# a-ludi/dentist

Measured on AMD Instinct MI355X. Metric: gap-bases closed/sec, higher is better.
Workload: dtype u8

## Files before the change

dentist_amd/_lib.py:

```python
import ctypes
import os
import weakref

import numpy as np

_HERE = os.path.dirname(os.path.abspath(__file__))


def lib_path():
    return os.environ.get("DH_DEV_LIB") or os.path.join(_HERE, "libdentist_hip.so")


class DhError(RuntimeError):
    def __init__(self, code, msg):
        super().__init__(f"libdentist_hip error {code}: {msg}")
        self.code = code


class AlignOpts(ctypes.Structure):
    _fields_ = [(n, ctypes.c_int32) for n in (
        "k", "hmin", "band_shift", "tspace", "min_len", "pen", "xdrop", "max_err_ppm", "max_cand",
        "max_la", "tcap", "strands", "skip_self", "dmax", "width", "kmer_mod", "algo")]


class AlignStats(ctypes.Structure):
    _fields_ = [("hits", ctypes.c_int64), ("cands", ctypes.c_int64), ("alignments", ctypes.c_int64),
                ("wave_cells", ctypes.c_int64), ("las", ctypes.c_int64), ("b_bases", ctypes.c_int64),
                ("ms_index", ctypes.c_float), ("ms_seed", ctypes.c_float), ("ms_wave", ctypes.c_float),
                ("ms_gather", ctypes.c_float), ("ms_total", ctypes.c_float),
                ("wave_launches", ctypes.c_int32), ("overflow_items", ctypes.c_int32), ("big_items", ctypes.c_int64)]

    def as_dict(self):
        return {n: getattr(self, n) for n, _ in self._fields_}


class CumStats(ctypes.Structure):
    _fields_ = [("ms_index", ctypes.c_double), ("ms_seed", ctypes.c_double), ("ms_wave", ctypes.c_double),
                ("ms_gather", ctypes.c_double)] + [(n, ctypes.c_int64) for n in (
                    "wave_launches", "wave_cells", "alignments", "las", "aligned_bp", "trace_values", "hits",
                    "b_bases")]

    def as_dict(self):
        return {n: getattr(self, n) for n, _ in self._fields_}


class ProcessOpts(ctypes.Structure):
    _fields_ = [(n, ctypes.c_int32) for n in (
        "tspace_map", "allowance", "min_anchor", "min_reads", "max_reads", "tspace_pile", "rounds",
        "flank_window", "max_align_err_ppm", "max_ins_err_ppm", "bad_fraction_ppm", "width", "dust", "algo",
        "max_partners", "min_relative_score_ppm")]


INSERTION_DTYPE = np.dtype([(n, "<i4") for n in (
    "contig_left", "status", "nreads", "ref_read", "ref_read_id", "crop_left", "crop_right", "left_aepos",
    "right_abpos", "ins_begin", "ins_end", "comp", "cons_len", "left_diffs", "right_diffs", "join")]
    + [("cons_off", "<i8"), ("contig_right", "<i4"), ("pad", "<i4")])

LA_DTYPE = np.dtype([("tlen", "<i4"), ("diffs", "<i4"), ("abpos", "<i4"), ("bbpos", "<i4"),
                     ("aepos", "<i4"), ("bepos", "<i4"), ("flags", "<u4"), ("aread", "<i4"),
                     ("bread", "<i4"), ("pad", "<i4"), ("toff", "<i8")])

SYMBOLS = [
    "dh_last_error", "dh_abi_version", "dh_ctx_create", "dh_ctx_destroy", "dh_ctx_sync",
    "dh_default_align_opts", "dh_db_create", "dh_db_destroy", "dh_db_drop_cache", "dh_db_nreads",
    "dh_db_total_bases", "dh_la_set_destroy", "dh_la_set_count", "dh_la_set_trace_len",
    "dh_la_set_records", "dh_la_set_trace", "dh_la_set_tspace", "dh_get_align_stats", "dh_get_cum_stats", "dh_get_mjoin_counts", "dh_ctx_release_scratch",
    "dh_align_db",
    "dh_las_write", "dh_las_read", "dh_default_process_opts", "dh_collect_spanning", "dh_pileups_destroy",
    "dh_pileups_count", "dh_pileups_get", "dh_process_pileups", "dh_insertions_destroy",
    "dh_insertions_count", "dh_insertions_records", "dh_insertions_bases", "dh_insertions_bases_len",
    "dh_get_process_stats", "dh_dazz_create_dam", "dh_dazz_create_db", "dh_dazz_split", "dh_dazz_open",
    "dh_dazz_close", "dh_dazz_nreads", "dh_dazz_first_id", "dh_dazz_bases", "dh_dazz_offsets",
    "dh_dazz_origin", "dh_dazz_fpulse", "dh_dazz_header", "dh_dazz_read_mask", "dh_dazz_write_mask",
    "dh_db_set_mask", "dh_output_fasta", "dh_tile_qv", "dh_consensus", "dh_las_merge",
    "dh_collect_candidates", "dh_pileups_create", "dh_pileups_select", "dh_align_db_block", "dh_la_set_merge",
    "dh_crop_pileups", "dh_cropped_create", "dh_cropped_destroy", "dh_cropped_npiles", "dh_cropped_records",
    "dh_cropped_nreads", "dh_cropped_pile", "dh_cropped_entry", "dh_cropped_read_id", "dh_cropped_offsets",
    "dh_cropped_bases", "dh_process_cropped", "dh_translate_trace_point", "dh_db_dust", "dh_db_get_mask",
    "dh_dazz_write_track", "dh_dazz_read_track", "dh_dazz_remove", "dh_dazz_flags",
    "dh_pileupdb_write", "dh_pileupdb_read", "dh_insertiondb_write", "dh_insertiondb_read", "dh_insertiondb_merge", "dh_chaindb_destroy",
    "dh_chaindb_npiles", "dh_chaindb_pile_counts", "dh_chaindb_nread_alignments", "dh_chaindb_read_alignment_counts",
    "dh_chaindb_nseeded", "dh_chaindb_seeded", "dh_chaindb_nlas", "dh_chaindb_las", "dh_chaindb_ntrace",
    "dh_chaindb_trace", "dh_chaindb_ninsertions", "dh_chaindb_insertions", "dh_chaindb_bases", "dh_chaindb_read_ids",
    "dh_insertions_write_db", "dh_pileups_write_db", "dh_pileups_flat", "dh_collect_filter",
    "dh_map_reads", "dh_validate_regions", "dh_propagate_mask", "dh_db_mask_coverage", "dh_max_coverage_reads", "dh_max_improper_coverage_reads",
    "dh_default_scaffold_opts", "dh_scaffold_pileups", "dh_scaffold_npiles", "dh_scaffold_nentries", "dh_scaffold_joins",
    "dh_scaffold_entries", "dh_scaffold_destroy", "dh_scaffold_spanning", "dh_scaffold_gap_pileups", "dh_cropped_create2",
    "dh_cropped_kind", "dh_get_process_work", "dh_scaffold_pileups_cb", "dh_scaffold_pileups_resolved", "dh_comm_unique_id", "dh_comm_create", "dh_comm_create_local", "dh_comm_destroy",
    "dh_comm_rank", "dh_comm_world", "dh_comm_all_gather", "dh_comm_all_to_all", "dh_shard_run", "dh_set_near_best", "dh_ctx_set_near_best", "dh_shard_free", "dh_shard_pack_candidates", "dh_shard_plan_create", "dh_shard_read_joins", "dh_align_db_transposed", "dh_remap_skipping_reads", "dh_shard_graph_plan_create", "dh_shard_plan_destroy",
    "dh_shard_plan_las", "dh_shard_plan_nlas", "dh_shard_plan_pileups", "dh_shard_plan_owner", "dh_shard_pack_cropped",
    "dh_shard_unpack_cropped", "dh_insertions_read_ids", "dh_insertions_read_ids_off", "dh_output_assembly", "dh_default_output_opts",
    "dh_common_trace_point", "dh_pileups_create_joins", "dh_pileups_get_join", "dh_scaffold_all_pileups",
    "dh_crop_pileups_masked", "dh_process_pileups_masked", "dh_process_pileups_set", "dh_la_set_trace_on_device", "dh_scaffold_graph_probe",
    "dh_la_edit_paths", "dh_la_set_edit_paths", "dh_edit_paths_destroy", "dh_edit_paths_count", "dh_edit_paths_op_off",
    "dh_edit_paths_ops", "dh_edit_paths_score", "dh_edit_paths_tile_off", "dh_edit_paths_tile_score",
    "dh_edit_paths_general_tiles", "dh_format_cigar", "dh_format_alignment", "dh_la_transpose", "dh_la_set_transpose",
]

_LIB = None


def lib():
    global _LIB
    if _LIB is not None:
        return _LIB
    path = lib_path()
    if not os.path.exists(path):
        raise RuntimeError(f"{path} is missing: build it with `make` or __graft_entry__.build(); "
                           "dentist_amd has no CPU fallback")
    L = ctypes.CDLL(path)
    vp, i32, i64 = ctypes.c_void_p, ctypes.c_int32, ctypes.c_int64
    L.dh_last_error.restype = ctypes.c_char_p
    L.dh_abi_version.restype = i32
    L.dh_ctx_create.argtypes = [i32, vp, ctypes.POINTER(vp)]
    L.dh_ctx_destroy.argtypes = [vp]
    L.dh_ctx_sync.argtypes = [vp]
    L.dh_default_align_opts.argtypes = [ctypes.POINTER(AlignOpts)]
    L.dh_db_create.argtypes = [vp, vp, vp, i32, vp, ctypes.POINTER(vp)]
    L.dh_db_destroy.argtypes = [vp]
    L.dh_db_drop_cache.argtypes = [vp]
    L.dh_db_nreads.argtypes = [vp]
    L.dh_db_nreads.restype = i32
    L.dh_db_total_bases.argtypes = [vp]
    L.dh_db_total_bases.restype = i64
    L.dh_la_set_destroy.argtypes = [vp]
    L.dh_la_set_count.argtypes = [vp]
    L.dh_la_set_count.restype = i64
    L.dh_la_set_trace_len.argtypes = [vp]
    L.dh_la_set_trace_len.restype = i64
    L.dh_la_set_records.argtypes = [vp]
    L.dh_la_set_records.restype = vp
    L.dh_la_set_trace.argtypes = [vp]
    L.dh_la_set_trace.restype = vp
    L.dh_la_set_tspace.argtypes = [vp]
    L.dh_la_set_tspace.restype = i32
    L.dh_get_align_stats.argtypes = [vp, ctypes.POINTER(AlignStats)]
    L.dh_get_cum_stats.argtypes = [vp, ctypes.POINTER(CumStats), i32]
    L.dh_align_db.argtypes = [vp, vp, vp, ctypes.POINTER(AlignOpts), i32, ctypes.POINTER(vp)]
    L.dh_align_db_block.argtypes = [vp, vp, vp, i32, i32, ctypes.POINTER(AlignOpts), i32, ctypes.POINTER(vp)]
    L.dh_la_set_merge.argtypes = [ctypes.POINTER(vp), i32, ctypes.POINTER(vp)]
    L.dh_las_write.argtypes = [ctypes.c_char_p, vp, i64, vp, i32]
    L.dh_las_read.argtypes = [ctypes.c_char_p, ctypes.POINTER(vp)]
    L.dh_default_process_opts.argtypes = [ctypes.POINTER(ProcessOpts)]
    L.dh_collect_spanning.argtypes = [vp, i64, vp, i32, ctypes.POINTER(ProcessOpts), ctypes.POINTER(vp)]
    L.dh_collect_candidates.argtypes = L.dh_collect_spanning.argtypes
    L.dh_pileups_create.argtypes = [vp, vp, i32, vp, ctypes.POINTER(vp)]
    L.dh_pileups_select.argtypes = [vp, vp, i64, ctypes.POINTER(ProcessOpts), ctypes.POINTER(vp)]
    L.dh_pileups_destroy.argtypes = [vp]
    L.dh_pileups_count.argtypes = [vp]
    L.dh_pileups_count.restype = i32
    L.dh_pileups_get.argtypes = [vp, i32, ctypes.POINTER(i32), ctypes.POINTER(vp)]
    L.dh_pileups_get.restype = i32
    L.dh_process_pileups.argtypes = [vp, vp, vp, vp, i64, vp, vp, ctypes.POINTER(ProcessOpts), ctypes.POINTER(vp)]
    L.dh_crop_pileups.argtypes = [vp, vp, vp, i32, vp, i64, vp, vp, ctypes.POINTER(ProcessOpts), ctypes.POINTER(vp)]
    L.dh_cropped_create.argtypes = [vp, i32, i32, vp, vp, vp, vp, vp, ctypes.POINTER(vp)]
    L.dh_cropped_create2.argtypes = [vp, i32, i32, vp, vp, vp, vp, vp, vp, ctypes.POINTER(vp)]
    L.dh_cropped_kind.argtypes = [vp]
    L.dh_cropped_kind.restype = vp
    L.dh_cropped_destroy.argtypes = [vp]
    for fn in (L.dh_cropped_npiles, L.dh_cropped_nreads):
        fn.argtypes = [vp]
        fn.restype = i32
    for fn in (L.dh_cropped_records, L.dh_cropped_pile, L.dh_cropped_entry, L.dh_cropped_read_id,
               L.dh_cropped_offsets, L.dh_cropped_bases):
        fn.argtypes = [vp]
        fn.restype = vp
    L.dh_process_cropped.argtypes = [vp, vp, vp, ctypes.POINTER(ProcessOpts), ctypes.POINTER(vp)]
    L.dh_translate_trace_point.argtypes = [vp, vp, i32, i32, i32, ctypes.POINTER(i32), ctypes.POINTER(i32)]
    L.dh_insertions_destroy.argtypes = [vp]
    L.dh_insertions_count.argtypes = [vp]
    L.dh_insertions_count.restype = i32
    L.dh_insertions_records.argtypes = [vp]
    L.dh_insertions_records.restype = vp
    L.dh_insertions_bases.argtypes = [vp]
    L.dh_insertions_bases.restype = vp
    L.dh_insertions_bases_len.argtypes = [vp]
    L.dh_insertions_bases_len.restype = i64
    L.dh_get_process_stats.argtypes = [vp, vp, vp]
    L.dh_dazz_create_dam.argtypes = [ctypes.c_char_p, ctypes.c_char_p, i64]
    L.dh_dazz_create_db.argtypes = [ctypes.c_char_p, ctypes.c_char_p, i64]
    L.dh_dazz_split.argtypes = [ctypes.c_char_p, i32, i32, i64]
    L.dh_dazz_open.argtypes = [ctypes.c_char_p, ctypes.POINTER(vp)]
    L.dh_dazz_close.argtypes = [vp]
    L.dh_dazz_nreads.argtypes = [vp]
    L.dh_dazz_nreads.restype = i32
    L.dh_dazz_first_id.argtypes = [vp]
    L.dh_dazz_first_id.restype = i32
    for fn in (L.dh_dazz_bases, L.dh_dazz_offsets, L.dh_dazz_origin, L.dh_dazz_fpulse):
        fn.argtypes = [vp]
        fn.restype = vp
    L.dh_dazz_header.argtypes = [vp, i32]
    L.dh_dazz_read_mask.argtypes = [vp, ctypes.c_char_p, ctypes.c_char_p, vp, vp, i64]
    L.dh_dazz_read_mask.restype = i64
    L.dh_dazz_write_mask.argtypes = [ctypes.c_char_p, ctypes.c_char_p, i32, vp, vp]
    L.dh_db_set_mask.argtypes = [vp, vp, vp]
    L.dh_db_dust.argtypes = [vp]
    L.dh_db_get_mask.argtypes = [vp, vp, vp, i64]
    L.dh_db_get_mask.restype = i64
    L.dh_las_merge.argtypes = [ctypes.POINTER(ctypes.c_char_p), i32, ctypes.c_char_p]
    L.dh_tile_qv.argtypes = [vp, vp, vp, i64, vp, i32, i32, vp, i32]
    L.dh_consensus.argtypes = [vp, vp, vp, i64, vp, i32, i32, i32, vp, i64, ctypes.POINTER(i64)]
    L.dh_output_fasta.argtypes = [ctypes.c_char_p, ctypes.c_char_p, vp, vp, i32, vp, ctypes.POINTER(ctypes.c_char_p),
                                  vp, vp, i32, vp, i32, i32]
    L.dh_dazz_header.restype = ctypes.c_char_p
    L.dh_la_edit_paths.argtypes = [vp, vp, vp, vp, i64, vp, i32, i64, i64, ctypes.POINTER(vp)]
    L.dh_la_set_edit_paths.argtypes = [vp, vp, vp, vp, i64, i64, ctypes.POINTER(vp)]
    L.dh_la_transpose.argtypes = [vp, vp, vp, vp, i64, vp, i32, i32, ctypes.POINTER(vp), vp]
    L.dh_la_set_transpose.argtypes = [vp, vp, vp, vp, i32, ctypes.POINTER(vp), vp]
    L.dh_edit_paths_destroy.argtypes = [vp]
    L.dh_edit_paths_destroy.restype = None
    for fn in (L.dh_edit_paths_count, L.dh_edit_paths_general_tiles):
        fn.argtypes = [vp]
        fn.restype = i64
    for fn in (L.dh_edit_paths_op_off, L.dh_edit_paths_ops, L.dh_edit_paths_score, L.dh_edit_paths_tile_off,
               L.dh_edit_paths_tile_score):
        fn.argtypes = [vp]
        fn.restype = vp
    L.dh_format_cigar.argtypes = [vp, i64, i32, vp, i64]
    L.dh_format_cigar.restype = i64
    L.dh_format_alignment.argtypes = [vp, vp, vp, i64, i32, vp, i64]
    L.dh_format_alignment.restype = i64
    _LIB = L
    return L


def _check(rc):
    if rc != 0:
        raise DhError(rc, lib().dh_last_error().decode(errors="replace"))


def default_align_opts(**kw):
    o = AlignOpts()
    lib().dh_default_align_opts(ctypes.byref(o))
    for k, v in kw.items():
        if not hasattr(o, k):
            raise AttributeError(k)
        setattr(o, k, v)
    return o


class _LaSetOwner:

    def __init__(self, h):
        self._h = h

    def __del__(self):
        try:
            if self._h:
                lib().dh_la_set_destroy(self._h)
                self._h = None
        except Exception:
            pass


def _take_la_set(h):
    L = lib()
    n, tn = L.dh_la_set_count(h), L.dh_la_set_trace_len(h)
    ts = L.dh_la_set_tspace(h)
    owner = _LaSetOwner(h)
    if n:
        buf = (ctypes.c_uint8 * (n * LA_DTYPE.itemsize)).from_address(L.dh_la_set_records(h))
        buf._owner = owner
        las = np.frombuffer(buf, dtype=LA_DTYPE)
    else:
        las = np.zeros(0, dtype=LA_DTYPE)
    if tn:
        buf = (ctypes.c_uint16 * tn).from_address(L.dh_la_set_trace(h))
        buf._owner = owner
        trace = np.frombuffer(buf, dtype=np.uint16)
    else:
        trace = np.zeros(0, dtype=np.uint16)
    return las, trace, ts


class Context:

    def __init__(self, device=0, stream=None):
        h = ctypes.c_void_p()
        _check(lib().dh_ctx_create(device, ctypes.c_void_p(stream) if stream else None, ctypes.byref(h)))
        self._h = h
        self._dbs = []

    def close(self):
        if self._h:
            for ref in self._dbs:
                d = ref()
                if d is not None:
                    d.close()
            self._dbs = []
            lib().dh_ctx_destroy(self._h)
            self._h = None

    def __del__(self):
        try:
            self.close()
        except Exception:
            pass

    def sync(self):
        _check(lib().dh_ctx_sync(self._h))

    def db(self, seqdb):
        return Db(self, seqdb)

    def align_stats(self):
        st = AlignStats()
        _check(lib().dh_get_align_stats(self._h, ctypes.byref(st)))
        return st

    def release_scratch(self):
        lib().dh_ctx_release_scratch.argtypes = [ctypes.c_void_p]
        _check(lib().dh_ctx_release_scratch(self._h))

    def mjoin_counts(self, reset=False):
        out = (ctypes.c_int64 * 2)()
        lib().dh_get_mjoin_counts.argtypes = [ctypes.c_void_p, ctypes.c_void_p, ctypes.c_int32]
        _check(lib().dh_get_mjoin_counts(self._h, out, int(reset)))
        return int(out[0]), int(out[1])

    def cum_stats(self, reset=False):
        st = CumStats()
        _check(lib().dh_get_cum_stats(self._h, ctypes.byref(st), int(reset)))
        return st

    def remap_skipping_reads(self, contigs, reads, contig_ids, read_ids, opts, allowance):
        ci = np.ascontiguousarray(contig_ids, dtype=np.int32)
        ri = np.ascontiguousarray(read_ids, dtype=np.int32)
        h = ctypes.c_void_p()
        L = lib()
        L.dh_remap_skipping_reads.argtypes = [ctypes.c_void_p, ctypes.c_void_p, ctypes.c_void_p, ctypes.c_void_p, ctypes.c_int32,
                                              ctypes.c_void_p, ctypes.c_int32, ctypes.c_void_p, ctypes.c_int32,
# ... 997 lines not shown
    nb = L.dh_insertions_bases_len(h)
    rec = (np.frombuffer(ctypes.string_at(L.dh_insertions_records(h), n * INSERTION_DTYPE.itemsize),
                         dtype=INSERTION_DTYPE).copy() if n else np.zeros(0, dtype=INSERTION_DTYPE))
    bases = (np.frombuffer(ctypes.string_at(L.dh_insertions_bases(h), nb), dtype=np.uint8).copy()
             if nb else np.zeros(0, dtype=np.uint8))
    ids = None
    if read_ids:
        L.dh_insertions_read_ids.restype = ctypes.c_void_p
        L.dh_insertions_read_ids_off.restype = ctypes.c_void_p
        L.dh_insertions_read_ids.argtypes = L.dh_insertions_read_ids_off.argtypes = [ctypes.c_void_p]
        po = L.dh_insertions_read_ids_off(h)
        if po and n:
            off = np.frombuffer(ctypes.string_at(po, 4 * (n + 1)), dtype=np.int32).astype(np.int64)
            tot = int(off[-1])
            idv = (np.frombuffer(ctypes.string_at(L.dh_insertions_read_ids(h), 4 * tot), dtype=np.int32).copy()
                   if tot else np.zeros(0, np.int32))
            ids = (idv, off)
        else:
            ids = (np.zeros(0, np.int32), np.zeros(n + 1, np.int64))
    L.dh_insertions_destroy(h)
    return (rec, bases, ids) if read_ids else (rec, bases)


def _mask_args(repeat_mask):
    if repeat_mask is None:
        return None, None, None
    rp = np.ascontiguousarray(repeat_mask[0], dtype=np.int64)
    ri = np.ascontiguousarray(np.concatenate([np.asarray(repeat_mask[1]).reshape(-1), [0, 0]]), dtype=np.int32)
    return (rp, ri), rp.ctypes.data, ri.ctypes.data


def process_pileups(ctx, contigs, reads, las, trace, piles, opts, insertions_db=None, read_ids=False, repeat_mask=None):
    L = lib()
    h = ctypes.c_void_p()
    keep, rp, ri = _mask_args(repeat_mask)
    if isinstance(trace, DeviceTrace):
        L.dh_process_pileups_set.argtypes = [ctypes.c_void_p] * 9
        _check(L.dh_process_pileups_set(ctx._h, contigs._h, reads._h, trace._h, piles._h, rp, ri, ctypes.byref(opts), ctypes.byref(h)))
        return _take_insertions(h, insertions_db, read_ids)
    arr = np.ascontiguousarray(las, dtype=LA_DTYPE)
    tr = np.ascontiguousarray(trace, dtype=np.uint16)
    L.dh_process_pileups_masked.argtypes = [ctypes.c_void_p] * 4 + [ctypes.c_int64] + [ctypes.c_void_p] * 6
    _check(L.dh_process_pileups_masked(ctx._h, contigs._h, reads._h, arr.ctypes.data, len(arr), tr.ctypes.data,
                                       piles._h, rp, ri, ctypes.byref(opts), ctypes.byref(h)))
    return _take_insertions(h, insertions_db, read_ids)


class OutputOpts(ctypes.Structure):
    _fields_ = [("line_width", ctypes.c_int32), ("highlight", ctypes.c_int32), ("join_policy", ctypes.c_int32),
                ("agp_dazzler", ctypes.c_int32), ("agp_skip_read_ids", ctypes.c_int32), ("only", ctypes.c_int32),
                ("agp_version", ctypes.c_char_p), ("tool", ctypes.c_char_p), ("input_assembly", ctypes.c_char_p),
                ("min_extension_length", ctypes.c_int32), ("pad", ctypes.c_int32)]


JOIN_POLICIES = {"scaffoldGaps": 0, "scaffolds": 1, "contigs": 2}


def output_assembly(fasta_path, contigs, scaffold_of, headers, gap_len, rec, bases, read_ids=None, bed_path=None,
                    agp_path=None, join_policy="scaffoldGaps", agp_dazzler=False, agp_skip_read_ids=False, read_names=None,
                    line_width=50, highlight=True, tool=None, input_assembly=None, only="spanning", min_extension_length=100):
    L = lib()
    o = OutputOpts()
    L.dh_default_output_opts.argtypes = [ctypes.POINTER(OutputOpts)]
    L.dh_default_output_opts(ctypes.byref(o))
    o.line_width, o.highlight, o.join_policy = line_width, int(bool(highlight)), JOIN_POLICIES[join_policy]
    o.agp_dazzler, o.agp_skip_read_ids = int(bool(agp_dazzler)), int(bool(agp_skip_read_ids))
    o.only, o.min_extension_length = {"spanning": 1, "extending": 2, "both": 3}[only], int(min_extension_length)
    if tool is not None:
        o.tool = tool.encode()
    if input_assembly is not None:
        o.input_assembly = input_assembly.encode()
    cb = np.ascontiguousarray(contigs.bases, dtype=np.uint8)
    co = np.ascontiguousarray(contigs.off, dtype=np.int64)
    so = np.ascontiguousarray(scaffold_of, dtype=np.int32)
    gl = np.ascontiguousarray(gap_len, dtype=np.int32) if gap_len is not None else None
    r = np.ascontiguousarray(rec, dtype=INSERTION_DTYPE)
    b = np.ascontiguousarray(bases, dtype=np.uint8)
    hs = (ctypes.c_char_p * len(headers))(*[h.encode() for h in headers])
    ids = off = None
    if read_ids is not None:
        ids = np.ascontiguousarray(read_ids[0], dtype=np.int32)
        off = np.ascontiguousarray(read_ids[1], dtype=np.int32)
    rn = (ctypes.c_char_p * len(read_names))(*[x.encode() for x in read_names]) if read_names is not None else None
    dropped = ctypes.c_int32(0)
    vp = ctypes.c_void_p
    L.dh_output_assembly.argtypes = [ctypes.c_char_p, ctypes.c_char_p, ctypes.c_char_p, vp, vp, ctypes.c_int32, vp, vp, vp, vp,
                                     ctypes.c_int32, vp, vp, vp, ctypes.c_int32, vp, ctypes.POINTER(OutputOpts), ctypes.POINTER(ctypes.c_int32)]
    _check(L.dh_output_assembly(fasta_path.encode(), bed_path.encode() if bed_path else None,
                                agp_path.encode() if agp_path else None, cb.ctypes.data, co.ctypes.data, len(co) - 1,
                                so.ctypes.data, ctypes.cast(hs, vp), gl.ctypes.data if gl is not None else None,
                                r.ctypes.data, len(r), b.ctypes.data if len(b) else None,
                                ids.ctypes.data if ids is not None and len(ids) else (ids.ctypes.data if ids is not None else None),
                                off.ctypes.data if off is not None else None, len(read_names) if read_names is not None else -1,
                                ctypes.cast(rn, vp) if rn is not None else None,
                                ctypes.byref(o), ctypes.byref(dropped)))
    return int(dropped.value)


def output_fasta(fasta_path, contigs, scaffold_of, headers, gap_len, rec, bases, bed_path=None, line_width=50,
                 highlight=True):
    cb = np.ascontiguousarray(contigs.bases, dtype=np.uint8)
    co = np.ascontiguousarray(contigs.off, dtype=np.int64)
    so = np.ascontiguousarray(scaffold_of, dtype=np.int32)
    gl = np.ascontiguousarray(gap_len, dtype=np.int32) if gap_len is not None else None
    r = np.ascontiguousarray(rec, dtype=INSERTION_DTYPE)
    b = np.ascontiguousarray(bases, dtype=np.uint8)
    hs = (ctypes.c_char_p * len(headers))(*[h.encode() for h in headers])
    _check(lib().dh_output_fasta(fasta_path.encode(), bed_path.encode() if bed_path else None, cb.ctypes.data,
                                 co.ctypes.data, len(co) - 1, so.ctypes.data, hs,
                                 gl.ctypes.data if gl is not None else None, r.ctypes.data, len(r),
                                 b.ctypes.data if len(b) else None, line_width, int(bool(highlight))))


def las_merge(paths, out_path):
    arr = (ctypes.c_char_p * len(paths))(*[p.encode() for p in paths])
    _check(lib().dh_las_merge(arr, len(paths), out_path.encode()))


def tile_qv(ctx, db, las, trace, tspace, cov, maxtiles):
    arr = np.ascontiguousarray(las, dtype=LA_DTYPE)
    tr = np.ascontiguousarray(trace, dtype=np.uint16)
    qv = np.zeros((lib().dh_db_nreads(db._h), maxtiles), dtype=np.uint8)
    _check(lib().dh_tile_qv(ctx._h, db._h, arr.ctypes.data, len(arr), tr.ctypes.data, tspace, cov, qv.ctypes.data,
                            maxtiles))
    return qv


def consensus(ctx, db, las, trace, tspace, ref_read, rounds=1):
    arr = np.ascontiguousarray(las, dtype=LA_DTYPE)
    tr = np.ascontiguousarray(trace, dtype=np.uint16)
    cap = 1 << 20
    while True:
        out = np.zeros(cap, dtype=np.uint8)
        n = ctypes.c_int64(0)
        rc = lib().dh_consensus(ctx._h, db._h, arr.ctypes.data, len(arr), tr.ctypes.data, tspace, ref_read, rounds,
                                out.ctypes.data, cap, ctypes.byref(n))
        if rc != 0 and n.value > cap:
            cap = int(n.value)
            continue
        _check(rc)
        return out[:n.value].copy()


def process_stats(ctx):
    ms = (ctypes.c_float * 7)()
    cnt = (ctypes.c_int64 * 3)()
    _check(lib().dh_get_process_stats(ctx._h, ms, cnt))
    names = ("crop", "pile_align", "tile_qv", "consensus", "realign", "flank_align", "total")
    d = {f"ms_{n}": float(ms[i]) for i, n in enumerate(names)}
    d.update(pile_las=int(cnt[0]), tiles=int(cnt[1]), nw_cells=int(cnt[2]))
    wk = (ctypes.c_int64 * 4)()
    _check(lib().dh_get_process_work(ctx._h, wk))
    d.update(pile_ups=int(wk[0]), entries=int(wk[1]), cropped_bases=int(wk[2]), algorithmic_bytes=int(wk[3]))
    return d


def dazz_create_dam(path, fasta_text):
    b = fasta_text.encode() if isinstance(fasta_text, str) else fasta_text
    _check(lib().dh_dazz_create_dam(path.encode(), b, len(b)))


def dazz_create_db(path, fasta_text):
    b = fasta_text.encode() if isinstance(fasta_text, str) else fasta_text
    _check(lib().dh_dazz_create_db(path.encode(), b, len(b)))


def dazz_split(path, cutoff=0, all_reads=True, size_mb=200):
    _check(lib().dh_dazz_split(path.encode(), cutoff, int(all_reads), size_mb))


class DazzDb:

    def __init__(self, path):
        L = lib()
        h = ctypes.c_void_p()
        _check(L.dh_dazz_open(path.encode(), ctypes.byref(h)))
        n = L.dh_dazz_nreads(h)
        self.first_id = L.dh_dazz_first_id(h)
        self.off = np.frombuffer((ctypes.c_int64 * (n + 1)).from_address(L.dh_dazz_offsets(h)), dtype=np.int64).copy()
        tot = int(self.off[-1])
        self.bases = (np.frombuffer((ctypes.c_uint8 * tot).from_address(L.dh_dazz_bases(h)), dtype=np.uint8).copy()
                      if tot else np.zeros(0, np.uint8))
        self.origin = (np.frombuffer((ctypes.c_int32 * n).from_address(L.dh_dazz_origin(h)), dtype=np.int32).copy()
                       if n else np.zeros(0, np.int32))
        self.fpulse = (np.frombuffer((ctypes.c_int32 * n).from_address(L.dh_dazz_fpulse(h)), dtype=np.int32).copy()
                       if n else np.zeros(0, np.int32))
        self.headers = [L.dh_dazz_header(h, i).decode() for i in range(n)]
        self.group = None
        self.mask = None
        self._h = h
        self._path = path

    def read_mask(self, name):
        L = lib()
        ptr = np.zeros(self.n + 1, dtype=np.int64)
        m = L.dh_dazz_read_mask(self._h, self._path.encode(), name.encode(), ptr.ctypes.data, None, 0)
        if m < 0:
            _check(int(m))
        iv = np.zeros(max(2 * m, 2), dtype=np.int32)
        L.dh_dazz_read_mask(self._h, self._path.encode(), name.encode(), ptr.ctypes.data, iv.ctypes.data, m)
        return ptr, iv[:2 * m]

    def close(self):
        if getattr(self, "_h", None):
            lib().dh_dazz_close(self._h)
            self._h = None

    def __del__(self):
        try:
            self.close()
        except Exception:
            pass

    @property
    def n(self):
        return len(self.off) - 1

    def seq(self, i):
        return self.bases[self.off[i]:self.off[i + 1]]


def dazz_write_mask(db_path, name, ptr, iv):
    p = np.ascontiguousarray(ptr, dtype=np.int64)
    v = np.ascontiguousarray(iv, dtype=np.int32)
    _check(lib().dh_dazz_write_mask(db_path.encode(), name.encode(), len(p) - 1, p.ctypes.data, v.ctypes.data))


SEEDED_DTYPE = np.dtype([("id", "<i8"), ("contig_a_id", "<u4"), ("contig_a_len", "<u4"), ("contig_b_id", "<u4"),
                         ("contig_b_len", "<u4"), ("flags", "u1"), ("seed", "u1"), ("tspace", "<u2"), ("nla", "<i4")])
CHAIN_LA_DTYPE = np.dtype([("a_begin", "<u4"), ("a_end", "<u4"), ("b_begin", "<u4"), ("b_end", "<u4"), ("diffs", "<u4"),
                           ("ntp", "<i4")])
INSERTION_REC_DTYPE = np.dtype([("start_contig", "<i8"), ("end_contig", "<i8"), ("start_part", "u1"), ("end_part", "u1"),
                                ("pad", "u1", (6,)), ("seq_len", "<i8"), ("contig_len", "<i8"), ("noverlaps", "<i4"),
                                ("nread_ids", "<i4")])
assert SEEDED_DTYPE.itemsize == 32 and CHAIN_LA_DTYPE.itemsize == 24 and INSERTION_REC_DTYPE.itemsize == 48


def _arr(ptr, n, dt):
    if not n:
        return np.zeros(0, dt)
    addr = ptr if isinstance(ptr, int) else ctypes.cast(ptr, ctypes.c_void_p).value
    return np.frombuffer((ctypes.c_uint8 * (n * np.dtype(dt).itemsize)).from_address(addr), dtype=dt).copy()


def _take_chaindb(h):
    L = lib()
    vp = ctypes.c_void_p
    for fn in ("dh_chaindb_pile_counts", "dh_chaindb_read_alignment_counts", "dh_chaindb_seeded", "dh_chaindb_las",
               "dh_chaindb_trace", "dh_chaindb_insertions", "dh_chaindb_bases", "dh_chaindb_read_ids"):
        getattr(L, fn).restype = vp
        getattr(L, fn).argtypes = [vp]
    for fn in ("dh_chaindb_nseeded", "dh_chaindb_nlas", "dh_chaindb_ntrace"):
        getattr(L, fn).restype = ctypes.c_int64
        getattr(L, fn).argtypes = [vp]
    for fn in ("dh_chaindb_npiles", "dh_chaindb_nread_alignments", "dh_chaindb_ninsertions"):
        getattr(L, fn).argtypes = [vp]
    L.dh_chaindb_destroy.argtypes = [vp]
    ins = _arr(L.dh_chaindb_insertions(h), L.dh_chaindb_ninsertions(h), INSERTION_REC_DTYPE)
    out = dict(pile_counts=_arr(L.dh_chaindb_pile_counts(h), L.dh_chaindb_npiles(h), np.int32),
               ra_counts=_arr(L.dh_chaindb_read_alignment_counts(h), L.dh_chaindb_nread_alignments(h), np.int32),
               seeded=_arr(L.dh_chaindb_seeded(h), L.dh_chaindb_nseeded(h), SEEDED_DTYPE),
               las=_arr(L.dh_chaindb_las(h), L.dh_chaindb_nlas(h), CHAIN_LA_DTYPE),
               trace=_arr(L.dh_chaindb_trace(h), L.dh_chaindb_ntrace(h), np.uint16),
               insertions=ins, bases=_arr(L.dh_chaindb_bases(h), int(ins["seq_len"].sum()) if len(ins) else 0, np.uint8),
               read_ids=_arr(L.dh_chaindb_read_ids(h), int(ins["nread_ids"].sum()) if len(ins) else 0, np.uint32))
    L.dh_chaindb_destroy(h)
    return out


def pileupdb_write(path, pile_counts, ra_counts, seeded, las, trace):
    pc, rc = (np.ascontiguousarray(x, dtype=np.int32) for x in (pile_counts, ra_counts))
    sa, la = np.ascontiguousarray(seeded, dtype=SEEDED_DTYPE), np.ascontiguousarray(las, dtype=CHAIN_LA_DTYPE)
    tr = np.ascontiguousarray(trace, dtype=np.uint16)
    L = lib()
    L.dh_pileupdb_write.argtypes = [ctypes.c_char_p, ctypes.c_int32] + [ctypes.c_void_p] * 5
    _check(L.dh_pileupdb_write(path.encode(), len(pc), pc.ctypes.data, rc.ctypes.data, sa.ctypes.data, la.ctypes.data,
                               tr.ctypes.data))


def pileupdb_read(path):
    h = ctypes.c_void_p()
    L = lib()
    L.dh_pileupdb_read.argtypes = [ctypes.c_char_p, ctypes.POINTER(ctypes.c_void_p)]
    _check(L.dh_pileupdb_read(path.encode(), ctypes.byref(h)))
    return _take_chaindb(h)


def insertiondb_write(path, insertions, bases, read_ids, seeded, las, trace):
    ins = np.ascontiguousarray(insertions, dtype=INSERTION_REC_DTYPE)
    b, ids = np.ascontiguousarray(bases, dtype=np.uint8), np.ascontiguousarray(read_ids, dtype=np.uint32)
    sa, la = np.ascontiguousarray(seeded, dtype=SEEDED_DTYPE), np.ascontiguousarray(las, dtype=CHAIN_LA_DTYPE)
    tr = np.ascontiguousarray(trace, dtype=np.uint16)
    L = lib()
    L.dh_insertiondb_write.argtypes = [ctypes.c_char_p, ctypes.c_int32] + [ctypes.c_void_p] * 6
    _check(L.dh_insertiondb_write(path.encode(), len(ins), ins.ctypes.data, b.ctypes.data, ids.ctypes.data, sa.ctypes.data,
                                  la.ctypes.data, tr.ctypes.data))


def insertiondb_read(path):
    h = ctypes.c_void_p()
    L = lib()
    L.dh_insertiondb_read.argtypes = [ctypes.c_char_p, ctypes.POINTER(ctypes.c_void_p)]
    _check(L.dh_insertiondb_read(path.encode(), ctypes.byref(h)))
    return _take_chaindb(h)


# ... 9 lines not shown
```

dentist_amd/csrc/dh_consensus.hip:

```cpp
#include <hip/hip_runtime.h>
#include <stdint.h>
#include <stdlib.h>

#include "dh_device.h"

#define MAXINS 4
#define OP_WORD(g) ((uint64_t *)opbuf)[(int64_t)(g)*NDP + dp]
#define OP_PUT(op_)                                         \
    {                                                       \
        oacc |= (uint64_t)(uint8_t)(op_) << (8 * (nops & 7)); \
        nops++;                                             \
        if ((nops & 7) == 0) {                              \
            OP_WORD((nops >> 3) - 1) = oacc;                \
            oacc = 0;                                       \
        }                                                   \
    }
#define OP_FLUSH \
    if (nops & 7) OP_WORD(nops >> 3) = oacc;
#define VSTRIDE (6 + 4 * MAXINS)
#define MAXQV 50
#define SEG_MAX 250


__global__ void __launch_bounds__(256)
k_gather_slices(const uint8_t *__restrict__ src, const int64_t *__restrict__ src_off,
                const int32_t *__restrict__ sidx, const int32_t *__restrict__ sbeg,
                const int64_t *__restrict__ dst_off, int32_t n, uint8_t *__restrict__ dst)
{
    const int32_t s = blockIdx.y;
    if (s >= n) return;
    const int64_t so = src_off[sidx[s]] + sbeg[s];
    const int64_t d0 = dst_off[s], len = dst_off[s + 1] - d0;
    for (int64_t i = (int64_t)blockIdx.x * blockDim.x + threadIdx.x; i < len;
         i += (int64_t)gridDim.x * blockDim.x)
        dst[d0 + i] = src[so + i];
}

struct PartDesc {
    int32_t src, sidx, sbeg, len, rc, pad;
    int64_t dst;
};

__global__ void __launch_bounds__(256)
k_gather_parts(const uint8_t *__restrict__ src0, const int64_t *__restrict__ off0,
               const uint8_t *__restrict__ src1, const int64_t *__restrict__ off1,
               const PartDesc *__restrict__ parts, int32_t n, uint8_t *__restrict__ dst)
{
    const int32_t p = blockIdx.y;
    if (p >= n) return;
    const PartDesc d = parts[p];
    const uint8_t *s = (d.src ? src1 + off1[d.sidx] : src0 + off0[d.sidx]) + d.sbeg;
    for (int32_t i = blockIdx.x * blockDim.x + threadIdx.x; i < d.len; i += gridDim.x * blockDim.x) {
        uint8_t c = d.rc ? s[d.len - 1 - i] : s[i];
        if (d.rc && c < 4) c = (uint8_t)(3 - c);
        dst[d.dst + i] = c;
    }
}

#define PF_MAXN 1024
#define PF_MAXG 8
__device__ __forceinline__ int32_t pf_score(int32_t ab, int32_t ae, int32_t bb, int32_t be) { return ((ae - ab) + (be - bb)) / 2; }

__global__ void __launch_bounds__(64)
k_pile_funnel(DhLa *__restrict__ las, const uint32_t *__restrict__ item_off, int32_t nreads, const int64_t *__restrict__ roff,
              int32_t max_err_ppm, int32_t tsp, int32_t *__restrict__ la_first, int32_t *__restrict__ live,
              int32_t *__restrict__ status)
{
    __shared__ int32_t s_b[PF_MAXN], s_ab[PF_MAXN], s_ae[PF_MAXN], s_bb[PF_MAXN], s_be[PF_MAXN];
    __shared__ uint32_t s_fl[PF_MAXN];
    const int32_t r = blockIdx.x;
    if (r >= nreads) return;
    const int lane = threadIdx.x;
    const int32_t l0 = (int32_t)item_off[2 * r], l1 = (int32_t)item_off[2 * r + 2], n = l1 - l0;
    if (lane == 0) {
        la_first[r] = l0;
        if (r == nreads - 1) la_first[nreads] = l1;
    }
    if (n > PF_MAXN) {
        if (lane == 0) {
            atomicOr(status, 1);
            live[r] = 0;
        }
        return;
    }
    for (int32_t i = lane; i < n; i += 64) {
        const DhLa la = las[l0 + i];
        uint32_t fl = la.flags;
        if ((int64_t)la.diffs * 1000000 > (int64_t)max_err_ppm * (la.aepos - la.abpos)) fl |= 0x20u;
        s_b[i] = la.bread;
        s_ab[i] = la.abpos;
        s_ae[i] = la.aepos;
        s_bb[i] = la.bbpos;
        s_be[i] = la.bepos;
        s_fl[i] = fl;
    }
    __syncthreads();
    for (int32_t i = lane; i < n; i += 64) {
        const int32_t b = s_b[i];
        bool leader = true;
        for (int32_t j = 0; j < i && leader; j++) leader = s_b[j] != b;
        if (!leader) continue;
        int32_t idx[PF_MAXG], nen = 0;
        for (int32_t j = i; j < n; j++)
            if (s_b[j] == b && !(s_fl[j] & 0x20u)) {
                if (nen < PF_MAXG) idx[nen] = j;
                nen++;
            }
        if (nen == 0) continue;
        if (nen > PF_MAXG) {
            atomicOr(status, 1);
            continue;
        }
        if (nen == 1) {
            const int32_t x = idx[0];
            if (pf_score(s_ab[x], s_ae[x], s_bb[x], s_be[x]) < tsp)
                s_fl[x] |= 0x20u;
            else
                s_fl[x] = (s_fl[x] & ~(0x4u | 0x8u | 0x10u)) | 0x4u | 0x10u;
            continue;
        }
        for (int32_t u = 1; u < nen; u++) {
            const int32_t x = idx[u];
            int32_t v = u - 1;
            while (v >= 0 && (s_ab[idx[v]] > s_ab[x] || (s_ab[idx[v]] == s_ab[x] && s_bb[idx[v]] > s_bb[x]))) {
                idx[v + 1] = idx[v];
                v--;
            }
            idx[v + 1] = x;
        }
        int32_t dist[PF_MAXG], pred[PF_MAXG];
        for (int32_t v = 0; v < nen; v++) {
            dist[v] = -pf_score(s_ab[idx[v]], s_ae[idx[v]], s_bb[idx[v]], s_be[idx[v]]);
            pred[v] = -1;
        }
        for (int32_t u = 0; u < nen; u++)
            for (int32_t v = u + 1; v < nen; v++) {
                const int32_t x = idx[u], y = idx[v];
                if ((s_fl[x] & 1u) != (s_fl[y] & 1u)) continue;
                const int32_t ga = s_ab[y] - s_ae[x], gb = s_bb[y] - s_be[x];
                if (!(s_ab[x] < s_ab[y] && s_bb[x] < s_bb[y])) continue;
                const int32_t aga = ga < 0 ? -ga : ga, agb = gb < 0 ? -gb : gb, dg = ga - gb < 0 ? gb - ga : ga - gb;
                if (dg > 1000 || (aga > agb ? aga : agb) > 10000) continue;
                const int32_t lax = s_ae[x] - s_ab[x], lay = s_ae[y] - s_ab[y], lbx = s_be[x] - s_bb[x], lby = s_be[y] - s_bb[y];
                const int32_t mla = lax < lay ? lax : lay, mlb = lbx < lby ? lbx : lby;
                if (!((double)(ga < 0 ? -ga : 0) <= 0.3 * (double)mla && (double)(gb < 0 ? -gb : 0) <= 0.3 * (double)mlb)) continue;
                const int32_t d = dist[u] + dg + (aga > agb ? aga : agb) / 10 - pf_score(s_ab[y], s_ae[y], s_bb[y], s_be[y]);
                if (dist[v] > d) {
                    dist[v] = d;
                    pred[v] = u;
                }
            }
        int32_t mind = dist[0];
        for (int32_t v = 1; v < nen; v++) mind = dist[v] < mind ? dist[v] : mind;
        const int32_t best = -mind;
        const double thr_d = (double)tsp > 1.0 * (double)best ? (double)tsp : 1.0 * (double)best;
        const int32_t thr = (int32_t)thr_d;
        int32_t ends[PF_MAXG];
// ... 137 lines not shown
        for (int off = 1; off < 64; off <<= 1) {
            const int32_t v = __shfl_up(incl, off, 64);
            if (lane >= off) incl += v;
        }
        const int32_t m = __shfl(incl, 63, 64);
        int32_t q = MAXQV;
        if (m > 0) {
            const int32_t use = m < cov ? m : cov;
            int32_t before = incl - mine, part = 0;
#pragma unroll
            for (int x = 0; x < 4; x++) {
                int32_t take = use - before;
                take = take < 0 ? 0 : (take > c[x] ? c[x] : take);
                part += take * (4 * lane + x);
                before += c[x];
            }
#pragma unroll
            for (int off = 32; off > 0; off >>= 1) part += __shfl_xor(part, off, 64);
            q = part / use;
            if (q > MAXQV) q = MAXQV;
        }
        if (lane == 0) qv[(int64_t)r * maxtiles + t] = (uint8_t)q;
        __builtin_amdgcn_wave_barrier();
    }
}


struct SegDesc {
    int32_t tmpl;
    int32_t a0, a1;
    int32_t bseq;
    int32_t b0, b1;
    int32_t comp;
    int32_t band;
};

__global__ void __launch_bounds__(64)
k_seg_vote(const SegDesc *__restrict__ segs, int32_t nseg, DbView T, DbView R,
           const uint8_t *__restrict__ rrc, const int64_t *__restrict__ voff,
           uint32_t *__restrict__ dmat, int32_t bandmax, uint8_t *__restrict__ opbuf,
           uint16_t *__restrict__ nops_out, int32_t *__restrict__ status)
{
    extern __shared__ __align__(16) uint8_t smem[];
    const int32_t dp = blockIdx.x * blockDim.x + threadIdx.x;
    if (dp >= nseg) return;
    const SegDesc sg = segs[dp];
    const int32_t rl = sg.a1 - sg.a0, ql = sg.b1 - sg.b0;
    if (rl > SEG_MAX || ql > SEG_MAX || sg.band > bandmax || rl - ql >= sg.band || ql - rl >= sg.band) {
        atomicOr(status, DH_ST_POOL_OVERFLOW);
        nops_out[dp] = 0;
        return;
    }
    const uint8_t *ref = T.bases + T.off[sg.tmpl] + sg.a0;
    const uint8_t *qry = (sg.comp ? rrc : R.bases) + R.off[sg.bseq] + sg.b0;
    const int64_t NDP = nseg;
    const int32_t w = sg.band < 1 ? 1 : sg.band;
    const int32_t WD = (2 * bandmax + 16) >> 4;
#define DM(i, cw) dmat[((int64_t)(i) * WD + (cw)) * NDP + dp]
    uint8_t *row = smem + threadIdx.x;
    uint32_t *qw = (uint32_t *)(smem + (size_t)(2 * bandmax + 2) * 64) + threadIdx.x;
    for (int32_t wd = 0; wd * 8 < ql; wd++) {
        uint32_t x = 0;
        for (int32_t b = 0; b < 8 && wd * 8 + b < ql; b++) x |= (uint32_t)(qry[wd * 8 + b] & 15u) << (4 * b);
        qw[wd * 64] = x;
    }
    for (int32_t c = 0; c <= 2 * w + 1; c++) {
        const int32_t j = c - w;
        row[c * 64] = (uint8_t)((j >= 0 && j <= ql && j < 255) ? j : 255);
    }
    for (int32_t i = 1; i <= rl; i++) {
        const uint32_t rc = ref[i - 1];
        int32_t cst, left;
        if (i <= w) {
            cst = w - i + 1;
            left = i;
        } else {
            cst = 0;
            left = 255;
        }
        int32_t diag = row[cst * 64];
        if (i <= w) row[(w - i) * 64] = (uint8_t)i;
        const int32_t cend = (ql - i + w) < 2 * w ? (ql - i + w) : 2 * w;
        const int32_t jq = i - w + cst - 1;
        int32_t widx = jq >> 3, inword = 8 - (jq & 7);
        uint32_t curw = qw[widx * 64] >> (4 * (jq & 7));
        uint32_t acc = 0;
        for (int32_t c = cst; c <= cend; c++) {
            const int32_t up = c == 2 * w ? 255 : (int32_t)row[(c + 1) * 64];
            const uint32_t qb = curw & 15u;
            curw >>= 4;
            if (--inword == 0) {
                widx++;
                curw = qw[widx * 64];
                inword = 8;
            }
            const int32_t m = diag + (rc == qb ? 0 : 1);
            int32_t v = m < up + 1 ? m : up + 1;
            v = v < left + 1 ? v : left + 1;
            v = v < 255 ? v : 255;
            const uint32_t op = (diag <= left && diag <= up) ? 0u : (left <= up ? 2u : 1u);
            acc |= op << (2 * (c & 15));
            if ((c & 15) == 15) {
                DM(i, c >> 4) = acc;
                acc = 0;
            }
            row[c * 64] = (uint8_t)v;
            diag = up;
            left = v;
        }
        if (cst <= cend && (cend & 15) != 15) DM(i, cend >> 4) = acc;
    }
    const int32_t opcap = 2 * SEG_MAX;
    int32_t i = rl, j = ql, nops = 0;
    uint64_t oacc = 0;
    while (i > 0 && j > 0) {
        const int32_t c = j - i + w;
        const uint8_t op = (uint8_t)((DM(i, c >> 4) >> (2 * (c & 15))) & 3u);
        if (op == 0) {
            --i;
            --j;
        } else if (op == 2) {
            --j;
        } else {
            --i;
        }
        OP_PUT(op)
    }
    while (i > 0) {
        OP_PUT(1)
        --i;
    }
    while (j > 0) {
        OP_PUT(2)
        --j;
    }
    OP_FLUSH
    (void)opcap;
    nops_out[dp] = (uint16_t)nops;
#undef DM
}

#ifdef DH_SEED_PROF
__device__ unsigned long long g_vote_prof[16];
#define VP(i)                                          \
    if (threadIdx.x == 0) {                            \
        const unsigned long long t_ = wall_clock64();  \
        atomicAdd(&g_vote_prof[i], t_ - tp_);          \
        tp_ = t_;                                      \
    }
#else
#define VP(i)
#endif

template <int NW>
struct BV {
    uint64_t w[NW];
};
template <int NW>
__device__ __forceinline__ BV<NW> bv_shl1(const BV<NW> &a)
{
    BV<NW> r;
#pragma unroll
    for (int k = NW - 1; k > 0; k--) r.w[k] = (a.w[k] << 1) | (a.w[k - 1] >> 63);
    r.w[0] = a.w[0] << 1;
    return r;
}
template <int NW>
__device__ __forceinline__ BV<NW> bv_shr1(const BV<NW> &a, uint64_t top)
{
    BV<NW> r;
#pragma unroll
    for (int k = 0; k < NW - 1; k++) r.w[k] = (a.w[k] >> 1) | (a.w[k + 1] << 63);
    r.w[NW - 1] = (a.w[NW - 1] >> 1) | (top << 63);
    return r;
}

template <int NW>
__global__ void __launch_bounds__(64)
k_seg_vote_bp(const SegDesc *__restrict__ segs, int32_t nseg, DbView T, DbView R, const uint8_t *__restrict__ rrc,
              uint64_t *__restrict__ dmat, uint8_t *__restrict__ opbuf, uint16_t *__restrict__ nops_out,
              int32_t *__restrict__ status)
{
    constexpr int HALF = 32 * NW;
    constexpr int QW = (SEG_MAX + 63) / 64 + 1 + NW;
    __shared__ uint64_t s_pl[3][QW][64];
    const int32_t dp = blockIdx.x * blockDim.x + threadIdx.x;
    if (dp >= nseg) return;
    const SegDesc sg = segs[dp];
    const int32_t rl = sg.a1 - sg.a0, ql = sg.b1 - sg.b0;
    if (rl > SEG_MAX || ql > SEG_MAX || sg.band > HALF - 1 || rl - ql >= sg.band || ql - rl >= sg.band) {
        atomicOr(status, DH_ST_POOL_OVERFLOW);
        nops_out[dp] = 0;
        return;
    }
    const uint8_t *ref = T.bases + T.off[sg.tmpl] + sg.a0;
    const uint8_t *qry = (sg.comp ? rrc : R.bases) + R.off[sg.bseq] + sg.b0;
    const int64_t NDP = nseg;
    const int lane = threadIdx.x;
#ifdef DH_SEED_PROF
    unsigned long long tp_ = wall_clock64();
#endif
    {
        uint64_t a0 = 0, a1 = 0, a2 = 0;
        int32_t wi = HALF / 64, bi = HALF % 64;
#pragma unroll
        for (int k = 0; k < QW; k++) s_pl[0][k][lane] = s_pl[1][k][lane] = s_pl[2][k][lane] = 0;
        uint64_t qnext = 0;
        if (ql > 0) __builtin_memcpy(&qnext, qry, 8);
        for (int32_t j0 = 0; j0 < ql; j0 += 8) {
            const uint64_t qw = qnext;
            if (j0 + 8 < ql) __builtin_memcpy(&qnext, qry + j0 + 8, 8);
#pragma unroll
            for (int u = 0; u < 8; u++) {
                const int32_t j = j0 + u;
                if (j >= ql) break;
                const uint64_t c = (qw >> (8 * u)) & 7u;
                a0 |= (c & 1u) << bi;
                a1 |= ((c >> 1) & 1u) << bi;
                a2 |= ((c >> 2) & 1u) << bi;
                if (++bi == 64 || j + 1 == ql) {
                    s_pl[0][wi][lane] = a0;
                    s_pl[1][wi][lane] = a1;
                    s_pl[2][wi][lane] = a2;
                    a0 = a1 = a2 = 0;
                    bi = 0;
                    wi++;
                }
            }
        }
    }
    VP(8)
    BV<NW> p0, p1, p2;
#pragma unroll
    for (int k = 0; k < NW; k++) {
        p0.w[k] = s_pl[0][k][lane];
        p1.w[k] = s_pl[1][k][lane];
        p2.w[k] = s_pl[2][k][lane];
    }
    uint64_t f0 = s_pl[0][NW][lane], f1 = s_pl[1][NW][lane], f2 = s_pl[2][NW][lane];
    int32_t fword = NW, fleft = 64;
    BV<NW> Pv, Mv, lv;
#pragma unroll
    for (int k = 0; k < NW; k++) {
        const uint64_t hi = k * 64 >= HALF ? ~0ull : (k * 64 + 64 <= HALF ? 0ull : ~0ull << (HALF - k * 64));
        Pv.w[k] = hi;
        Mv.w[k] = ~hi;
        const int hb = HALF + 1;
        lv.w[k] = k * 64 >= hb ? ~0ull : (k * 64 + 64 <= hb ? 0ull : ~0ull << (hb - k * 64));
    }
#define DMW(i, k) dmat[((int64_t)(i) * (2 * NW) + (k)) * NDP + dp]
    uint64_t refw = 0;
    for (int32_t i = 1; i <= rl; i++) {
        if (((i - 1) & 7) == 0) __builtin_memcpy(&refw, ref + (i - 1), 8);
        const uint32_t rc = (uint32_t)(refw >> (8 * ((i - 1) & 7))) & 7u;
        const uint64_t x0 = 0ull - (uint64_t)(rc & 1u), x1 = 0ull - (uint64_t)((rc >> 1) & 1u), x2 = 0ull - (uint64_t)((rc >> 2) & 1u);
        {
            const uint64_t top = lv.w[NW - 1] >> 63;
            lv = bv_shr1<NW>(lv, top);
        }
        BV<NW> Eq, D0, HP, HN;
        uint64_t carry = 0;
#pragma unroll
        for (int k = 0; k < NW; k++) {
            Eq.w[k] = ~((p0.w[k] ^ x0) | (p1.w[k] ^ x1) | (p2.w[k] ^ x2)) & lv.w[k];
            const uint64_t x = Eq.w[k] & Pv.w[k];
            const uint64_t s1 = x + Pv.w[k];
            const uint64_t c1 = s1 < x ? 1ull : 0ull;
            const uint64_t s2 = s1 + carry;
            const uint64_t c2 = s2 < s1 ? 1ull : 0ull;
            carry = c1 | c2;
            D0.w[k] = (s2 ^ Pv.w[k]) | Eq.w[k] | Mv.w[k];
            HP.w[k] = Mv.w[k] | ~(D0.w[k] | Pv.w[k]);
            HN.w[k] = Pv.w[k] & D0.w[k];
        }
        const BV<NW> HPs = bv_shl1<NW>(HP), HNs = bv_shl1<NW>(HN);
#pragma unroll
        for (int k = 0; k < NW; k++) {
            uint64_t A = ~HNs.w[k];
            const uint64_t B = ~(D0.w[k] & HP.w[k]);
            const uint64_t t2 = HPs.w[k] & HP.w[k];
            const uint64_t t1 = (HPs.w[k] & ~HP.w[k] & ~HN.w[k]) | (~HPs.w[k] & ~HNs.w[k] & HP.w[k]);
            uint64_t L = ~t2 & ~(t1 & D0.w[k]);
            if (k == 0) {
                A |= 1ull;
                L &= ~1ull;
            }
            DMW(i, k) = A & B;
            DMW(i, NW + k) = L;
        }
        const BV<NW> Xv = bv_shr1<NW>(D0, 0ull);
#pragma unroll
        for (int k = 0; k < NW; k++) {
            Pv.w[k] = HN.w[k] | ~(Xv.w[k] | HP.w[k]);
            Mv.w[k] = HP.w[k] & Xv.w[k];
        }
        p0 = bv_shr1<NW>(p0, f0 & 1ull);
        p1 = bv_shr1<NW>(p1, f1 & 1ull);
        p2 = bv_shr1<NW>(p2, f2 & 1ull);
        f0 >>= 1;
        f1 >>= 1;
        f2 >>= 1;
        if (--fleft == 0) {
            fword++;
            f0 = fword < QW ? s_pl[0][fword][lane] : 0ull;
            f1 = fword < QW ? s_pl[1][fword][lane] : 0ull;
            f2 = fword < QW ? s_pl[2][fword][lane] : 0ull;
            fleft = 64;
        }
    }
    VP(9)
    int32_t i = rl, j = ql, nops = 0;
    uint64_t oacc = 0;
    constexpr int PB = NW == 1 ? 8 : 4;
    while (i > 0 && j > 0) {
        uint64_t zr[PB][NW], lr[PB][NW];
        const int32_t i0 = i;
#pragma unroll
        for (int u = 0; u < PB; u++)
#pragma unroll
            for (int k = 0; k < NW; k++) {
                zr[u][k] = i0 - u > 0 ? DMW(i0 - u, k) : 0ull;
                lr[u][k] = i0 - u > 0 ? DMW(i0 - u, NW + k) : 0ull;
            }
#pragma unroll
        for (int u = 0; u < PB; u++) {
            while (i == i0 - u && i > 0 && j > 0) {
                const int32_t Rr = j - i + HALF;
                uint64_t z = zr[u][0], l = lr[u][0];
                if (NW > 1 && (Rr >> 6)) {
                    z = zr[u][NW - 1];
                    l = lr[u][NW - 1];
                }
                const uint8_t op = ((z >> (Rr & 63)) & 1ull) ? 0 : (((l >> (Rr & 63)) & 1ull) ? 2 : 1);
                if (op == 0) {
                    --i;
                    --j;
                } else if (op == 2) {
                    --j;
                } else {
                    --i;
                }
                OP_PUT(op)
            }
        }
    }
    while (i > 0) {
        OP_PUT(1)
        --i;
    }
    while (j > 0) {
        OP_PUT(2)
        --j;
    }
    OP_FLUSH
    nops_out[dp] = (uint16_t)nops;
    VP(10)
#ifdef DH_SEED_PROF
    if (threadIdx.x == 0) atomicAdd(&g_vote_prof[15], 1ull);
#endif
#undef DMW
}

__host__ __device__ inline int32_t seg_vote2_arr(int32_t ncolmax) { return (ncolmax + 2 + 7) & ~7; }
__host__ __device__ inline int32_t seg_vote2_row(int32_t ncolmax)
{
    const int32_t s = 3 * seg_vote2_arr(ncolmax);
    return ((s >> 3) & 1) ? s : s + 8;
}
__device__ __forceinline__ bool has_byte5(uint64_t w)
{
    const uint64_t t = w ^ 0x0505050505050505ull;
    return (((t - 0x0101010101010101ull) & ~t) & 0x8080808080808080ull) != 0ull;
}
__device__ __forceinline__ uint32_t zero_bytes8(uint64_t t)
{
    const uint64_t m = ~(((t & 0x7F7F7F7F7F7F7F7Full) + 0x7F7F7F7F7F7F7F7Full) | t) & 0x8080808080808080ull;
    const uint32_t lo = (((uint32_t)m >> 7) * 0x01020408u) >> 24, hi = (((uint32_t)(m >> 32) >> 7) * 0x01020408u) >> 24;
    return (lo & 15u) | ((hi & 15u) << 4);
}
__device__ __forceinline__ uint32_t bit_plane8(uint64_t t, int k)
{
    const uint64_t m = (t >> k) & 0x0101010101010101ull;
    const uint32_t lo = ((uint32_t)m * 0x01020408u) >> 24, hi = ((uint32_t)(m >> 32) * 0x01020408u) >> 24;
    return (lo & 15u) | ((hi & 15u) << 4);
}
struct ColSet {
    uint64_t lo, hi;
    __device__ __forceinline__ void put8(int32_t xb, uint32_t m8)
    {
        if (xb < 64)
            lo |= (uint64_t)m8 << xb;
        else
            hi |= (uint64_t)m8 << (xb - 64);
    }
    __device__ __forceinline__ bool test(int32_t x) const { return ((x < 64 ? lo >> x : hi >> (x - 64)) & 1ull) != 0ull; }
    __device__ __forceinline__ void set(int32_t x)
    {
        if (x < 64)
            lo |= 1ull << x;
        else
            hi |= 1ull << (x - 64);
    }
    __device__ __forceinline__ void clear(int32_t x)
    {
        if (x < 64)
            lo &= ~(1ull << x);
        else
            hi &= ~(1ull << (x - 64));
    }
    __device__ __forceinline__ bool any() const { return (lo | hi) != 0ull; }
    __device__ __forceinline__ int32_t pop_lowest()
    {
        if (lo) {
            const int32_t x = __builtin_ctzll(lo);
            lo &= lo - 1;
            return x;
        }
        const int32_t x = __builtin_ctzll(hi);
        hi &= hi - 1;
        return 64 + x;
    }
    __device__ __forceinline__ void keep_below(int32_t n)
    {
        if (n <= 64) {
            hi = 0ull;
            if (n < 64) lo &= (1ull << n) - 1ull;
        } else if (n < 128)
            hi &= (1ull << (n - 64)) - 1ull;
    }
};
__device__ __forceinline__ ColSet operator&(const ColSet &a, const ColSet &b) { return ColSet{a.lo & b.lo, a.hi & b.hi}; }
__device__ __forceinline__ int32_t walk_left(const ColSet &w, int32_t x)
{
    ColSet t{~w.lo, ~w.hi};
    t.keep_below(x);
    if (t.hi) return 128 - __builtin_clzll(t.hi);
    if (t.lo) return 64 - __builtin_clzll(t.lo);
    return 0;
}

template <int NW8>
__global__ void __launch_bounds__(64)
k_seg_vote2(const SegDesc *__restrict__ segs, int32_t nseg, DbView T, DbView R,
            const uint8_t *__restrict__ rrc, const int64_t *__restrict__ voff,
            const uint8_t *__restrict__ opbuf, const uint16_t *__restrict__ nops_in, int32_t ncolmax,
            uint32_t *__restrict__ votes, uint32_t *__restrict__ cdiff, uint32_t *__restrict__ vother)
{
    extern __shared__ __align__(16) uint8_t smem[];
    const int32_t dp = blockIdx.x * blockDim.x + threadIdx.x;
    if (dp >= nseg) return;
    const SegDesc sg = segs[dp];
    const int32_t rl = sg.a1 - sg.a0;
    const int32_t nops = nops_in[dp];
    if (rl > ncolmax || nops == 0) return;
    const uint8_t *ref = T.bases + T.off[sg.tmpl] + sg.a0;
    const uint8_t *qry = (sg.comp ? rrc : R.bases) + R.off[sg.bseq] + sg.b0;
    const int64_t NDP = nseg;
    const int32_t ARR = seg_vote2_arr(ncolmax);
    uint8_t *colst = smem + (size_t)threadIdx.x * seg_vote2_row(ncolmax);
    uint8_t *ins = colst + ARR;
    uint8_t *ibp = ins + ARR;
#ifdef DH_SEED_PROF
    unsigned long long tp_ = wall_clock64();
#endif
#define CS(x) colst[(x)]
#define IN(x) ins[(x)]
#define IB(x) ibp[(x)]
#define CS8(x) (*(const uint64_t *)(colst + (x)))
#define IN8(x) (*(const uint64_t *)(ins + (x)))
#define IB8(x) (*(const uint64_t *)(ibp + (x)))
    uint64_t rwv[NW8 > 0 ? NW8 : 1];
    if (NW8 > 0) {
#pragma unroll
        for (int w = 0; w < NW8; w++) __builtin_memcpy(&rwv[w], ref + min(8 * w, rl & ~7), 8);
    }
    for (int32_t x = 0; x <= rl; x += 8) {
        *(uint64_t *)(ins + x) = 0ull;
        *(uint64_t *)(ibp + x) = 0ull;
    }
    VP(0)
    {
        const uint64_t *opw = (const uint64_t *)opbuf;
        int32_t x = 0, y = 0;
        int32_t g = (nops - 1) >> 3;
        uint64_t wnext = opw[(int64_t)g * NDP + dp];
        uint64_t qnext;
        __builtin_memcpy(&qnext, qry, 8);
        uint32_t rn = 0, rv = 0, rb = 0;
        for (; g >= 0; g--) {
            const uint64_t ow = wnext, qw = qnext;
            const int32_t y0 = y;
            if (g > 0) {
                const uint32_t nval = (uint32_t)min(8, nops - 8 * g);
                const uint32_t dels = zero_bytes8(ow ^ 0x0101010101010101ull) & ((1u << nval) - 1u);
                wnext = opw[(int64_t)(g - 1) * NDP + dp];
                __builtin_memcpy(&qnext, qry + y + ((int32_t)nval - __builtin_popcount(dels)), 8);
            }
#pragma unroll
            for (int u = 7; u >= 0; u--) {
                if (8 * g + u >= nops) continue;
                const uint8_t op = (uint8_t)(ow >> (8 * u));
                if (op <= 1) {
                    if (rn) {
                        IN(x) = (uint8_t)(rn | (rv << 3));
                        IB(x) = (uint8_t)rb;
                        rn = rv = rb = 0;
                    }
                    CS(x) = op == 0 ? (uint8_t)(qw >> (8 * (y - y0))) : (uint8_t)5;
                    y += op == 0 ? 1 : 0;
                    x++;
                } else {
                    const uint32_t q = (uint8_t)(qw >> (8 * (y - y0)));
                    if (rn < MAXINS) {
// ... 246 lines not shown
        for (int k = 0; k < MAXINS; k++) net -= v[(int64_t)re * VSTRIDE + 6 + 4 * k + c];
    const int64_t adj = net >= 0 ? (2 * net + den) / (2 * den) : -((2 * (-net) + den) / (2 * den));
    int64_t target = (int64_t)ncols - adj;
    if (target < 0) target = 0;
    if (target > ncols + MAXINS) target = ncols + MAXINS;
    int64_t extra = target > ncols ? target - ncols : 0, keep = target < ncols ? target : ncols;
    for (int32_t x = rs; x < re; x++) {
        const uint32_t *col = v + (int64_t)x * VSTRIDE;
        uint8_t *o = stage + (voff[t] + x) * ESTR;
        int32_t n = 0;
        const uint32_t cover = col[5];
        const uint8_t pc = (x == rs && rs > 0) ? ref[rs - 1] : 255;
        for (int k = 0; k < MAXINS; k++) {
            const uint32_t *iv = col + 6 + 4 * k;
            uint32_t tot = 0;
            int best = -1;
            for (int b = 0; b < 4; b++) {
                if (b == c || b == pc) continue;
                tot += iv[b];
                if (best < 0 || iv[b] > iv[best]) best = b;
            }
            if (best < 0 || 2 * tot <= cover + 1) break;
            o[n++] = (uint8_t)best;
        }
        int best = c < 4 ? c : 0;
        uint32_t bv[4];
        for (int k = 0; k < 4; k++) bv[k] = col[k] + ((c == k) ? 1u : 0u);
        for (int k = 0; k < 4; k++)
            if (bv[k] > bv[best]) best = k;
        if (best != c) {
            if (2 * col[4] <= cover + 1) o[n++] = (uint8_t)best;
        } else {
            if (x == rs)
                for (int64_t e = 0; e < extra; e++) o[n++] = c;
            if (keep > 0) {
                o[n++] = c;
                keep--;
            }
        }
        cnt[voff[t] + x] = (uint8_t)n;
    }
}

__global__ void __launch_bounds__(256)
k_emit_pack(DbView T, int32_t ntmpl, const int64_t *__restrict__ voff, const uint8_t *__restrict__ stage,
            const uint8_t *__restrict__ cnt, const int64_t *__restrict__ out_off,
            uint8_t *__restrict__ out, int32_t *__restrict__ out_len)
{
    __shared__ int32_t part[256];
    __shared__ int32_t carry;
    const int32_t t = blockIdx.x;
    if (t >= ntmpl) return;
    const int32_t rlen = (int32_t)(T.off[t + 1] - T.off[t]);
    const uint8_t *cn = cnt + voff[t];
    const uint8_t *st = stage + voff[t] * ESTR;
    uint8_t *o = out + out_off[t];
    if (threadIdx.x == 0) carry = 0;
    __syncthreads();
    for (int32_t base = 0; base < rlen; base += 256) {
        const int32_t x = base + threadIdx.x;
        const int32_t my = x < rlen ? cn[x] : 0;
        part[threadIdx.x] = my;
        __syncthreads();
        for (int s = 1; s < 256; s <<= 1) {
            const int32_t add = (int)threadIdx.x >= s ? part[threadIdx.x - s] : 0;
            __syncthreads();
            part[threadIdx.x] += add;
            __syncthreads();
        }
        const int32_t off = carry + part[threadIdx.x] - my;
        for (int32_t e = 0; e < my; e++) o[off + e] = st[(int64_t)x * ESTR + e];
        __syncthreads();
        if (threadIdx.x == 255) carry += part[255];
        __syncthreads();
    }
    if (threadIdx.x == 0) out_len[t] = carry;
}


extern "C" {

void dhk_gather_slices(hipStream_t st, const uint8_t *src, const int64_t *src_off, const int32_t *sidx,
                       const int32_t *sbeg, const int64_t *dst_off, int32_t n, int32_t max_len,
                       uint8_t *dst)
{
    if (n <= 0) return;
    int gx = (max_len + 255) / 256;
    gx = gx < 1 ? 1 : (gx > 64 ? 64 : gx);
    for (int32_t s0 = 0; s0 < n; s0 += 65535) {
        const int32_t cnt = n - s0 < 65535 ? n - s0 : 65535;
        hipLaunchKernelGGL(k_gather_slices, dim3(gx, cnt), dim3(256), 0, st, src, src_off, sidx + s0,
                           sbeg + s0, dst_off + s0, cnt, dst);
    }
}

__global__ void __launch_bounds__(256)
k_gather_ranges16(const uint16_t *__restrict__ src, const int64_t *__restrict__ desc, int32_t n, uint16_t *__restrict__ dst)
{
    const int32_t r = blockIdx.x * 4 + (threadIdx.x >> 6);
    if (r >= n) return;
    const int64_t so = desc[3 * (int64_t)r], d0 = desc[3 * (int64_t)r + 1], len = desc[3 * (int64_t)r + 2];
    for (int64_t e = threadIdx.x & 63; e < len; e += 64) dst[d0 + e] = src[so + e];
}

void dhk_gather_ranges16(hipStream_t st, const uint16_t *src, const int64_t *desc, int32_t n, uint16_t *dst)
{
    if (n <= 0) return;
    hipLaunchKernelGGL(k_gather_ranges16, dim3((uint32_t)((n + 3) / 4)), dim3(256), 0, st, src, desc, n, dst);
}

void dhk_gather_parts(hipStream_t st, const uint8_t *src0, const int64_t *off0, const uint8_t *src1,
                      const int64_t *off1, const void *parts, int32_t n, int32_t max_len, uint8_t *dst)
{
    if (n <= 0) return;
    int gx = (max_len + 255) / 256;
    gx = gx < 1 ? 1 : (gx > 64 ? 64 : gx);
    for (int32_t s0 = 0; s0 < n; s0 += 65535) {
        const int32_t cnt = n - s0 < 65535 ? n - s0 : 65535;
        hipLaunchKernelGGL(k_gather_parts, dim3(gx, cnt), dim3(256), 0, st, src0, off0, src1, off1,
                           (const PartDesc *)parts + s0, cnt, dst);
    }
}

void dhk_pile_funnel(hipStream_t st, DhLa *las, const uint32_t *item_off, int32_t nreads, const int64_t *roff,
                     int32_t max_err_ppm, int32_t tsp, int32_t *la_first, int32_t *live, int32_t *status)
{
    if (nreads <= 0) return;
    hipLaunchKernelGGL(k_pile_funnel, dim3(nreads), dim3(64), 0, st, las, item_off, nreads, roff, max_err_ppm, tsp, la_first,
                       live, status);
}

void dhk_gather_read_records(hipStream_t st, const DhLa *las, const int32_t *la_first, const int32_t *sel,
                             const int32_t *dst_off, int32_t nsel, DhLa *out)
{
    if (nsel <= 0) return;
    hipLaunchKernelGGL(k_gather_read_records, dim3(nsel), dim3(64), 0, st, las, la_first, sel, dst_off, nsel, out);
}

void dhk_tile_qv(hipStream_t st, const DhLa *las, const uint16_t *trace, const int32_t *la_first,
                 const int64_t *roff, int32_t nreads, int32_t tspace, const int32_t *cov, int32_t maxtiles,
                 uint8_t *qv)
{
    if (nreads <= 0) return;
    hipLaunchKernelGGL(k_tile_qv, dim3(nreads), dim3(64), 0, st, las, trace, la_first, roff, nreads,
                       tspace, cov, maxtiles, qv);
}

void dhk_seg_vote(hipStream_t st, const void *segs, int32_t nseg, DbView T, DbView R,
                  const uint8_t *rrc, const int64_t *voff, uint32_t *dmat, int32_t bandmax, int32_t qmax,
                  int32_t ncolmax, uint8_t *opbuf, uint16_t *nops, uint32_t *votes, uint32_t *cdiff,
                  uint32_t *vother, int32_t *status, int32_t mode)
{
    if (nseg <= 0) return;
    if (mode == 1)
        hipLaunchKernelGGL(k_seg_vote_bp<1>, dim3((nseg + 63) / 64), dim3(64), 0, st, (const SegDesc *)segs, nseg, T, R, rrc,
                           (uint64_t *)dmat, opbuf, nops, status);
    else if (mode == 2)
        hipLaunchKernelGGL(k_seg_vote_bp<2>, dim3((nseg + 63) / 64), dim3(64), 0, st, (const SegDesc *)segs, nseg, T, R, rrc,
                           (uint64_t *)dmat, opbuf, nops, status);
    else {
        const size_t lds = (size_t)(2 * bandmax + 2) * 64 + ((size_t)(qmax + 7) / 8 + 1) * 256;
        hipLaunchKernelGGL(k_seg_vote, dim3((nseg + 63) / 64), dim3(64), lds, st, (const SegDesc *)segs, nseg,
                           T, R, rrc, voff, dmat, bandmax, opbuf, nops, status);
    }
    const size_t lds2 = (size_t)seg_vote2_row(ncolmax) * 64;
    const char *ev = getenv("DH_VOTE_BYTEWISE");
    const bool bytewise = ev && atoi(ev) != 0;
    const int32_t nw8 = seg_vote2_arr(ncolmax) / 8;
    auto launch = [&](auto kern) {
        if (lds2 > 65536) (void)hipFuncSetAttribute((const void *)kern, hipFuncAttributeMaxDynamicSharedMemorySize, (int)lds2);
        hipLaunchKernelGGL(kern, dim3((nseg + 63) / 64), dim3(64), lds2, st, (const SegDesc *)segs, nseg, T, R, rrc, voff,
                           (const uint8_t *)opbuf, (const uint16_t *)nops, ncolmax, votes, cdiff, vother);
    };
    if (bytewise || nw8 > 16)
        launch(k_seg_vote2<0>);
    else if (nw8 <= 13)
        launch(k_seg_vote2<13>);
    else
        launch(k_seg_vote2<16>);
#ifdef DH_SEED_PROF
    if (getenv("DH_TRACE") && nseg > 100000) {
        (void)hipStreamSynchronize(st);
        unsigned long long h[16], z[16] = {0};
        (void)hipMemcpyFromSymbol(h, HIP_SYMBOL(g_vote_prof), sizeof h);
        (void)hipMemcpyToSymbol(HIP_SYMBOL(g_vote_prof), z, sizeof z);
        const double w = h[7] ? (double)h[7] : 1.0, wb = h[15] ? (double)h[15] : 1.0;
        fprintf(stderr, "[vote prof] fill mode %d, %.0f wavefronts timed: planes %.1f fill %.1f traceback %.1f us/wavefront\n", mode, wb,
                h[8] / wb / 100.0, h[9] / wb / 100.0, h[10] / wb / 100.0);
        fprintf(stderr, "[vote prof] %d tiles, %.0f wavefronts timed: init %.1f ops %.1f canon-del %.1f canon-ins %.1f votes %.1f us/wavefront\n",
                nseg, w, h[0] / w / 100.0, h[1] / w / 100.0, h[2] / w / 100.0, h[3] / w / 100.0, h[4] / w / 100.0);
    }
#endif
}

void dhk_col_tmpl(hipStream_t st, const int64_t *voff, int32_t ntmpl, int64_t ncols_total, int32_t *col_tmpl)
{
    if (ncols_total <= 0 || ntmpl <= 0) return;
    hipLaunchKernelGGL(k_col_tmpl, dim3((unsigned)((ncols_total + 255) / 256)), dim3(256), 0, st, voff, ntmpl,
                       ncols_total, col_tmpl);
}

void dhk_votes_finish(hipStream_t st, DbView T, const int64_t *voff, const int32_t *col_tmpl, int64_t ncols_total,
                      const uint32_t *cexcl, const uint32_t *vother, uint32_t *votes)
{
    if (ncols_total <= 0) return;
    hipLaunchKernelGGL(k_votes_finish, dim3((unsigned)((ncols_total + 255) / 256)), dim3(256), 0, st, T, voff,
                       col_tmpl, ncols_total, cexcl, vother, votes);
}

void dhk_emit(hipStream_t st, DbView T, int32_t ntmpl, const int64_t *voff, const uint32_t *votes,
              const int32_t *col_tmpl, int64_t ncols_total, uint8_t *stage, uint8_t *cnt,
              const int64_t *out_off, uint8_t *out, int32_t *out_len)
{
    if (ntmpl <= 0) return;
    hipLaunchKernelGGL(k_emit_runs, dim3((unsigned)((ncols_total + 255) / 256)), dim3(256), 0, st, T, ntmpl,
                       voff, votes, col_tmpl, ncols_total, stage, cnt);
    hipLaunchKernelGGL(k_emit_pack, dim3(ntmpl), dim3(256), 0, st, T, ntmpl, voff, stage, cnt, out_off, out,
                       out_len);
}

}
```

dentist_amd/csrc/dh_editpath.h:

```cpp
#ifndef DH_EDITPATH_H
#define DH_EDITPATH_H

#include <stdint.h>
#include <string.h>

#include "dh_bitvec.h"

#if defined(__HIPCC__)
#define EP_HD __host__ __device__ __forceinline__
#else
#define EP_HD inline
#endif

#define EP_OP_MATCH 0
#define EP_OP_DEL 1
#define EP_OP_INS 2
#define EP_OP_MISMATCH 3

#define EP_TSPACE_MAX 250
#define EP_QL_FACTOR 4
#define EP_GEN_COLS 16
#define EP_REJECTED 0x80000000u

struct EpTile {
    int64_t aoff, boff;
    int32_t rl, ql;
    int32_t diffs;
    int32_t comp;
};
struct EpResult {
    uint32_t nops;
    uint32_t score;
};

struct EpCopy {
    int64_t wbase, wstride;
    int64_t out;
    int32_t nops, general;
};

struct EpTrRec {
    int64_t op0;
    int64_t slot0;
    int32_t nops, comp;
    int32_t a0, a1;
};

namespace ep {
using namespace dhbv;

template <int H>
EP_HD void shl1(const uint32_t (&a)[H], uint32_t (&r)[H])
{
    for (int k = H - 1; k > 0; k--) r[k] = funnel32(a[k], a[k - 1], 31);
    r[0] = a[0] << 1;
}
template <int H>
EP_HD void shr1(const uint32_t (&a)[H], uint32_t top, uint32_t (&r)[H])
{
    for (int k = 0; k < H - 1; k++) r[k] = funnel32(a[k + 1], a[k], 1);
    r[H - 1] = (a[H - 1] >> 1) | (top << 31);
}

template <int NW>
EP_HD int64_t dm_index(int32_t i, int p, int k, int64_t stride)
{
    return ((int64_t)(i - 1) * (3 * NW) + p * NW + k) * stride;
}

template <int NW>
EP_HD void fill(const uint8_t *ref, int32_t rl, const uint8_t *qry, int32_t ql, uint64_t *dm, int64_t stride)
{
    constexpr int H = 2 * NW, HALF = 32 * NW;
    uint32_t p0[H], p1[H], p2[H];
    for (int h = 0; h < H; h++) p0[h] = p1[h] = p2[h] = 0;
    for (int g = 0; g < HALF / 8; g++) {
        uint64_t qw = 0;
        if (g * 8 < ql) memcpy(&qw, qry + g * 8, 8);
        uint32_t b0 = 0, b1 = 0, b2 = 0;
        for (int u = 0; u < 8; u++) {
            const uint32_t c = (uint32_t)(qw >> (8 * u));
            b0 |= (c & 1u) << u;
            b1 |= ((c >> 1) & 1u) << u;
            b2 |= ((c >> 2) & 1u) << u;
        }
        const int h = H / 2 + g / 4, sh = 8 * (g & 3);
        p0[h] |= b0 << sh;
        p1[h] |= b1 << sh;
        p2[h] |= b2 << sh;
    }
    uint32_t Pv[H], Mv[H], lv[H];
    for (int h = 0; h < H; h++) {
        Pv[h] = h >= H / 2 ? ~0u : 0u;
        Mv[h] = ~Pv[h];
        lv[h] = h > H / 2 ? ~0u : (h == H / 2 ? ~1u : 0u);
    }
    uint64_t refw = 0, qfw = 0;
    for (int32_t i = 1; i <= rl; i++) {
        const int32_t o = (i - 1) & 7;
        if (o == 0) {
            memcpy(&refw, ref + (i - 1), 8);
            qfw = 0;
            if (HALF + i - 1 < ql) memcpy(&qfw, qry + HALF + i - 1, 8);
        }
        const uint32_t rc = (uint32_t)(refw >> (8 * o));
        const uint32_t n0 = ~bitmask(rc, 0), n1 = ~bitmask(rc, 1), n2 = ~bitmask(rc, 2);
        {
            uint32_t t[H];
            shr1<H>(lv, lv[H - 1] >> 31, t);
            for (int h = 0; h < H; h++) lv[h] = t[h];
        }
        uint32_t Eq[H], S[H], EM[H], sum[H];
        for (int h = 0; h < H; h++) {
            const uint32_t a = b3<(BA ^ BB) & BC>(p0[h], n0, lv[h]);
            const uint32_t e = b3<BA & (BB ^ BC)>(a, p1[h], n1);
            Eq[h] = b3<BA & (BB ^ BC)>(e, p2[h], n2);
            S[h] = Eq[h] & Pv[h];
            EM[h] = Eq[h] | Mv[h];
        }
        {
            uint64_t carry = 0;
            for (int k = 0; k < NW; k++) {
                const uint64_t x = ((uint64_t)S[2 * k + 1] << 32) | S[2 * k], y = ((uint64_t)Pv[2 * k + 1] << 32) | Pv[2 * k];
                const uint64_t s1 = x + y, s2 = s1 + carry;
                carry = (uint64_t)(s1 < x) | (uint64_t)(s2 < s1);
                sum[2 * k] = (uint32_t)s2;
                sum[2 * k + 1] = (uint32_t)(s2 >> 32);
            }
        }
        uint32_t D0[H], HP[H], HN[H], HPs[H], HNs[H], Xv[H];
        for (int h = 0; h < H; h++) {
            D0[h] = b3<(BA ^ BB) | BC>(sum[h], Pv[h], EM[h]);
            HP[h] = b3<BA | ~(BB | BC)>(Mv[h], D0[h], Pv[h]);
            HN[h] = Pv[h] & D0[h];
        }
        shl1<H>(HP, HPs);
        shl1<H>(HN, HNs);
        uint32_t Z[H], L[H];
        for (int h = 0; h < H; h++) {
            Z[h] = b3<~BA & ~(BB & BC)>(HNs[h], D0[h], HP[h]);
            const uint32_t u = b3<BA & ~BB & ~BC>(HPs[h], HP[h], HN[h]);
            const uint32_t v = b3<~BA & ~BB & BC>(HPs[h], HNs[h], HP[h]);
            const uint32_t t1 = b3<(BA | BB) & BC>(u, v, D0[h]);
            L[h] = b3<~(BA & BB) & ~BC>(HPs[h], HP[h], t1);
        }
        L[0] &= ~1u;
        for (int k = 0; k < NW; k++) {
            dm[dm_index<NW>(i, 0, k, stride)] = ((uint64_t)Z[2 * k + 1] << 32) | Z[2 * k];
            dm[dm_index<NW>(i, 1, k, stride)] = ((uint64_t)L[2 * k + 1] << 32) | L[2 * k];
            dm[dm_index<NW>(i, 2, k, stride)] = ((uint64_t)Eq[2 * k + 1] << 32) | Eq[2 * k];
        }
        shr1<H>(D0, 0u, Xv);
        for (int h = 0; h < H; h++) {
            Pv[h] = b3<BA | ~(BB | BC)>(HN[h], Xv[h], HP[h]);
            Mv[h] = HP[h] & Xv[h];
        }
        const uint32_t qc = (uint32_t)(qfw >> (8 * o));
        uint32_t t[H];
        shr1<H>(p0, qc & 1u, t);
        for (int h = 0; h < H; h++) p0[h] = t[h];
        shr1<H>(p1, (qc >> 1) & 1u, t);
        for (int h = 0; h < H; h++) p1[h] = t[h];
        shr1<H>(p2, (qc >> 2) & 1u, t);
        for (int h = 0; h < H; h++) p2[h] = t[h];
    }
}

struct OpWriter {
    uint64_t *ow;
    int64_t ostride;
    uint64_t acc = 0;
    uint32_t nops = 0;
    EP_HD OpWriter(uint64_t *ow_, int64_t ostride_) : ow(ow_), ostride(ostride_) {}
    EP_HD void put(uint32_t op)
    {
        acc |= (uint64_t)op << (8 * (nops & 7));
        nops++;
        if ((nops & 7) == 0) {
            ow[(int64_t)((nops >> 3) - 1) * ostride] = acc;
            acc = 0;
        }
    }
    EP_HD void flush()
    {
        if (nops & 7) ow[(int64_t)(nops >> 3) * ostride] = acc;
    }
};

template <int NW>
EP_HD EpResult traceback(int32_t rl, int32_t ql, const uint64_t *dm, int64_t stride, uint64_t *ow, int64_t ostride)
{
    constexpr int HALF = 32 * NW;
    constexpr int PB = NW == 1 ? 8 : 4;
    OpWriter w(ow, ostride);
    int32_t i = rl, j = ql;
    uint32_t cost = 0, bad = 0;
    while (i > 0 && j > 0 && !bad) {
        uint64_t zr[PB][NW], lr[PB][NW], er[PB][NW];
        const int32_t i0 = i;
        for (int u = 0; u < PB; u++)
            for (int k = 0; k < NW; k++) {
                const bool in = i0 - u > 0;
                zr[u][k] = in ? dm[dm_index<NW>(i0 - u, 0, k, stride)] : 0ull;
                lr[u][k] = in ? dm[dm_index<NW>(i0 - u, 1, k, stride)] : 0ull;
                er[u][k] = in ? dm[dm_index<NW>(i0 - u, 2, k, stride)] : 0ull;
            }
        for (int u = 0; u < PB; u++) {
            while (i == i0 - u && i > 0 && j > 0) {
                const int32_t R = j - i + HALF;
                if ((uint32_t)R >= (uint32_t)(2 * HALF)) {
                    bad = 1;
                    i = -1;
                    break;
                }
                uint64_t z = zr[u][0], l = lr[u][0], e = er[u][0];
                if (NW > 1 && (R >> 6)) {
                    z = zr[u][NW - 1];
                    l = lr[u][NW - 1];
                    e = er[u][NW - 1];
                }
                const uint32_t sh = (uint32_t)R & 63u;
                if ((z >> sh) & 1ull) {
                    const uint32_t m = (uint32_t)(e >> sh) & 1u;
                    w.put(m ? EP_OP_MATCH : EP_OP_MISMATCH);
                    cost += 1u - m;
                    --i;
                    --j;
                } else if ((l >> sh) & 1ull) {
                    w.put(EP_OP_INS);
                    cost++;
                    --j;
                } else {
                    w.put(EP_OP_DEL);
                    cost++;
                    --i;
                }
            }
        }
    }
    while (i > 0) {
        w.put(EP_OP_DEL);
        cost++;
        --i;
    }
    while (j > 0 && !bad) {
        w.put(EP_OP_INS);
        cost++;
        --j;
    }
    w.flush();
    EpResult r;
    r.nops = w.nops | (bad ? EP_REJECTED : 0u);
    r.score = cost;
    return r;
}

inline int tile_class(int32_t rl, int32_t ql, int32_t diffs)
{
    const int64_t band = (int64_t)diffs + 1;
    const int32_t d = rl > ql ? rl - ql : ql - rl;
    if (diffs < 0 || band > 63 || d >= band) return 0;
    return band <= 31 ? 1 : 2;
}


#define EP_TR_NONE 4u
#define EP_TR_LANE_OPS 64
#define EP_TR_PASS_OPS (64 * EP_TR_LANE_OPS)

EP_HD uint64_t tr_word(const uint8_t *ops, int32_t nops, int32_t comp, int32_t k)
{
    const int32_t lo = comp ? nops - 8 - k : k;
    uint64_t w = 0;
    if (lo >= 0 && lo + 8 <= nops) {
        memcpy(&w, ops + lo, 8);
    } else {
        for (int u = 0; u < 8; u++) {
            const int32_t x = lo + u;
            w |= (uint64_t)((x >= 0 && x < nops) ? (uint32_t)ops[x] : EP_TR_NONE) << (8 * u);
        }
    }
    return comp ? __builtin_bswap64(w) : w;
}

EP_HD void tr_count(uint64_t w, uint32_t &a, uint32_t &b, uint32_t &d)
{
    const uint64_t M = 0x0101010101010101ull;
    const uint64_t lo = w & M, hi = (w >> 1) & M, valid = ~(w >> 2) & M;
    a += (uint32_t)__builtin_popcountll(valid & ~(lo & ~hi));
    b += (uint32_t)__builtin_popcountll(valid & ~(hi & ~lo));
    d += (uint32_t)__builtin_popcountll(valid & (lo | hi));
}

template <typename F>
EP_HD void tr_walk(const uint64_t (&w)[8], int32_t pos, int32_t ts, uint32_t b, uint32_t d, F &&at_grid)
{
    int32_t next = (pos / ts + 1) * ts;
    for (int j = 0; j < 8; j++)
        for (int u = 0; u < 8; u++) {
            const uint32_t c = (uint32_t)(w[j] >> (8 * u)) & 0xFFu;
            if (c & EP_TR_NONE) continue;
            b += c != EP_OP_INS;
            d += c != EP_OP_MATCH;
            if (c == EP_OP_DEL || ++pos != next) continue;
            at_grid(next, d, b);
            next += ts;
        }
}

EP_HD int32_t tr_tiles(int32_t a0, int32_t a1, int32_t ts) { return (a1 + ts - 1) / ts - a0 / ts; }

}

#endif
```

dentist_amd/csrc/dh_process.cpp:

```cpp
#include <array>
#include <chrono>
#include <thread>
#include <cstdio>
#include <cstdlib>
#include <cstring>
#include <map>
#include <mutex>
#include <numeric>

#include "dh_internal.h"
#include "dh_parallel.h"

extern "C" {
void dhk_gather_slices(hipStream_t st, const uint8_t *src, const int64_t *src_off, const int32_t *sidx,
                       const int32_t *sbeg, const int64_t *dst_off, int32_t n, int32_t max_len,
                       uint8_t *dst);
void dhk_gather_parts(hipStream_t st, const uint8_t *src0, const int64_t *off0, const uint8_t *src1,
                      const int64_t *off1, const void *parts, int32_t n, int32_t max_len, uint8_t *dst);
void dhk_gather_ranges16(hipStream_t st, const uint16_t *src, const int64_t *desc, int32_t n, uint16_t *dst);
void dhk_tile_qv(hipStream_t st, const DhLa *las, const uint16_t *trace, const int32_t *la_first,
                 const int64_t *roff, int32_t nreads, int32_t tspace, const int32_t *cov, int32_t maxtiles,
                 uint8_t *qv);
void dhk_pile_funnel(hipStream_t st, DhLa *las, const uint32_t *item_off, int32_t nreads, const int64_t *roff,
                     int32_t max_err_ppm, int32_t tsp, int32_t *la_first, int32_t *live, int32_t *status);
void dhk_gather_read_records(hipStream_t st, const DhLa *las, const int32_t *la_first, const int32_t *sel,
                             const int32_t *dst_off, int32_t nsel, DhLa *out);
void dhk_seg_vote(hipStream_t st, const void *segs, int32_t nseg, DbView T, DbView R,
                  const uint8_t *rrc, const int64_t *voff, uint32_t *dmat, int32_t bandmax, int32_t qmax,
                  int32_t ncolmax, uint8_t *opbuf, uint16_t *nops, uint32_t *votes, uint32_t *cdiff,
                  uint32_t *vother, int32_t *status, int32_t mode);
void dhk_votes_finish(hipStream_t st, DbView T, const int64_t *voff, const int32_t *col_tmpl, int64_t ncols_total,
                      const uint32_t *cexcl, const uint32_t *vother, uint32_t *votes);
void dhk_scan(hipStream_t st, uint32_t *v, int64_t n, uint32_t *sums);
void dhk_col_tmpl(hipStream_t st, const int64_t *voff, int32_t ntmpl, int64_t ncols_total, int32_t *col_tmpl);
void dhk_emit(hipStream_t st, DbView T, int32_t ntmpl, const int64_t *voff, const uint32_t *votes,
              const int32_t *col_tmpl, int64_t ncols_total, uint8_t *stage, uint8_t *cnt,
              const int64_t *out_off, uint8_t *out, int32_t *out_len);
}

#define MAXINS 4
#define VSTRIDE (6 + 4 * MAXINS)
#define MAXQV 50
#define SEG_MAX 250
#define FLAG_IMPROPER 0x40u

struct PartDescH {
    int32_t src, sidx, sbeg, len, rc, pad;
    int64_t dst;
};

struct SegDescH {
    int32_t tmpl, a0, a1, bseq, b0, b1, comp, band;
};

extern "C" void dh_default_process_opts(dh_process_opts *o)
{
    memset(o, 0, sizeof(*o));
    o->tspace_map = 100;
    o->allowance = 100;
    o->min_anchor = 500;
    o->min_reads = 3;
    o->max_reads = 60;
    o->tspace_pile = 126;
    o->rounds = 3;
    o->flank_window = 20000;
    o->max_align_err_ppm = 300000;
    o->max_ins_err_ppm = 100000;
    o->bad_fraction_ppm = 80000;
    o->width = 30;
    o->dust = 1;
    o->min_relative_score_ppm = 1000000;
}


int dh_db_adopt(dh_ctx *ctx, uint8_t *d_alloc, uint8_t *d_bases, const std::vector<int64_t> &off,
                const std::vector<int32_t> &group, dh_db **out)
{
    dh_db *db = new dh_db();
    db->ctx = ctx;
    db->n = (int32_t)off.size() - 1;
    db->h_off = off;
    db->total = off.back();
    db->d_bases = d_bases;
    db->d_bases_alloc = d_alloc;
    for (int32_t i = 0; i < db->n; i++)
        db->max_len = std::max<int32_t>(db->max_len, (int32_t)(off[(size_t)i + 1] - off[(size_t)i]));
    HIPCHK(dh_dev_alloc(&db->d_off, sizeof(int64_t) * off.size()));
    HIPCHK(hipMemcpyAsync(db->d_off, off.data(), sizeof(int64_t) * off.size(), hipMemcpyHostToDevice,
                          ctx->stream));
    if (!group.empty()) {
        db->h_group = group;
        for (int32_t g : group) db->ngroups = std::max(db->ngroups, g + 1);
        HIPCHK(dh_dev_alloc(&db->d_group, sizeof(int32_t) * group.size()));
        HIPCHK(hipMemcpyAsync(db->d_group, group.data(), sizeof(int32_t) * group.size(),
                              hipMemcpyHostToDevice, ctx->stream));
    }
    HIPCHK(hipStreamSynchronize(ctx->stream));
    *out = db;
    return DH_OK;
}

int dh_db_from_slices(dh_ctx *ctx, const dh_db *src, const std::vector<int32_t> &sidx,
                      const std::vector<int32_t> &sbeg, const std::vector<int32_t> &slen,
                      const std::vector<int32_t> &group, dh_db **out, bool inherit_mask)
{
    const int32_t n = (int32_t)sidx.size();
    std::vector<int64_t> off((size_t)n + 1, 0);
    int32_t max_len = 0;
    for (int32_t i = 0; i < n; i++) {
        off[(size_t)i + 1] = off[(size_t)i] + slen[(size_t)i];
        max_len = std::max(max_len, slen[(size_t)i]);
    }
    uint8_t *d_alloc = nullptr, *d_bases = nullptr;
    if (int rc = dh_alloc_bases(ctx->stream, off.back(), &d_alloc, &d_bases)) return rc;
    if (int rc = dh_db_adopt(ctx, d_alloc, d_bases, off, group, out)) {
        dh_dev_free(d_alloc);
        return rc;
    }
    if (n > 0) {
        DevBuf<int32_t> d_sidx, d_sbeg;
        HIPCHK(d_sidx.alloc((size_t)n));
        HIPCHK(d_sbeg.alloc((size_t)n));
        HIPCHK(hipMemcpyAsync(d_sidx.p, sidx.data(), sizeof(int32_t) * (size_t)n, hipMemcpyHostToDevice,
                              ctx->stream));
        HIPCHK(hipMemcpyAsync(d_sbeg.p, sbeg.data(), sizeof(int32_t) * (size_t)n, hipMemcpyHostToDevice,
                              ctx->stream));
        dhk_gather_slices(ctx->stream, src->d_bases, src->d_off, d_sidx.p, d_sbeg.p, (*out)->d_off, n,
                          max_len, d_bases);
        if (inherit_mask && src->d_mask_bits) {
            uint8_t *layer;
            if (int rc = dh_ensure_mask_layer(*out, 0, &layer)) return rc;
            dhk_mask_slices(ctx->stream, (const uint32_t *)src->d_mask_bits, src->d_off, d_sidx.p, d_sbeg.p, (*out)->d_off, n,
                            max_len, (uint32_t *)layer);
            if (int rc = dh_mask_recompose(*out)) return rc;
        }
        HIPCHK(hipGetLastError());
        HIPCHK(hipStreamSynchronize(ctx->stream));
    }
    return DH_OK;
}


struct dh_pileups {
    std::vector<int32_t> contig_left;
    std::vector<std::vector<int32_t>> triples;
    std::vector<std::array<int32_t, 4>> join;
    std::array<int32_t, 4> join_of(size_t i) const
    {
        return join.empty() ? std::array<int32_t, 4>{contig_left[i], DH_SEED_BACK, contig_left[i] + 1, DH_SEED_FRONT} : join[i];
    }
};
static int refuse_general(const dh_pileups *p, const char *who)
{
    return p && !p->join.empty() ? dh_fail(DH_EINVAL, std::string(who) + ": pile-ups of general joins are not handled here") : DH_OK;
}

static int collect_candidates(const dh_la *las, int64_t n, const int64_t *contig_off, int32_t ncontigs,
                              const dh_process_opts &o, dh_pileups **out)
{
    if (n >= (1ll << 31)) return dh_fail(DH_EINVAL, "dh_collect_spanning: more than 2^31 - 1 local alignments");
    const int64_t lgrain = 1 << 16, lchunks = (n + lgrain - 1) / lgrain;
    std::vector<std::vector<std::pair<int32_t, int32_t>>> live((size_t)std::max<int64_t>(lchunks, 1));
    std::atomic<int> bad{0};
// ... 525 lines not shown
    std::vector<int32_t> dist(n), pred(n, -1), comp(n);
    for (size_t v = 0; v < n; v++) {
        dist[v] = -score(la[order[v]]);
        comp[v] = (int32_t)v;
    }
    for (size_t u = 0; u < n; u++)
        for (size_t v = u + 1; v < n; v++)
            if (chainable(la[order[u]], la[order[v]])) {
                const int32_t d = dist[u] + chain_score(la[order[u]], la[order[v]]);
                if (dist[v] > d) {
                    dist[v] = d;
                    pred[v] = (int32_t)u;
                }
                const int32_t cu = comp[u], cv = comp[v];
                if (cu != cv)
                    for (size_t w = 0; w < n; w++)
                        if (comp[w] == cv) comp[w] = cu;
            }
    std::vector<size_t> cmin(n, SIZE_MAX), cord;
    for (size_t v = 0; v < n; v++) cmin[(size_t)comp[v]] = std::min(cmin[(size_t)comp[v]], order[v]);
    for (size_t v = 0; v < n; v++)
        if (cmin[v] != SIZE_MAX) cord.push_back(v);
    std::sort(cord.begin(), cord.end(), [&](size_t x, size_t y) { return cmin[x] < cmin[y]; });
    struct Sel {
        size_t end;
        bool alt;
        int32_t score;
    };
    std::vector<Sel> sel;
    std::vector<uint8_t> forbidden(n, 0);
    std::vector<size_t> ends;
    for (size_t c : cord) {
        ends.clear();
        for (size_t v = 0; v < n; v++)
            if ((size_t)comp[v] == c) ends.push_back(v);
        std::stable_sort(ends.begin(), ends.end(), [&](size_t x, size_t y) { return dist[x] < dist[y]; });
        const int32_t cbest = -dist[ends[0]];
        const int32_t cthr = (int32_t)std::max<double>(min_score, min_rel_score * cbest);
        for (size_t e : ends) {
            if (forbidden[e] || -dist[e] < cthr) continue;
            bool alt = false;
            for (int32_t v = (int32_t)e; v >= 0; v = pred[(size_t)v]) {
                alt = alt || forbidden[(size_t)v];
                forbidden[(size_t)v] = 1;
            }
            sel.push_back({e, alt, -dist[e]});
        }
    }
    int32_t best = 0;
    for (size_t x = 0; x < sel.size(); x++)
        if (x == 0 || sel[x].score > best) best = sel[x].score;
    const int32_t thr = (int32_t)std::max<double>(min_score, min_rel_score * best);
    std::vector<uint8_t> occ(n, 0);
    std::vector<size_t> path;
    for (const Sel &c : sel) {
        if (c.score < thr) continue;
        path.clear();
        for (int32_t v = (int32_t)c.end; v >= 0; v = pred[(size_t)v]) path.push_back((size_t)v);
        std::reverse(path.begin(), path.end());
        for (size_t k = 0; k < path.size(); k++) {
            const size_t v = path[k];
            dh_la &l = la[order[v]];
            const uint32_t f = k == 0 ? (DH_FLAG_START | (c.alt ? 0u : DH_FLAG_BEST)) : DH_FLAG_NEXT;
            if (!occ[v]) {
                occ[v] = 1;
                l.flags = (l.flags & ~cmask) | f;
            } else
                dups.push_back({order[v], (l.flags & ~cmask) | f});
        }
    }
    for (size_t v = 0; v < n; v++)
        if (!occ[v]) la[order[v]].flags |= DH_FLAG_DISABLED;
}



extern "C" void dh_insertions_destroy(dh_insertions *r) { delete r; }
extern "C" int32_t dh_insertions_count(const dh_insertions *r) { return r ? (int32_t)r->rec.size() : 0; }
extern "C" const dh_insertion *dh_insertions_records(const dh_insertions *r) { return r ? r->rec.data() : nullptr; }
extern "C" const uint8_t *dh_insertions_bases(const dh_insertions *r) { return r ? r->bases.data() : nullptr; }
extern "C" int64_t dh_insertions_bases_len(const dh_insertions *r) { return r ? (int64_t)r->bases.size() : 0; }
extern "C" const int32_t *dh_insertions_read_ids(const dh_insertions *r) { return r ? r->ids.data() : nullptr; }
extern "C" const int32_t *dh_insertions_read_ids_off(const dh_insertions *r)
{
    return r && r->ids_off.size() == r->rec.size() + 1 ? r->ids_off.data() : nullptr;
}

extern "C" int dh_insertions_write_db(const dh_insertions *r, const int64_t *contig_off, int32_t ncontigs,
                                      int32_t tspace, const char *path)
{
    if (!r || !contig_off || !path || ncontigs < 0) return dh_fail(DH_EINVAL, "dh_insertions_write_db: bad argument");
    std::vector<dh_insertion_rec> ins;
    std::vector<uint8_t> bases;
    std::vector<uint32_t> ids;
    std::vector<dh_seeded> sa;
    std::vector<dh_chain_la> la;
    std::vector<uint16_t> tp;
    for (size_t i = 0; i < r->rec.size(); i++) {
        const dh_insertion &x = r->rec[i];
        if (x.status != DH_PILE_OK || r->flank_of[i] < 0) continue;
        const bool ext = (x.join & DH_JOIN_EXTENSION) != 0;
        const int32_t nf = ext ? 1 : 2;
        const int32_t fcontig[2] = {x.contig_left, ext ? x.contig_left : (x.join == 0 && x.contig_right == 0 ? x.contig_left + 1 : x.contig_right)};
        const bool front[2] = {(x.join & DH_JOIN_FLANK0_FRONT) != 0, (x.join & DH_JOIN_FLANK1_BACK) == 0};
        if (fcontig[0] < 0 || fcontig[0] >= ncontigs || fcontig[1] < 0 || fcontig[1] >= ncontigs)
            return dh_fail(DH_EINVAL, "dh_insertions_write_db: gap outside the contigs");
        dh_insertion_rec q;
        memset(&q, 0, sizeof(q));
        q.start_contig = fcontig[0] + 1;
        q.end_contig = fcontig[1] + 1;
        if (ext) {
            q.start_part = front[0] ? 0 : 2;
            q.end_part = front[0] ? 1 : 3;
        } else {
            q.start_part = front[0] ? 1 : 2;
            q.end_part = front[1] ? 1 : 2;
        }
        q.seq_len = x.cons_len;
        q.contig_len = 0;
        q.noverlaps = nf;
        q.nread_ids = r->ids_off[i + 1] - r->ids_off[i];
        ins.push_back(q);
        bases.insert(bases.end(), r->bases.begin() + x.cons_off, r->bases.begin() + x.cons_off + x.cons_len);
        std::vector<uint32_t> my(r->ids.begin() + r->ids_off[i], r->ids.begin() + r->ids_off[i + 1]);
        for (uint32_t &v : my) v += 1;
        std::sort(my.begin(), my.end());
        ids.insert(ids.end(), my.begin(), my.end());
        for (int side = 0; side < nf; side++) {
            const dh_la &f = r->flank[(size_t)r->flank_of[i] + (size_t)side];
            const int32_t c = fcontig[side];
            dh_seeded s;
            memset(&s, 0, sizeof(s));
            s.id = (int64_t)sa.size();
            s.contig_a_id = (uint32_t)(c + 1);
            s.contig_a_len = (uint32_t)(contig_off[c + 1] - contig_off[c]);
            s.contig_b_id = 1;
            s.contig_b_len = (uint32_t)x.cons_len;
            s.flags = (f.flags & DH_FLAG_COMP) ? 1 : 0;
            s.seed = front[side] ? 0 : 1;
            s.tspace = (uint16_t)tspace;
            s.nla = 1;
            sa.push_back(s);
            la.push_back(dh_chain_la{(uint32_t)f.abpos, (uint32_t)f.aepos, (uint32_t)f.bbpos, (uint32_t)f.bepos, (uint32_t)f.diffs, f.tlen / 2});
            tp.insert(tp.end(), r->flank_tr.begin() + f.toff, r->flank_tr.begin() + f.toff + f.tlen);
        }
    }
    return dh_insertiondb_write(path, (int32_t)ins.size(), ins.data(), bases.data(), ids.data(), sa.data(), la.data(), tp.data());
}

struct ProcStats {
    float ms[7] = {0, 0, 0, 0, 0, 0, 0};
    int64_t counters[3] = {0, 0, 0};
    int64_t work[4] = {0, 0, 0, 0};
};
static thread_local ProcStats g_pstats;

extern "C" int dh_get_process_work(dh_ctx *ctx, int64_t *work4)
{
    if (!ctx || !work4) return dh_fail(DH_EINVAL, "dh_get_process_work: NULL argument");
    memcpy(work4, g_pstats.work, sizeof(g_pstats.work));
    return DH_OK;
}

extern "C" int dh_get_process_stats(dh_ctx *ctx, float *ms7, int64_t *counters3)
{
    if (!ctx) return dh_fail(DH_EINVAL, "ctx is NULL");
    if (ms7) memcpy(ms7, g_pstats.ms, sizeof(g_pstats.ms));
    if (counters3) memcpy(counters3, g_pstats.counters, sizeof(g_pstats.counters));
    return DH_OK;
}


static int consensus_round(dh_ctx *ctx, dh_db *T, dh_db *R, const LaVec &las,
                           const TraceVec &trace, const std::vector<int32_t> &tmpl_of,
                           int32_t ts, dh_db **newT, int64_t *nseg_out, int64_t *ncell_out)
{
    hipStream_t st = ctx->stream;
    std::vector<SegDescH, PinnedAlloc<SegDescH>> segs;
    int32_t wmax = 1, bandmax = 1;
    int64_t ncell = 0;
    size_t class_end[3] = {0, 0, 0};
    {
        std::vector<size_t> sel;
        std::vector<size_t> soff(1, 0);
        {
            const int64_t grain = 1 << 16, nch = ((int64_t)las.size() + grain - 1) / grain;
            std::vector<std::array<std::vector<size_t>, 3>> part((size_t)std::max<int64_t>(nch, 1));
            dh_parallel_for(nch, 1, [&](int64_t clo, int64_t chi) {
                for (int64_t c = clo; c < chi; c++) {
                    const size_t i1 = std::min(las.size(), (size_t)(c + 1) * (size_t)grain);
                    for (size_t i = (size_t)c * (size_t)grain; i < i1; i++)
                        if (tmpl_of[i] >= 0 && !(las[i].flags & DH_FLAG_DISABLED)) {
                            const uint16_t *tr = trace.data() + las[i].toff;
                            bool too_long = false;
                            int32_t dmax = 0;
                            for (int32_t e = 0; e < las[i].tlen / 2; e++) {
                                too_long = too_long || tr[2 * e + 1] > SEG_MAX;
                                dmax = std::max<int32_t>(dmax, tr[2 * e]);
                            }
                            if (!too_long) part[(size_t)c][dmax + 1 <= 31 ? 0 : (dmax + 1 <= 63 ? 1 : 2)].push_back(i);
                        }
                }
            });
            for (int cls = 0; cls < 3; cls++) {
                for (const auto &v : part)
                    for (size_t i : v[(size_t)cls]) {
                        sel.push_back(i);
                        soff.push_back(soff.back() + (size_t)(las[i].tlen / 2));
                    }
                class_end[cls] = soff.back();
            }
        }
        segs.resize(soff.back());
        std::mutex red;
        dh_parallel_for((int64_t)sel.size(), 256, [&](int64_t lo_, int64_t hi_) {
            int32_t wm = 1, bm = 1;
            int64_t nc = 0;
            for (int64_t q = lo_; q < hi_; q++) {
                const size_t i = sel[(size_t)q];
                const int32_t t = tmpl_of[i];
                const dh_la &la = las[i];
                const uint16_t *tr = trace.data() + la.toff;
                SegDescH *out = segs.data() + soff[(size_t)q];
                int32_t a0 = la.abpos, b0 = la.bbpos;
                for (int32_t e = 0; e < la.tlen / 2; e++) {
                    int32_t a1 = (a0 / ts + 1) * ts;
                    if (a1 > la.aepos) a1 = la.aepos;
                    const int32_t b1 = b0 + tr[2 * e + 1];
                    const int32_t band = std::min<int32_t>((int32_t)tr[2 * e], std::max(a1 - a0, b1 - b0)) + 1;
                    out[e] = SegDescH{t, a0, a1, la.bread, b0, b1, (int32_t)(la.flags & DH_FLAG_COMP), band};
                    wm = std::max(wm, b1 - b0);
                    bm = std::max(bm, band);
                    nc += (int64_t)(a1 - a0) * std::min(b1 - b0, 2 * band + 1);
                    a0 = a1;
                    b0 = b1;
                }
            }
            std::lock_guard<std::mutex> lk(red);
            wmax = std::max(wmax, wm);
            bandmax = std::max(bandmax, bm);
            ncell += nc;
        });
    }
    *nseg_out = (int64_t)segs.size();
    *ncell_out = ncell;
    const int32_t nt = T->n;
    std::vector<int64_t> voff((size_t)nt + 1, 0), ooff((size_t)nt + 1, 0);
    for (int32_t t = 0; t < nt; t++) {
        const int64_t len = T->h_off[(size_t)t + 1] - T->h_off[(size_t)t];
        voff[(size_t)t + 1] = voff[(size_t)t] + len + 1;
        ooff[(size_t)t + 1] = ooff[(size_t)t] + len * (1 + 2 * MAXINS) + 8;
    }
    struct { int64_t *p; } d_voff, d_ooff;
    struct { uint32_t *p; } d_votes;
    struct { uint8_t *p; } d_out, d_stage, d_cnt;
    struct { int32_t *p; } d_status, d_outlen, d_coltmpl;
#define SCRP(id, buf, count)                                                                     \
    if (int rc_ = dh_scratch(ctx, id, sizeof(*buf.p) * std::max<size_t>((size_t)(count), 1), (void **)&buf.p)) return rc_;
    SCRP(17, d_voff, voff.size() + ooff.size())
    d_ooff.p = d_voff.p + voff.size();
    SCRP(18, d_votes, (size_t)voff.back() * VSTRIDE)
    SCRP(19, d_out, (size_t)ooff.back())
    SCRP(20, d_status, 2 + (size_t)nt + (size_t)voff.back())
    d_outlen.p = d_status.p + 2;
    d_coltmpl.p = d_outlen.p + nt;
    SCRP(21, d_stage, (size_t)voff.back() * (2 + 2 * MAXINS))
    d_cnt.p = d_stage.p + (size_t)voff.back() * (1 + 2 * MAXINS);
    HIPCHK(hipMemcpyAsync(d_voff.p, voff.data(), sizeof(int64_t) * voff.size(), hipMemcpyHostToDevice, st));
    HIPCHK(hipMemcpyAsync(d_ooff.p, ooff.data(), sizeof(int64_t) * ooff.size(), hipMemcpyHostToDevice, st));
    HIPCHK(dhk_memset(st, d_votes.p, 0, sizeof(uint32_t) * (size_t)voff.back() * VSTRIDE));
    HIPCHK(hipMemsetAsync(d_status.p, 0, sizeof(int32_t), st));
    const size_t ncolp = (size_t)voff.back() + 2;
    struct { uint32_t *p; } d_cdiff;
    SCRP(25, d_cdiff, 2 * ncolp + ncolp / 2048 + 8)
    uint32_t *d_vother = d_cdiff.p + ncolp, *d_csums = d_vother + ncolp;
    HIPCHK(dhk_memset(st, d_cdiff.p, 0, sizeof(uint32_t) * 2 * ncolp));
    if (int rc = dh_ensure_rc(R)) return rc;
    for (int cls = 0; cls < 3; cls++) {
        const size_t c0 = cls ? class_end[cls - 1] : 0, c1 = class_end[cls];
        if (c1 <= c0) continue;
        const int32_t mode = getenv("DH_CONS_SCALAR") ? 0 : (cls == 0 ? 1 : (cls == 1 ? 2 : 0));
        const size_t mrow = mode ? (size_t)16 * (size_t)mode : 4 * (size_t)((2 * bandmax + 16) >> 4);
        const int64_t per_dp = (int64_t)(ts + 1) * (int64_t)mrow + 2 * SEG_MAX;
        const int64_t max_dp = std::max<int64_t>(4096, (6ll << 30) / per_dp);
        for (size_t s0 = c0; s0 < c1; s0 += (size_t)max_dp) {
            const int32_t cnt = (int32_t)std::min<size_t>((size_t)max_dp, c1 - s0);
            struct { SegDescH *p; } ds;
            struct { uint8_t *p; } fm, ob;
            SCRP(22, ds, (size_t)cnt)
            SCRP(23, fm, (size_t)cnt * (size_t)(ts + 1) * mrow + (size_t)cnt * 2 * SEG_MAX + (size_t)cnt * 2 + 32)
            ob.p = fm.p + (((size_t)cnt * (size_t)(ts + 1) * mrow + 7) & ~(size_t)7);
            uint16_t *d_nops = (uint16_t *)(ob.p + (((size_t)cnt * 2 * SEG_MAX + 7) & ~(size_t)7));
            HIPCHK(hipMemcpyAsync(ds.p, segs.data() + s0, sizeof(SegDescH) * (size_t)cnt, hipMemcpyHostToDevice, st));
            dhk_seg_vote(st, ds.p, cnt, T->view(), R->view(), R->d_rc, d_voff.p, (uint32_t *)fm.p, bandmax, wmax, ts,
                         ob.p, d_nops, d_votes.p, d_cdiff.p, d_vother, d_status.p, mode);
            HIPCHK(hipGetLastError());
            HIPCHK(hipStreamSynchronize(st));
        }
    }
    {
        dhk_col_tmpl(st, d_voff.p, nt, voff.back(), d_coltmpl.p);
        HIPCHK(dhk_memset(st, d_cnt.p, 0, (size_t)voff.back()));
        dhk_scan(st, d_cdiff.p, (int64_t)ncolp, d_csums);
        dhk_votes_finish(st, T->view(), d_voff.p, d_coltmpl.p, voff.back(), d_cdiff.p, d_vother, d_votes.p);
        dhk_emit(st, T->view(), nt, d_voff.p, d_votes.p, d_coltmpl.p, voff.back(), d_stage.p, d_cnt.p, d_ooff.p,
                 d_out.p, d_outlen.p);
        HIPCHK(hipStreamSynchronize(st));
    }
    HIPCHK(hipGetLastError());
    std::vector<int32_t> outlen((size_t)nt);
    int32_t status = 0;
    HIPCHK(hipMemcpyAsync(outlen.data(), d_outlen.p, sizeof(int32_t) * (size_t)nt, hipMemcpyDeviceToHost, st));
    HIPCHK(hipMemcpyAsync(&status, d_status.p, sizeof(int32_t), hipMemcpyDeviceToHost, st));
    HIPCHK(hipStreamSynchronize(st));
    if (status) return dh_fail(DH_EOVERFLOW, "consensus: tile exceeds the score-matrix capacity");
    std::vector<int64_t> noff((size_t)nt + 1, 0);
    int32_t max_len = 0;
    for (int32_t t = 0; t < nt; t++) {
        noff[(size_t)t + 1] = noff[(size_t)t] + outlen[(size_t)t];
        max_len = std::max(max_len, outlen[(size_t)t]);
    }
    uint8_t *d_alloc = nullptr, *d_bases = nullptr;
    if (int rc = dh_alloc_bases(st, noff.back(), &d_alloc, &d_bases)) return rc;
    if (int rc = dh_db_adopt(ctx, d_alloc, d_bases, noff, T->h_group, newT)) {
        dh_dev_free(d_alloc);
        return rc;
    }
    std::vector<int32_t> ident((size_t)nt), zero((size_t)nt, 0);
    std::iota(ident.begin(), ident.end(), 0);
    DevBuf<int32_t> d_id, d_zero;
    HIPCHK(d_id.alloc((size_t)nt));
    HIPCHK(d_zero.alloc((size_t)nt));
    HIPCHK(hipMemcpyAsync(d_id.p, ident.data(), sizeof(int32_t) * (size_t)nt, hipMemcpyHostToDevice, st));
    HIPCHK(hipMemcpyAsync(d_zero.p, zero.data(), sizeof(int32_t) * (size_t)nt, hipMemcpyHostToDevice, st));
    dhk_gather_slices(st, d_out.p, d_ooff.p, d_id.p, d_zero.p, (*newT)->d_off, nt, max_len, d_bases);
    HIPCHK(hipGetLastError());
    HIPCHK(hipStreamSynchronize(st));
    return DH_OK;
}


struct DbGuard {
    std::vector<dh_db *> dbs;
    ~DbGuard()
    {
        for (dh_db *d : dbs) dh_db_destroy(d);
    }
};
struct SetGuard {
    std::vector<dh_la_set *> sets;
    ~SetGuard()
    {
        for (dh_la_set *s : sets) dh_la_set_destroy(s);
    }
};

struct ProcTimer {
    hipStream_t st = nullptr;
    hipEvent_t ev[4] = {nullptr, nullptr, nullptr, nullptr};
    bool trace = false;
    double tmark = 0;
    ~ProcTimer()
    {
        for (hipEvent_t e : ev)
            if (e) (void)hipEventDestroy(e);
    }
    static double now_ms()
    {
        return (double)std::chrono::duration_cast<std::chrono::microseconds>(
                   std::chrono::steady_clock::now().time_since_epoch()).count() / 1e3;
    }
    int init(hipStream_t s)
    {
        st = s;
        for (auto &e : ev) HIPCHK(hipEventCreate(&e));
        trace = getenv("DH_TRACE") != nullptr;
        tmark = now_ms();
        return DH_OK;
    }
    hipError_t mark(int i) { return hipEventRecord(ev[i], st); }
    int add_elapsed(int a, int b, float &acc)
    {
        float t = 0;
        HIPCHK(hipEventSynchronize(ev[b]));
        HIPCHK(hipEventElapsedTime(&t, ev[a], ev[b]));
        acc += t;
        return DH_OK;
    }
    void lap(const char *what)
    {
        const double t = now_ms();
        if (trace) fprintf(stderr, "[dh_process] %-28s %.2f ms\n", what, t - tmark);
        tmark = t;
    }
};

static dh_align_opts pile_align_opts(int32_t tspace, int32_t min_len, int32_t max_la, int32_t max_cand)
{
    dh_align_opts ao;
    dh_default_align_opts(&ao);
    ao.tspace = tspace;
    ao.min_len = min_len;
    ao.max_la = max_la;
    ao.max_cand = max_cand;
    return ao;
}

static int realign_round(dh_ctx *ctx, dh_db *R, const dh_align_opts &ro, const std::vector<uint8_t> *active_ok, DbGuard &dbg,
                         SetGuard &sg, ProcTimer *tm, ProcStats *ps, dh_db **T)
{
    const dh_db *T0 = *T;
    dh_la_set *rset = nullptr;
    if (tm) HIPCHK(tm->mark(0));
    if (int rc = dh_align_db_ex(ctx, *T, R, &ro, 0, 0, &rset)) return rc;
    sg.sets.push_back(rset);
    if (tm) {
        HIPCHK(tm->mark(1));
        if (int rc = tm->add_elapsed(0, 1, ps->ms[4])) return rc;
    }
    std::vector<int32_t> tmpl_of(rset->la.size(), -1);
    for (size_t i = 0; i < rset->la.size(); i++) {
        dh_la &la = rset->la[i];
        const int32_t a = la.aread;
        const int32_t alen = (int32_t)(T0->h_off[(size_t)a + 1] - T0->h_off[(size_t)a]);
        const int32_t blen = (int32_t)(R->h_off[(size_t)la.bread + 1] - R->h_off[(size_t)la.bread]);
        if (!valid_pileup_alignment(la, false, alen, blen, ro.tspace)) la.flags |= DH_FLAG_DISABLED;
        if (!active_ok || (*active_ok)[(size_t)a]) tmpl_of[i] = a;
    }
    if (tm) HIPCHK(tm->mark(0));
    dh_db *nT = nullptr;
    int64_t nseg = 0, ncell = 0;
    if (int rc = consensus_round(ctx, *T, R, rset->la, rset->trace, tmpl_of, ro.tspace, &nT, &nseg, &ncell)) return rc;
    dbg.dbs.push_back(nT);
    *T = nT;
    if (tm) {
        ps->counters[1] += nseg;
        ps->counters[2] += ncell;
        HIPCHK(tm->mark(1));
        if (int rc = tm->add_elapsed(0, 1, ps->ms[3])) return rc;
    }
    return DH_OK;
}


static int64_t trace_extent(const dh_la *las, int64_t n)
{
    int64_t m = 0;
    for (int64_t i = 0; i < n; i++) m = std::max<int64_t>(m, las[i].toff + las[i].tlen);
    return m;
}

extern "C" int dh_tile_qv(dh_ctx *ctx, dh_db *db, const dh_la *las, int64_t n, const uint16_t *trace,
                          int32_t tspace, int32_t cov, uint8_t *qv, int32_t maxtiles)
{
    if (!ctx || !db || !qv || (n > 0 && (!las || !trace)) || tspace < 1 || maxtiles < 1 || cov < 1)
        return dh_fail(DH_EINVAL, "dh_tile_qv: bad argument");
    HIPCHK(hipSetDevice(ctx->device));
    hipStream_t st = ctx->stream;
    const int32_t npr = db->n;
    std::vector<int32_t> la_first((size_t)npr + 1, 0);
    for (int64_t i = 0; i < n; i++) {
        if (las[i].aread < 0 || las[i].aread >= npr || (i > 0 && las[i].aread < las[i - 1].aread))
            return dh_fail(DH_EINVAL, "dh_tile_qv: overlaps must be grouped by aread (ascending) and inside the DB");
        la_first[(size_t)las[i].aread + 1]++;
    }
    for (int32_t r = 0; r < npr; r++) la_first[(size_t)r + 1] += la_first[(size_t)r];
    const int64_t nt = trace_extent(las, n);
    DevBuf<DhLa> d_las;
    DevBuf<uint16_t> d_tr;
    DevBuf<int32_t> d_first, d_cov;
    DevBuf<uint8_t> d_qv;
    std::vector<int32_t> cov_of((size_t)npr, cov);
    HIPCHK(d_las.alloc((size_t)n));
    HIPCHK(d_tr.alloc((size_t)nt));
    HIPCHK(d_first.alloc(la_first.size()));
    HIPCHK(d_cov.alloc(cov_of.size()));
    HIPCHK(d_qv.alloc((size_t)npr * maxtiles));
    if (n > 0) {
        HIPCHK(hipMemcpyAsync(d_las.p, las, sizeof(dh_la) * (size_t)n, hipMemcpyHostToDevice, st));
        HIPCHK(hipMemcpyAsync(d_tr.p, trace, sizeof(uint16_t) * (size_t)nt, hipMemcpyHostToDevice, st));
    }
    HIPCHK(hipMemcpyAsync(d_first.p, la_first.data(), sizeof(int32_t) * la_first.size(), hipMemcpyHostToDevice, st));
    HIPCHK(hipMemcpyAsync(d_cov.p, cov_of.data(), sizeof(int32_t) * cov_of.size(), hipMemcpyHostToDevice, st));
    HIPCHK(hipMemsetAsync(d_qv.p, 255, (size_t)npr * maxtiles, st));
    dhk_tile_qv(st, d_las.p, d_tr.p, d_first.p, db->d_off, npr, tspace, d_cov.p, maxtiles, d_qv.p);
    HIPCHK(hipGetLastError());
    HIPCHK(hipMemcpyAsync(qv, d_qv.p, (size_t)npr * maxtiles, hipMemcpyDeviceToHost, st));
    HIPCHK(hipStreamSynchronize(st));
    return DH_OK;
}

extern "C" int dh_consensus(dh_ctx *ctx, dh_db *db, const dh_la *las, int64_t n, const uint16_t *trace,
                            int32_t tspace, int32_t ref_read, int32_t rounds, uint8_t *out, int64_t cap,
                            int64_t *out_len)
{
    if (!ctx || !db || !out || !out_len || (n > 0 && (!las || !trace)) || ref_read < 0 || ref_read >= db->n ||
        rounds < 1 || rounds > 8 || tspace < 16 || tspace > SEG_MAX)
        return dh_fail(DH_EINVAL, "dh_consensus: bad argument");
    HIPCHK(hipSetDevice(ctx->device));
    hipStream_t st = ctx->stream;
    DbGuard dbg;
    SetGuard sg;
    LaVec pl(las, las + n);
    const int64_t nt = trace_extent(las, n);
    TraceVec tr(trace, trace + nt);
    dh_db *T = nullptr;
    const int32_t rlen = (int32_t)(db->h_off[(size_t)ref_read + 1] - db->h_off[(size_t)ref_read]);
    const int32_t grp = db->h_group.empty() ? 0 : db->h_group[(size_t)ref_read];
    if (int rc = dh_db_from_slices(ctx, db, {ref_read}, {0}, {rlen}, {grp}, &T)) return rc;
    dbg.dbs.push_back(T);
    {
        std::vector<int32_t> tmpl_of(pl.size(), -1);
        for (size_t i = 0; i < pl.size(); i++)
            if (pl[i].aread == ref_read) tmpl_of[i] = 0;
        dh_db *nT = nullptr;
        int64_t nseg = 0, ncell = 0;
        if (int rc = consensus_round(ctx, T, db, pl, tr, tmpl_of, tspace, &nT, &nseg, &ncell)) return rc;
        dbg.dbs.push_back(nT);
        T = nT;
    }
    const dh_align_opts ro = pile_align_opts(tspace, 500, 4, 32);
    for (int32_t round = 1; round < rounds; round++)
        if (int rc = realign_round(ctx, db, ro, nullptr, dbg, sg, nullptr, nullptr, &T)) return rc;
    *out_len = T->total;
    if (T->total > cap) return dh_fail(DH_EOVERFLOW, "dh_consensus: output buffer too small");
    if (T->total > 0) HIPCHK(hipMemcpyAsync(out, T->d_bases, (size_t)T->total, hipMemcpyDeviceToHost, st));
    HIPCHK(hipStreamSynchronize(st));
    return DH_OK;
}

struct dh_cropped {
    dh_ctx *ctx = nullptr;
    std::vector<dh_insertion> rec;
    std::vector<int32_t> pile, entry, read_id;
    std::vector<uint8_t> kind;
    std::vector<int64_t> off{0};
    std::vector<uint8_t, PinnedAlloc<uint8_t>> bases;
    bool host_valid = false;
    bool comp_known = true;
    int32_t batch_most = 0;
    dh_db *dev = nullptr;
    float ms_crop = 0;
};

extern "C" void dh_cropped_destroy(dh_cropped *c)
{
    if (!c) return;
    if (c->dev) dh_db_destroy(c->dev);
    delete c;
}
extern "C" int32_t dh_cropped_npiles(const dh_cropped *c) { return c ? (int32_t)c->rec.size() : 0; }
extern "C" const dh_insertion *dh_cropped_records(const dh_cropped *c) { return c ? c->rec.data() : nullptr; }
extern "C" int32_t dh_cropped_nreads(const dh_cropped *c) { return c ? (int32_t)c->pile.size() : 0; }
extern "C" const int32_t *dh_cropped_pile(const dh_cropped *c) { return c ? c->pile.data() : nullptr; }
extern "C" const int32_t *dh_cropped_entry(const dh_cropped *c) { return c ? c->entry.data() : nullptr; }
extern "C" const int32_t *dh_cropped_read_id(const dh_cropped *c) { return c ? c->read_id.data() : nullptr; }
extern "C" const uint8_t *dh_cropped_kind(const dh_cropped *c) { return c ? c->kind.data() : nullptr; }
extern "C" const int64_t *dh_cropped_offsets(const dh_cropped *c) { return c ? c->off.data() : nullptr; }
extern "C" const uint8_t *dh_cropped_bases(dh_cropped *c)
{
    if (!c) return nullptr;
    if (!c->host_valid) {
        c->bases.resize((size_t)std::max<int64_t>(c->off.back(), 1));
        if (c->dev && c->off.back() > 0) {
            if (hipSetDevice(c->ctx->device) != hipSuccess ||
                hipMemcpyAsync(c->bases.data(), c->dev->d_bases, (size_t)c->off.back(), hipMemcpyDeviceToHost,
                               c->ctx->stream) != hipSuccess ||
                hipStreamSynchronize(c->ctx->stream) != hipSuccess) {
                dh_fail(DH_EHIP, "dh_cropped_bases: device to host copy failed");
                return nullptr;
            }
        }
        c->host_valid = true;
    }
    return c->bases.data();
}

extern "C" int dh_cropped_create(const dh_insertion *rec, int32_t npiles, int32_t nreads, const int32_t *pile,
                                 const int32_t *entry, const int32_t *read_id, const int64_t *off,
                                 const uint8_t *bases, dh_cropped **out)
{
    return dh_cropped_create2(rec, npiles, nreads, pile, entry, read_id, nullptr, off, bases, out);
}

extern "C" int dh_cropped_create2(const dh_insertion *rec, int32_t npiles, int32_t nreads, const int32_t *pile,
                                  const int32_t *entry, const int32_t *read_id, const uint8_t *kind, const int64_t *off,
                                  const uint8_t *bases, dh_cropped **out)
{
    if (npiles < 0 || nreads < 0 || !out || (npiles > 0 && !rec) ||
        (nreads > 0 && (!pile || !entry || !read_id || !off || !bases)))
        return dh_fail(DH_EINVAL, "dh_cropped_create: bad argument");
    dh_cropped *c = new dh_cropped();
    c->rec.assign(rec, rec + npiles);
    if (nreads > 0) {
        if (off[0] != 0) {
            delete c;
            return dh_fail(DH_EINVAL, "dh_cropped_create: off[0] must be 0");
        }
        for (int32_t i = 0; i < nreads; i++)
            if (pile[i] < 0 || pile[i] >= npiles || off[i + 1] < off[i] ||
                (i > 0 && (pile[i] < pile[i - 1] || (pile[i] == pile[i - 1] && entry[i] <= entry[i - 1])))) {
                delete c;
                return dh_fail(DH_EINVAL, "dh_cropped_create: reads must be ordered by (pile, entry)");
            }
        c->pile.assign(pile, pile + nreads);
        c->entry.assign(entry, entry + nreads);
        c->read_id.assign(read_id, read_id + nreads);
        if (kind)
            c->kind.assign(kind, kind + nreads);
        else {
            c->kind.assign((size_t)nreads, 0);
            c->comp_known = false;
        }
        for (uint8_t k : c->kind)
            if ((k & 3) > 2 || k > 15) {
                delete c;
                return dh_fail(DH_EINVAL, "dh_cropped_create: kind must be 0, 1 or 2 (| 4, 8: complement alignment on flank 0, 1)");
            }
        c->off.assign(off, off + nreads + 1);
        c->bases.assign(bases, bases + off[nreads]);
    }
    c->host_valid = true;
    *out = c;
    return DH_OK;
}

extern "C" int dh_crop_pileups(dh_ctx *ctx, dh_db *contigs, dh_db *reads, int32_t read_first, const dh_la *las,
                               int64_t n, const uint16_t *trace, const dh_pileups *piles,
                               const dh_process_opts *opts, dh_cropped **out)
{
    return dh_crop_pileups_masked(ctx, contigs, reads, read_first, las, n, trace, piles, nullptr, nullptr, opts, out);
}

extern "C" int dh_crop_pileups_masked(dh_ctx *ctx, dh_db *contigs, dh_db *reads, int32_t read_first, const dh_la *las,
                                      int64_t n, const uint16_t *trace, const dh_pileups *piles, const int64_t *rep_ptr,
                                      const int32_t *rep_iv, const dh_process_opts *opts, dh_cropped **out)
{
    if (!ctx || !contigs || !reads || !piles || !opts || !out || (n > 0 && !las) || (rep_ptr && !rep_iv && rep_ptr[contigs->n] > 0))
        return dh_fail(DH_EINVAL, "dh_crop_pileups: NULL argument");
    const dh_process_opts &o = *opts;
    HIPCHK(hipSetDevice(ctx->device));
    hipStream_t st = ctx->stream;
    hipEvent_t ev[2];
    for (auto &e : ev) HIPCHK(hipEventCreate(&e));
    struct EvGuard {
        hipEvent_t *e;
        ~EvGuard()
        {
            for (int i = 0; i < 2; i++) (void)hipEventDestroy(e[i]);
        }
    } evg{ev};
    HIPCHK(hipEventRecord(ev[0], st));
    dh_cropped *c = new dh_cropped();
    c->ctx = ctx;
    struct CGuard {
        dh_cropped *&c;
        bool ok = false;
        ~CGuard()
        {
            if (!ok) dh_cropped_destroy(c);
        }
    } cg{c};
    const int32_t np = (int32_t)piles->contig_left.size();
    c->rec.resize((size_t)np);
    const int32_t tsm = o.tspace_map;
    std::vector<PartDescH> parts;
    int32_t pile_max_len = 0;
    struct Slice {
        int32_t e, rd, lrd, b0, b1, kind;
    };
    struct PileCrop {
        int32_t pc[2] = {-1, -1}, p0[2] = {0, 0}, p1[2] = {0, 0};
        std::vector<Slice> sl;
    };
    std::vector<PileCrop> pc((size_t)np);
    std::atomic<int> err{0};
// ... 203 lines not shown
    const int64_t grain = 1 << 15, nch = (n + grain - 1) / grain;
    std::vector<std::vector<int64_t>> part((size_t)std::max<int64_t>(nch, 1));
    std::atomic<int> bad{0};
    dh_parallel_for(nch, 1, [&](int64_t clo, int64_t chi) {
        for (int64_t c = clo; c < chi; c++) {
            auto &v = part[(size_t)c];
            for (int64_t i = c * grain; i < std::min(n, (c + 1) * grain); i++) {
                if (la[i].bread < 0 || la[i].bread >= reads->n) continue;
                if (!need[(size_t)la[i].bread] || la[i].tlen <= 0) continue;
                if (la[i].toff < 0 || la[i].toff + la[i].tlen > set->d_trace_own_len) bad = 1;
                v.push_back(i);
            }
        }
    });
    if (bad.load()) return dh_fail(DH_EINVAL, "dh_process_pileups_set: a record's trace lies outside the set's trace");
    std::vector<int64_t> desc;
    int64_t total = 0;
    for (const auto &v : part)
        for (int64_t i : v) {
            desc.push_back(la[i].toff);
            desc.push_back(total);
            desc.push_back(la[i].tlen);
            total += la[i].tlen;
        }
    const int64_t nsel = (int64_t)desc.size() / 3;
    TraceVec sparse_v((size_t)std::max<int64_t>(set->d_trace_own_len, 1));
    uint16_t *sparse = sparse_v.data();
    if (nsel > 0) {
        if (nsel > INT32_MAX) return dh_fail(DH_EOVERFLOW, "dh_process_pileups_set: too many records");
        DevBuf<int64_t> d_desc;
        DevBuf<uint16_t> d_tt;
        HIPCHK(d_desc.alloc(desc.size()));
        HIPCHK(d_tt.alloc((size_t)total));
        TraceVec tmp((size_t)total);
        HIPCHK(hipMemcpyAsync(d_desc.p, desc.data(), sizeof(int64_t) * desc.size(), hipMemcpyHostToDevice, st));
        dhk_gather_ranges16(st, set->d_trace_own, d_desc.p, (int32_t)nsel, d_tt.p);
        HIPCHK(hipGetLastError());
        HIPCHK(hipMemcpyAsync(tmp.data(), d_tt.p, sizeof(uint16_t) * (size_t)total, hipMemcpyDeviceToHost, st));
        HIPCHK(hipStreamSynchronize(st));
        const int64_t *dp = desc.data();
        const uint16_t *tp = tmp.data();
        dh_parallel_for(nsel, 4096, [&](int64_t lo, int64_t hi) {
            for (int64_t r = lo; r < hi; r++) memcpy(sparse + dp[3 * r], tp + dp[3 * r + 1], sizeof(uint16_t) * (size_t)dp[3 * r + 2]);
        });
    }
    return dh_process_pileups_masked(ctx, contigs, reads, la, n, sparse, piles, rep_ptr, rep_iv, opts, out);
}

extern "C" int dh_process_pileups_masked(dh_ctx *ctx, dh_db *contigs, dh_db *reads, const dh_la *las, int64_t n,
                                         const uint16_t *trace, const dh_pileups *piles, const int64_t *rep_ptr,
                                         const int32_t *rep_iv, const dh_process_opts *opts, dh_insertions **out)
{
    if (!ctx || !contigs || !reads || !piles || !opts || !out || (n > 0 && (!las || !trace)))
        return dh_fail(DH_EINVAL, "dh_process_pileups: NULL argument");
    int32_t batch_most = 0;
    for (const auto &t : piles->triples) batch_most = std::max(batch_most, (int32_t)(t.size() / 3));
    auto one = [&](dh_ctx *cx, const dh_pileups *pl, dh_insertions **res) -> int {
        dh_cropped *c = nullptr;
        if (int rc = dh_crop_pileups_masked(cx, contigs, reads, 0, las, n, trace, pl, rep_ptr, rep_iv, opts, &c)) return rc;
        c->batch_most = batch_most;
        const int rc = dh_process_cropped(cx, contigs, c, opts, res);
        dh_cropped_destroy(c);
        return rc;
    };
    const size_t np = piles->contig_left.size();
    if (np < 64 || getenv("DH_PROCESS_SERIAL")) return one(ctx, piles, out);
    int32_t nparts = 3;
    if (const char *e = getenv("DH_PROCESS_PARTS")) nparts = std::max(1, std::min(4, atoi(e)));
    nparts = (int32_t)std::min<size_t>((size_t)nparts, np / 16);
    if (nparts < 2) return one(ctx, piles, out);
    for (int32_t k = 1; k < nparts; k++)
        if (!ctx->sub[k - 1])
            if (int rc = dh_ctx_create(ctx->device, nullptr, &ctx->sub[k - 1])) return rc;
    std::vector<double> cost(np);
    double total = 0;
    for (size_t p = 0; p < np; p++) {
        const double e = (double)piles->triples[p].size() / 3.0;
        cost[p] = e * e;
        total += cost[p];
    }
    std::vector<double> wcum((size_t)nparts + 1, 0.0);
    {
        std::vector<double> wt((size_t)nparts, 1.0);
        if (const char *e = getenv("DH_PROCESS_SPLIT")) {
            const char *q = e;
            for (int32_t k = 0; k < nparts && *q; k++) {
                wt[(size_t)k] = std::max(0.01, atof(q));
                while (*q && *q != ',') q++;
                if (*q == ',') q++;
            }
        }
        double sum = 0;
        for (double x : wt) sum += x;
        for (int32_t k = 0; k < nparts; k++) wcum[(size_t)k + 1] = wcum[(size_t)k] + wt[(size_t)k] / sum;
    }
    std::vector<size_t> cut((size_t)nparts + 1, np);
    cut[0] = 0;
    {
        size_t p = 0;
        double acc = 0;
        for (int32_t k = 1; k < nparts; k++) {
            while (p < np && acc + cost[p] <= total * wcum[(size_t)k]) acc += cost[p++];
            while (p < cut[(size_t)k - 1] + 1) acc += cost[p++];
            p = std::min(p, np - (size_t)(nparts - k));
            cut[(size_t)k] = p;
        }
    }
    std::vector<dh_pileups> part((size_t)nparts);
    for (int32_t k = 0; k < nparts; k++)
        for (size_t p = cut[(size_t)k]; p < cut[(size_t)k + 1]; p++) {
            part[(size_t)k].contig_left.push_back(piles->contig_left[p]);
            part[(size_t)k].triples.push_back(piles->triples[p]);
            if (!piles->join.empty()) part[(size_t)k].join.push_back(piles->join[p]);
        }
    std::vector<dh_insertions *> res((size_t)nparts, nullptr);
    std::vector<int> rcs((size_t)nparts, DH_OK);
    std::vector<std::string> msgs((size_t)nparts);
    std::vector<ProcStats> sts((size_t)nparts);
    std::vector<std::thread> workers;
    for (int32_t k = 1; k < nparts; k++)
        workers.emplace_back([&, k] {
            try {
                rcs[(size_t)k] = one(ctx->sub[k - 1], &part[(size_t)k], &res[(size_t)k]);
                if (rcs[(size_t)k]) msgs[(size_t)k] = dh_last_error();
            } catch (const std::exception &e) {
                rcs[(size_t)k] = DH_EINVAL;
                msgs[(size_t)k] = std::string("dh_process_pileups: a concurrent part of the batch failed: ") + e.what();
            }
            sts[(size_t)k] = g_pstats;
        });
    try {
        rcs[0] = one(ctx, &part[0], &res[0]);
    } catch (const std::exception &e) {
        rcs[0] = dh_fail(DH_EINVAL, std::string("dh_process_pileups: the first part of the batch failed: ") + e.what());
    }
    for (std::thread &w : workers) w.join();
    for (int32_t k = 1; k < nparts; k++) {
        dh_cum_stats &a = ctx->cum, &b = ctx->sub[k - 1]->cum;
        a.ms_index += b.ms_index; a.ms_seed += b.ms_seed; a.ms_wave += b.ms_wave; a.ms_gather += b.ms_gather;
        a.wave_launches += b.wave_launches; a.wave_cells += b.wave_cells; a.alignments += b.alignments; a.las += b.las;
        a.aligned_bp += b.aligned_bp; a.trace_values += b.trace_values; a.hits += b.hits; a.b_bases += b.b_bases;
        b = dh_cum_stats();
    }
    for (int32_t k = 0; k < nparts; k++)
        if (rcs[(size_t)k]) {
            for (dh_insertions *r : res) dh_insertions_destroy(r);
            if (k == 0) return rcs[0];
            return dh_fail(rcs[(size_t)k], msgs[(size_t)k].empty() ? "dh_process_pileups: a concurrent part of the batch failed" : msgs[(size_t)k]);
        }
    for (int32_t k = 1; k < nparts; k++) {
        for (int i = 0; i < 7; i++) g_pstats.ms[i] = std::max(g_pstats.ms[i], sts[(size_t)k].ms[i]);
        for (int i = 0; i < 3; i++) g_pstats.counters[i] += sts[(size_t)k].counters[i];
        for (int i = 0; i < 4; i++) g_pstats.work[i] += sts[(size_t)k].work[i];
    }
    dh_insertions *r0 = res[0];
    for (int32_t k = 1; k < nparts; k++) {
        dh_insertions *r1 = res[(size_t)k];
        const int64_t b0 = (int64_t)r0->bases.size();
        const int32_t f0 = (int32_t)r0->flank.size(), i0 = r0->ids_off.empty() ? 0 : r0->ids_off.back();
        const int64_t t0 = (int64_t)r0->flank_tr.size();
        for (dh_insertion x : r1->rec) {
            x.cons_off += b0;
            r0->rec.push_back(x);
        }
        r0->bases.insert(r0->bases.end(), r1->bases.begin(), r1->bases.end());
        for (dh_la f : r1->flank) {
            f.toff += t0;
            r0->flank.push_back(f);
        }
        r0->flank_tr.insert(r0->flank_tr.end(), r1->flank_tr.begin(), r1->flank_tr.end());
        for (int32_t v : r1->flank_of) r0->flank_of.push_back(v < 0 ? v : v + f0);
        if (!r1->ids_off.empty()) {
            if (r0->ids_off.empty()) r0->ids_off.push_back(0);
            for (size_t j = 1; j < r1->ids_off.size(); j++) r0->ids_off.push_back(r1->ids_off[j] + i0);
            r0->ids.insert(r0->ids.end(), r1->ids.begin(), r1->ids.end());
        }
        dh_insertions_destroy(r1);
    }
    *out = r0;
    return DH_OK;
}


struct ProcRun {
    dh_ctx *ctx;
    hipStream_t st;
    const dh_process_opts &o;
    dh_db *contigs;
    dh_cropped *crop;
    int32_t tsp, pwidth, palgo;
    dh_insertions *res = nullptr;
    ProcStats ps;
    ProcTimer tm;
    DbGuard dbg;
    SetGuard sg;
    ~ProcRun() { delete res; }
    dh_align_opts align_opts(int32_t min_len, int32_t max_la, int32_t max_cand) const
    {
        dh_align_opts ao = pile_align_opts(tsp, min_len, max_la, max_cand);
        ao.width = pwidth;
        ao.algo = palgo;
        return ao;
    }
};

struct PileLayout {
    int32_t na = 0;
    std::vector<int32_t> pile_of_active;
    std::vector<int32_t> first_read;
    std::vector<int32_t> read_id;
    std::vector<uint8_t> rkind;
    std::vector<uint8_t> rcomp;
    std::vector<int32_t> sgroup, keep;
    dh_db *pile = nullptr;
    std::vector<uint8_t> active_ok;
    std::vector<int32_t> ref_of;
};

struct FunnelOut {
    dh_la_set *pset = nullptr;
    bool on_dev = false;
    std::vector<int32_t> la_first;
    std::vector<int32_t> dev_live;
    DevBuf<int32_t> d_first_keep;
    std::vector<uint8_t> qv;
    int32_t maxtiles = 1;
    std::vector<int32_t> cov_of;
};

struct FlankOut {
    std::vector<int32_t> fbeg, flen, fbase;
    dh_la_set *fset = nullptr;
};

static int check_process_opts(dh_ctx *ctx, dh_db *contigs, dh_cropped *crop, const dh_process_opts *opts, dh_insertions **out,
                              int32_t *pwidth_out, int32_t *palgo_out)
{
    if (!ctx || !contigs || !crop || !opts || !out) return dh_fail(DH_EINVAL, "dh_process_cropped: NULL argument");
    const dh_process_opts &o = *opts;
    if (o.max_reads != 0 && (o.max_reads < 3 || o.max_reads > 250))
        return dh_fail(DH_EINVAL, "max_reads must be 0 (no cap) or in [3, 250]");
    if (o.max_partners != 0 && o.max_partners < 4) return dh_fail(DH_EINVAL, "max_partners must be 0 (every pair) or at least 4");
    if (o.min_relative_score_ppm < 1 || o.min_relative_score_ppm > 1000000)
        return dh_fail(DH_EINVAL, "min_relative_score_ppm must be in [1, 1000000] (1000000 = the default 1.0; fill the struct with dh_default_process_opts)");
    if (o.rounds < 1 || o.rounds > 8) return dh_fail(DH_EINVAL, "rounds must be in [1, 8]");
    if (o.tspace_pile < 16 || o.tspace_pile > SEG_MAX) return dh_fail(DH_EINVAL, "tspace_pile out of range");
    int32_t pwidth = o.width > 0 ? o.width : 30;
    if (const char *e = getenv("DH_PILE_WIDTH")) pwidth = atoi(e);
    if (pwidth < 1 || pwidth > 62) return dh_fail(DH_EINVAL, "process: width must be in [1, 62]");
    if (o.algo != 0 && o.algo != 1) return dh_fail(DH_EINVAL, "process: algo must be 0 (DH-1) or 1 (DH-2)");
    if (o.algo == 1) pwidth = o.width == 32 ? 32 : 64;
    *pwidth_out = pwidth;
    *palgo_out = o.algo;
    return DH_OK;
}

static void init_result(ProcRun &run)
{
    const dh_cropped *crop = run.crop;
    dh_insertions *res = run.res = new dh_insertions();
    const int32_t np = (int32_t)crop->rec.size();
    res->rec = crop->rec;
    res->flank_of.assign((size_t)np, -1);
    res->ids_off.assign((size_t)np + 1, 0);
    for (int32_t p : crop->pile) res->ids_off[(size_t)p + 1]++;
    for (int32_t p = 0; p < np; p++) res->ids_off[(size_t)p + 1] += res->ids_off[(size_t)p];
    res->ids.resize((size_t)res->ids_off.back());
    std::vector<int32_t> at(res->ids_off.begin(), res->ids_off.end() - 1);
    for (size_t i = 0; i < crop->pile.size(); i++) res->ids[(size_t)at[(size_t)crop->pile[i]]++] = crop->read_id[i];
}

static int plan_pile_db(ProcRun &run, PileLayout &lay)
{
    const dh_process_opts &o = run.o;
    const dh_db *contigs = run.contigs;
    const dh_cropped *crop = run.crop;
    dh_insertions *res = run.res;
    ProcStats &ps = run.ps;
    const int32_t np = (int32_t)crop->rec.size(), ncr = (int32_t)crop->pile.size();
    std::vector<int32_t> active_of((size_t)np, -1);
    for (int32_t p = 0; p < np; p++) {
        dh_insertion &r = res->rec[(size_t)p];
        r.nreads = res->ids_off[(size_t)p + 1] - res->ids_off[(size_t)p];
        if (r.status != DH_PILE_OK) continue;
        if (r.join == 0 && r.contig_right == 0 && r.contig_left + 1 < contigs->n) r.contig_right = r.contig_left + 1;
        if (r.contig_left < 0 || r.contig_left >= contigs->n || ((r.join & DH_JOIN_EXTENSION) ? r.contig_right != -1 : (r.contig_right <= r.contig_left || r.contig_right >= contigs->n)))
            return dh_fail(DH_EINVAL, "dh_process_cropped: gap outside the contigs DB");
        if (r.nreads < o.min_reads)
            r.status = DH_PILE_TOO_SMALL;
        else if (o.max_reads > 0 && r.nreads > o.max_reads)
            return dh_fail(DH_EINVAL, "dh_process_cropped: pile-up with more than max_reads reads");
    }
    for (int32_t i = 0; i < ncr; i++) {
        const int32_t p = crop->pile[(size_t)i];
        if (res->rec[(size_t)p].status != DH_PILE_OK) continue;
        if (active_of[(size_t)p] < 0) {
            active_of[(size_t)p] = (int32_t)lay.pile_of_active.size();
            lay.pile_of_active.push_back(p);
            lay.first_read.push_back((int32_t)lay.keep.size());
        }
        lay.sgroup.push_back(active_of[(size_t)p]);
        lay.keep.push_back(i);
        lay.read_id.push_back(crop->read_id[(size_t)i]);
        const uint8_t kd = crop->kind.empty() ? 0 : crop->kind[(size_t)i];
        lay.rkind.push_back((res->rec[(size_t)p].join & DH_JOIN_EXTENSION) ? ((kd & 3) == 1 ? 0 : 2) : (kd & 3));
        lay.rcomp.push_back(kd >> 2);
// ... 495 lines not shown
        DevBuf<uint16_t> d_tt;
        HIPCHK(d_desc.alloc(desc.size()));
        HIPCHK(d_tt.alloc((size_t)tot));
        if (!tl.empty()) {
            HIPCHK(hipMemcpyAsync(d_desc.p, desc.data(), sizeof(int64_t) * desc.size(), hipMemcpyHostToDevice, st));
            dhk_gather_ranges16(st, pset->d_trace, d_desc.p, (int32_t)tl.size(), d_tt.p);
            HIPCHK(hipGetLastError());
            HIPCHK(hipMemcpyAsync(ttrace.data(), d_tt.p, sizeof(uint16_t) * (size_t)tot, hipMemcpyDeviceToHost, st));
        }
        HIPCHK(hipStreamSynchronize(st));
        if (int rc = consensus_round(ctx, *T, pile, tl, ttrace, ttm, run.tsp, &nT, &nseg, &ncell)) return rc;
    } else if (int rc = consensus_round(ctx, *T, pile, pl, pset->trace, tmpl_of, run.tsp, &nT, &nseg, &ncell))
        return rc;
    run.dbg.dbs.push_back(nT);
    *T = nT;
    run.ps.counters[1] += nseg;
    run.ps.counters[2] += ncell;
    HIPCHK(run.tm.mark(1));
    return run.tm.add_elapsed(0, 1, run.ps.ms[3]);
}

static int align_flanks(ProcRun &run, const PileLayout &lay, dh_db *T, FlankOut &fk)
{
    const dh_process_opts &o = run.o;
    const dh_db *contigs = run.contigs;
    const int32_t na = lay.na, tsp = run.tsp;
    std::vector<int32_t> fidx, fgrp;
    fk.fbase.assign((size_t)na + 1, 0);
    for (int32_t a = 0; a < na; a++) {
        const dh_insertion &rec = run.res->rec[(size_t)lay.pile_of_active[(size_t)a]];
        const int32_t nf = (rec.join & DH_JOIN_EXTENSION) ? 1 : 2;
        const int32_t fw = o.flank_window > 0 ? o.flank_window : INT32_MAX;
        fk.fbase[(size_t)a] = (int32_t)fidx.size();
        for (int32_t f = 0; f < nf; f++) {
            const int32_t g = f == 0 ? rec.contig_left : rec.contig_right;
            const bool front = f == 0 ? (rec.join & DH_JOIN_FLANK0_FRONT) != 0 : (rec.join & DH_JOIN_FLANK1_BACK) == 0;
            const int32_t cl = (int32_t)(contigs->h_off[(size_t)g + 1] - contigs->h_off[(size_t)g]);
            const int32_t wl = front ? 0 : std::max(0, cl - std::min(cl, fw)) / tsp * tsp;
            fidx.push_back(g);
            fk.fbeg.push_back(wl);
            fk.flen.push_back(front ? std::min(cl, fw) : cl - wl);
            fgrp.push_back(a);
        }
    }
    fk.fbase[(size_t)na] = (int32_t)fidx.size();
    dh_db *F = nullptr;
    if (int rc = dh_db_from_slices(run.ctx, contigs, fidx, fk.fbeg, fk.flen, fgrp, &F, true)) return rc;
    run.dbg.dbs.push_back(F);
    if (o.dust)
        if (int rc = dh_db_dust_impl(F)) return rc;
    const dh_align_opts fo = run.align_opts(126, 4, 32);
    HIPCHK(run.tm.mark(0));
    if (int rc = dh_align_db_ex(run.ctx, F, T, &fo, 0, 0, &fk.fset)) return rc;
    run.sg.sets.push_back(fk.fset);
    HIPCHK(run.tm.mark(1));
    if (int rc = run.tm.add_elapsed(0, 1, run.ps.ms[5])) return rc;
    run.tm.lap("flank align");
    return DH_OK;
}

static int32_t insertion_of_pile(ProcRun &run, const PileLayout &lay, const FlankOut &fk, const dh_db *T,
                                 const std::vector<uint8_t> &cons, const std::vector<int32_t> &fl, int32_t a)
{
    const dh_process_opts &o = run.o;
    dh_insertions *res = run.res;
    const dh_la_set *fset = fk.fset;
    const std::vector<int32_t> &fbeg = fk.fbeg, &fbase = fk.fbase;
    const int32_t tsp = run.tsp, ref = lay.ref_of[(size_t)a];
    dh_insertion &rec = res->rec[(size_t)lay.pile_of_active[(size_t)a]];
    const int64_t c0 = T->h_off[(size_t)a], c1 = T->h_off[(size_t)a + 1];
    rec.cons_off = (int64_t)res->bases.size();
    rec.cons_len = (int32_t)(c1 - c0);
    res->bases.insert(res->bases.end(), cons.begin() + c0, cons.begin() + c1);
    const int32_t clen = rec.cons_len;
    const int32_t nf = (rec.join & DH_JOIN_EXTENSION) ? 1 : 2;
    const bool front[2] = {(rec.join & DH_JOIN_FLANK0_FRONT) != 0, (rec.join & DH_JOIN_FLANK1_BACK) == 0};
    const uint8_t refc = ref >= 0 ? lay.rcomp[(size_t)ref] : 0;
    const bool refc_known = run.crop->comp_known && ref >= 0;
    const dh_la *ov[2] = {nullptr, nullptr};
    int cnt[2] = {0, 0};
    for (int32_t i : fl) {
        const dh_la &la = fset->la[(size_t)i];
        const int32_t f = la.aread - fbase[(size_t)a];
        if (f < 0 || f >= nf) continue;
        if (refc_known && ((la.flags & DH_FLAG_COMP) != 0) != (((refc >> f) & 1) != 0)) continue;
        const int32_t fl_len = fk.flen[(size_t)la.aread];
        const bool proper = front[f] ? (la.abpos <= tsp && la.bepos + tsp >= clen) : (la.aepos + tsp >= fl_len && la.bbpos <= tsp);
        if (proper) {
            ov[f] = &la;
            cnt[f]++;
        }
    }
    if (cnt[0] != 1 || (nf == 2 && cnt[1] != 1)) return DH_PILE_FLANKS_NOT_UNIQUE;
    const dh_la *L = ov[0], *R = ov[1];
    if (nf == 2 && ((L->flags & DH_FLAG_COMP) == (R->flags & DH_FLAG_COMP)) != (front[0] != front[1])) return DH_PILE_ORIENTATION;
    rec.left_diffs = L->diffs;
    rec.right_diffs = R ? R->diffs : 0;
    for (int32_t f = 0; f < nf; f++)
        if ((int64_t)ov[f]->diffs * 1000000 > (int64_t)o.max_ins_err_ppm * (ov[f]->aepos - ov[f]->abpos))
            return DH_PILE_MAX_INSERTION_ERROR;
    for (int32_t f = 0; f < nf; f++) {
        dh_la c = *ov[f];
        const int32_t shift = fbeg[(size_t)(fbase[(size_t)a] + f)];
        c.abpos += shift;
        c.aepos += shift;
        c.toff = (int64_t)res->flank_tr.size();
        res->flank_tr.insert(res->flank_tr.end(), fset->trace.begin() + ov[f]->toff, fset->trace.begin() + ov[f]->toff + ov[f]->tlen);
        if (f == 0) res->flank_of[(size_t)lay.pile_of_active[(size_t)a]] = (int32_t)res->flank.size();
        res->flank.push_back(c);
    }
    rec.comp = (L->flags & DH_FLAG_COMP) ? 1 : 0;
    const int32_t sh0 = fbeg[(size_t)fbase[(size_t)a]];
    rec.left_aepos = sh0 + (front[0] ? L->abpos : L->aepos);
    const int32_t p0 = front[0] ? L->bbpos : L->bepos;
    if (nf == 2) {
        const int32_t sh1 = fbeg[(size_t)fbase[(size_t)a] + 1];
        rec.right_abpos = sh1 + (front[1] ? R->abpos : R->aepos);
        int32_t p1 = front[1] ? R->bbpos : R->bepos;
        if ((R->flags & DH_FLAG_COMP) != (L->flags & DH_FLAG_COMP)) p1 = clen - p1;
        rec.ins_begin = front[0] ? p1 : p0;
        rec.ins_end = front[0] ? p0 : p1;
    } else {
        rec.right_abpos = -1;
        rec.ins_begin = front[0] ? 0 : p0;
        rec.ins_end = front[0] ? p0 : clen;
    }
    return rec.ins_end < rec.ins_begin ? DH_PILE_NEGATIVE_INSERTION : DH_PILE_OK;
}

static int make_insertions(ProcRun &run, const PileLayout &lay, const FlankOut &fk, const dh_db *T)
{
    const int32_t na = lay.na;
    std::vector<uint8_t> cons((size_t)std::max<int64_t>(T->total, 1));
    if (T->total > 0) HIPCHK(hipMemcpy(cons.data(), T->d_bases, (size_t)T->total, hipMemcpyDeviceToHost));
    const LaVec &fla = fk.fset->la;
    std::vector<std::vector<int32_t>> fl_of((size_t)na);
    for (size_t i = 0; i < fla.size(); i++)
        if (fla[i].bread >= 0 && fla[i].bread < na) fl_of[(size_t)fla[i].bread].push_back((int32_t)i);
    for (int32_t a = 0; a < na; a++)
        if (lay.active_ok[(size_t)a])
            run.res->rec[(size_t)lay.pile_of_active[(size_t)a]].status = insertion_of_pile(run, lay, fk, T, cons, fl_of[(size_t)a], a);
    return DH_OK;
}

extern "C" int dh_process_cropped(dh_ctx *ctx, dh_db *contigs, dh_cropped *crop, const dh_process_opts *opts,
                                  dh_insertions **out)
{
    int32_t pwidth = 0, palgo = 0;
    if (int rc = check_process_opts(ctx, contigs, crop, opts, out, &pwidth, &palgo)) return rc;
    HIPCHK(hipSetDevice(ctx->device));
    ProcRun run{ctx, ctx->stream, *opts, contigs, crop, opts->tspace_pile, pwidth, palgo};
    ProcStats &ps = run.ps;
    ps.ms[0] = crop->ms_crop;
    if (int rc = run.tm.init(run.st)) return rc;
    init_result(run);
    PileLayout lay;
    if (int rc = plan_pile_db(run, lay)) return rc;
    if (int rc = build_pile_db(run, lay)) return rc;
    if (lay.na > 0) {
        FunnelOut fo;
        FlankOut fk;
        dh_db *T = nullptr;
        if (int rc = align_pile(run, lay, fo)) return rc;
        if (int rc = funnel_and_tile_qv(run, lay, fo)) return rc;
        dh_parallel_for(lay.na, 8, [&](int64_t alo, int64_t ahi) {
            for (int32_t a = (int32_t)alo; a < (int32_t)ahi; a++) rank_reference_read(run, lay, fo, a);
        });
        run.tm.lap("rank reference reads");
        if (int rc = first_consensus_round(run, lay, fo, &T)) return rc;
        const dh_align_opts ro = run.align_opts(500, 4, 32);
        for (int32_t round = 1; round < run.o.rounds; round++)
            if (int rc = realign_round(ctx, lay.pile, ro, &lay.active_ok, run.dbg, run.sg, &run.tm, &ps, &T)) return rc;
        run.tm.lap("consensus rounds");
        if (int rc = align_flanks(run, lay, T, fk)) return rc;
        if (int rc = make_insertions(run, lay, fk, T)) return rc;
    }
    run.tm.lap("insertions");
    ps.ms[6] = ps.ms[0] + ps.ms[1] + ps.ms[2] + ps.ms[3] + ps.ms[4] + ps.ms[5];
    g_pstats = ps;
    *out = run.res;
    run.res = nullptr;
    return DH_OK;
}

extern "C" int64_t dh_propagate_mask(const dh_la *las, int64_t n, const uint16_t *trace, int32_t tspace,
                                     const int64_t *mask_ptr, const int32_t *mask_iv, int32_t ncontigs,
                                     const int64_t *read_off, int32_t nreads, int64_t *out_ptr, int32_t *out_iv,
                                     int64_t cap)
{
    if ((n > 0 && (!las || !trace)) || n < 0 || !mask_ptr || !read_off || !out_ptr || tspace < 1 || ncontigs < 0 || nreads < 0)
        return dh_fail(DH_EINVAL, "dh_propagate_mask: bad argument");
    struct Iv {
        int32_t rd, b, e;
    };
    const int64_t grain = 4096, nchunks = (n + grain - 1) / grain;
    std::vector<std::vector<Iv>> found((size_t)std::max<int64_t>(nchunks, 1));
    std::atomic<int> bad{0};
    dh_parallel_for(nchunks, 1, [&](int64_t clo, int64_t chi) {
        for (int64_t c = clo; c < chi; c++) {
            std::vector<Iv> &out = found[(size_t)c];
            const int64_t i1 = std::min(n, (c + 1) * grain);
            for (int64_t i = c * grain; i < i1; i++) {
                const dh_la &l = las[i];
                if (l.aread < 0 || l.aread >= ncontigs || l.bread < 0 || l.bread >= nreads || l.tlen < 0 || l.tlen % 2 ||
                    l.tlen / 2 != (l.aepos + tspace - 1) / tspace - l.abpos / tspace) {
                    bad = 1;
                    continue;
                }
                const int64_t m0 = mask_ptr[l.aread], m1 = mask_ptr[l.aread + 1];
                if (m1 <= m0) continue;
                int64_t lo = m0, hi = m1;
                while (lo < hi) {
                    const int64_t mid = (lo + hi) >> 1;
                    if (mask_iv[2 * mid + 1] <= l.abpos)
                        lo = mid + 1;
                    else
                        hi = mid;
                }
                const int32_t blen = (int32_t)(read_off[l.bread + 1] - read_off[l.bread]);
                for (int64_t j = lo; j < m1 && mask_iv[2 * j] < l.aepos; j++) {
                    const int32_t ib = std::max(mask_iv[2 * j], l.abpos), ie = std::min(mask_iv[2 * j + 1], l.aepos);
                    int32_t ta, b0, b1;
                    translate_trace_point(l, trace + l.toff, tspace, ib, 0, &ta, &b0);
                    translate_trace_point(l, trace + l.toff, tspace, ie, 1, &ta, &b1);
                    if (l.flags & DH_FLAG_COMP) {
                        const int32_t x0 = blen - b1, x1 = blen - b0;
                        b0 = x0;
                        b1 = x1;
                    }
                    if (b1 > b0) out.push_back(Iv{l.bread, b0, b1});
                }
            }
        }
    });
    if (bad) return dh_fail(DH_EINVAL, "dh_propagate_mask: id out of range or trace length does not fit the A interval");
    std::vector<Iv> all;
    for (auto &v : found) all.insert(all.end(), v.begin(), v.end());
    std::sort(all.begin(), all.end(), [](const Iv &x, const Iv &y) {
        return x.rd != y.rd ? x.rd < y.rd : (x.b != y.b ? x.b < y.b : x.e < y.e);
    });
    int64_t m = 0;
    size_t at = 0;
    for (int32_t r = 0; r < nreads; r++) {
        out_ptr[r] = m;
        while (at < all.size() && all[at].rd == r) {
            int32_t b = all[at].b, e = all[at].e;
            at++;
            while (at < all.size() && all[at].rd == r && all[at].b <= e) {
                e = std::max(e, all[at].e);
                at++;
            }
            if (out_iv && m < cap) {
                out_iv[2 * m] = b;
                out_iv[2 * m + 1] = e;
            }
            m++;
        }
    }
    out_ptr[nreads] = m;
    return m;
}

namespace {
#pragma pack(push, 1)
struct CandRec {
    int32_t gap, read;
    dh_la L, R;
};
struct CropHead {
    int32_t pile, entry, read, len;
};
#pragma pack(pop)
static_assert(sizeof(CandRec) == 104 && sizeof(CropHead) == 16, "blob layouts");
}

static std::mutex g_plan_las_mu;
static std::vector<dh_la_vec> g_plan_las;
struct dh_shard_plan {
    dh_la_vec las;
    dh_pileups *piles = nullptr;
    std::vector<int32_t> owner;
    dh_shard_plan()
    {
        std::lock_guard<std::mutex> lk(g_plan_las_mu);
        if (!g_plan_las.empty()) {
            las = std::move(g_plan_las.back());
            g_plan_las.pop_back();
            las.clear();
        }
    }
    ~dh_shard_plan()
    {
        delete piles;
        std::lock_guard<std::mutex> lk(g_plan_las_mu);
        if (g_plan_las.size() < 8 && las.capacity() > 0 && las.capacity() * sizeof(dh_la) <= ((size_t)64 << 20)) g_plan_las.push_back(std::move(las));
    }
};

extern "C" void dh_shard_free(void *p) { free(p); }

extern "C" int dh_shard_pack_candidates(const dh_pileups *cands, const dh_la *las, int64_t n, int32_t read_shift,
                                        uint8_t **out, int64_t *nbytes)
{
    if (!cands || !out || !nbytes || (n > 0 && !las)) return dh_fail(DH_EINVAL, "dh_shard_pack_candidates: bad argument");
    if (int rc = refuse_general(cands, "dh_shard_pack_candidates")) return rc;
    int64_t tot = 0;
    for (const auto &t : cands->triples) tot += (int64_t)t.size() / 3;
    CandRec *rec = (CandRec *)malloc(std::max<size_t>((size_t)tot * sizeof(CandRec), 1));
    if (!rec) return dh_fail(DH_EINVAL, "dh_shard_pack_candidates: out of memory");
    int64_t at = 0;
    for (size_t g = 0; g < cands->contig_left.size(); g++) {
        const std::vector<int32_t> &t = cands->triples[g];
        for (size_t e = 0; e + 2 < t.size(); e += 3) {
            if (t[e + 1] < 0 || t[e + 1] >= n || t[e + 2] < 0 || t[e + 2] >= n) {
                free(rec);
                return dh_fail(DH_EINVAL, "dh_shard_pack_candidates: LA index out of range");
            }
            CandRec &r = rec[at++];
            r.gap = cands->contig_left[g];
            r.read = t[e] + read_shift;
            r.L = las[t[e + 1]];
            r.R = las[t[e + 2]];
        }
    }
    *out = (uint8_t *)rec;
    *nbytes = tot * (int64_t)sizeof(CandRec);
    return DH_OK;
}

static void plan_owners(dh_shard_plan *p, int32_t world)
{
// ... 292 lines not shown
```

include/dentist_hip.h:

```cpp
#ifndef DENTIST_HIP_H
#define DENTIST_HIP_H

#include <stddef.h>
#include <stdint.h>

#ifdef __cplusplus
extern "C" {
#endif

#define DH_OK 0
#define DH_EINVAL (-1)
#define DH_ENODEV (-2)
#define DH_EHIP (-3)
#define DH_EOVERFLOW (-4)
#define DH_EIO (-5)
#define DH_ENOMEM (-6)

const char *dh_last_error(void);
int32_t dh_abi_version(void);

typedef struct dh_ctx dh_ctx;
int dh_ctx_create(int32_t device, void *stream, dh_ctx **out);
void dh_ctx_destroy(dh_ctx *ctx);
int dh_ctx_sync(dh_ctx *ctx);
// ... 165 lines not shown
    int32_t count;
    int64_t first;
} dh_join;
typedef struct dh_read_alignment {
    int32_t read, la0, la1;
    uint8_t seed0, seed1, n, pad;
} dh_read_alignment;
typedef struct dh_scaffold dh_scaffold;
int dh_scaffold_pileups(const dh_la *las, int64_t n, const int64_t *contig_off, int32_t ncontigs,
                        const int64_t *read_off, int32_t nreads, const int32_t *input_gaps, int32_t ngaps,
                        const dh_scaffold_opts *opts, dh_scaffold **out);
typedef int (*dh_remap_fn)(void *user, const int32_t *contig_ids, int32_t ncontig_ids, const int32_t *read_ids, int32_t nread_ids,
                           dh_la **las_out, int64_t *n_out);
int dh_scaffold_pileups_cb(const dh_la *las, int64_t n, const int64_t *contig_off, int32_t ncontigs, const int64_t *read_off,
                           int32_t nreads, const int32_t *input_gaps, int32_t ngaps, const dh_scaffold_opts *opts,
                           int32_t max_bubble_size, int32_t max_iterations, dh_remap_fn remap, void *user, dh_scaffold **out,
                           dh_la_set **extra, int32_t *resolved);
int dh_scaffold_pileups_resolved(dh_ctx *ctx, dh_db *contigs, dh_db *reads, const dh_la *las, int64_t n, const int32_t *input_gaps,
                                 int32_t ngaps, const dh_scaffold_opts *opts, const dh_align_opts *map_opts, int32_t allowance,
                                 int32_t max_bubble_size, int32_t max_iterations, dh_scaffold **out, dh_la_set **extra,
                                 int32_t *resolved);
int32_t dh_scaffold_npiles(const dh_scaffold *s);
int64_t dh_scaffold_nentries(const dh_scaffold *s);
const dh_join *dh_scaffold_joins(const dh_scaffold *s);
const dh_read_alignment *dh_scaffold_entries(const dh_scaffold *s);
void dh_scaffold_destroy(dh_scaffold *s);
int dh_remap_skipping_reads(dh_ctx *ctx, dh_db *contigs, dh_db *reads, const int32_t *contig_ids, int32_t ncontig_ids,
                            const int32_t *read_ids, int32_t nread_ids, const dh_align_opts *opts, int32_t allowance,
                            dh_la_set **out);
int dh_scaffold_spanning(const dh_scaffold *s, const dh_la *las, int64_t n, dh_pileups **out, int32_t *skipped);
int dh_scaffold_gap_pileups(const dh_scaffold *s, const dh_la *las, int64_t n, dh_pileups **out, int32_t *skipped);
int dh_scaffold_all_pileups(const dh_scaffold *s, const dh_la *las, int64_t n, int32_t only, dh_pileups **out,
                            int32_t *skipped);

int dh_collect_filter(dh_la *las, int64_t n, const int64_t *contig_off, int32_t ncontigs, const int64_t *read_off,
                      int32_t nreads, const int64_t *rep_ptr, const int32_t *rep_iv, const dh_process_opts *opts,
                      int64_t *dropped6, uint8_t *read_used);

int64_t dh_pileups_flat(const dh_pileups *p, int32_t *contig_left, int32_t *count, int32_t *triples);

#define DH_PILE_OK 0
#define DH_PILE_NO_COMMON_TRACE_POINT 1
#define DH_PILE_TOO_SMALL 2
#define DH_PILE_EMPTY_ALIGNMENT 3
#define DH_PILE_FLANKS_NOT_UNIQUE 4
#define DH_PILE_ORIENTATION 5
#define DH_PILE_MAX_INSERTION_ERROR 6
#define DH_PILE_NEGATIVE_INSERTION 7
#define DH_PILE_ALIGN_OVERFLOW 8
#define DH_PILE_UNSUPPORTED_JOIN 9
#define DH_JOIN_FLANK0_FRONT 1
#define DH_JOIN_FLANK1_BACK 2
#define DH_JOIN_EXTENSION 4
typedef struct {
    int32_t contig_left;
    int32_t status;
    int32_t nreads;
    int32_t ref_read;
    int32_t ref_read_id;
    int32_t crop_left;
    int32_t crop_right;
    int32_t left_aepos;
    int32_t right_abpos;
    int32_t ins_begin;
    int32_t ins_end;
    int32_t comp;
    int32_t cons_len;
    int32_t left_diffs, right_diffs;
    int32_t join;
    int64_t cons_off;
    int32_t contig_right;
    int32_t pad;
} dh_insertion;

typedef struct dh_insertions dh_insertions;
int dh_process_pileups(dh_ctx *ctx, dh_db *contigs, dh_db *reads, const dh_la *las, int64_t n,
                       const uint16_t *trace, const dh_pileups *piles, const dh_process_opts *opts,
                       dh_insertions **out);
void dh_insertions_destroy(dh_insertions *r);
int32_t dh_insertions_count(const dh_insertions *r);
const dh_insertion *dh_insertions_records(const dh_insertions *r);
const uint8_t *dh_insertions_bases(const dh_insertions *r);
int64_t dh_insertions_bases_len(const dh_insertions *r);
const int32_t *dh_insertions_read_ids(const dh_insertions *r);
const int32_t *dh_insertions_read_ids_off(const dh_insertions *r);
typedef struct dh_cropped dh_cropped;
int dh_crop_pileups(dh_ctx *ctx, dh_db *contigs, dh_db *reads, int32_t read_first, const dh_la *las, int64_t n,
                    const uint16_t *trace, const dh_pileups *piles, const dh_process_opts *opts,
                    dh_cropped **out);
int dh_crop_pileups_masked(dh_ctx *ctx, dh_db *contigs, dh_db *reads, int32_t read_first, const dh_la *las, int64_t n,
                           const uint16_t *trace, const dh_pileups *piles, const int64_t *rep_ptr, const int32_t *rep_iv,
                           const dh_process_opts *opts, dh_cropped **out);
int dh_process_pileups_masked(dh_ctx *ctx, dh_db *contigs, dh_db *reads, const dh_la *las, int64_t n,
                              const uint16_t *trace, const dh_pileups *piles, const int64_t *rep_ptr, const int32_t *rep_iv,
                              const dh_process_opts *opts, dh_insertions **out);
int dh_process_pileups_set(dh_ctx *ctx, dh_db *contigs, dh_db *reads, dh_la_set *set, const dh_pileups *piles,
                           const int64_t *rep_ptr, const int32_t *rep_iv, const dh_process_opts *opts, dh_insertions **out);
int32_t dh_la_set_trace_on_device(const dh_la_set *s);
int dh_cropped_create(const dh_insertion *rec, int32_t npiles, int32_t nreads, const int32_t *pile,
                      const int32_t *entry, const int32_t *read_id, const int64_t *off, const uint8_t *bases,
                      dh_cropped **out);
int dh_cropped_create2(const dh_insertion *rec, int32_t npiles, int32_t nreads, const int32_t *pile,
                       const int32_t *entry, const int32_t *read_id, const uint8_t *kind, const int64_t *off,
                       const uint8_t *bases, dh_cropped **out);
void dh_cropped_destroy(dh_cropped *c);
int32_t dh_cropped_npiles(const dh_cropped *c);
const uint8_t *dh_cropped_kind(const dh_cropped *c);

typedef struct dh_shard_plan dh_shard_plan;
void dh_shard_free(void *p);
int dh_shard_pack_candidates(const dh_pileups *cands, const dh_la *las, int64_t n, int32_t read_shift, uint8_t **out,
                             int64_t *nbytes);
int dh_shard_plan_create(const uint8_t *const *blobs, const int64_t *sizes, int32_t world, const dh_process_opts *opts,
                         dh_shard_plan **out);
int dh_shard_read_joins(const dh_la *las, int64_t n, const int64_t *contig_off, int32_t ncontigs, const int64_t *read_off,
                        int32_t read_first, int32_t nreads, uint8_t **blob, int64_t *nbytes);
int dh_shard_graph_plan_create(const uint8_t *const *blobs, const int64_t *sizes, int32_t world, int32_t ncontigs,
                               const int32_t *input_gaps, int32_t ngaps, const dh_scaffold_opts *sopts,
                               const dh_process_opts *opts, dh_shard_plan **out);
void dh_shard_plan_destroy(dh_shard_plan *p);
const dh_la *dh_shard_plan_las(const dh_shard_plan *p);
int64_t dh_shard_plan_nlas(const dh_shard_plan *p);
const dh_pileups *dh_shard_plan_pileups(const dh_shard_plan *p);
const int32_t *dh_shard_plan_owner(const dh_shard_plan *p);
int dh_shard_pack_cropped(dh_cropped *crop, const int32_t *owner, int32_t world, uint8_t **blobs, int64_t *sizes);
int dh_shard_unpack_cropped(const uint8_t *const *blobs, const int64_t *sizes, int32_t world, const dh_insertion *rec,
                            int32_t npiles, const int32_t *owner, int32_t rank, dh_cropped **out);
const dh_insertion *dh_cropped_records(const dh_cropped *c);
typedef struct dh_comm dh_comm;
int dh_comm_unique_id(uint8_t *id128);
int dh_comm_create(const uint8_t *id128, int32_t rank, int32_t world, dh_ctx *ctx, dh_comm **out);
int dh_comm_create_local(int32_t world, dh_ctx *const *ctxs, dh_comm **out);
void dh_comm_destroy(dh_comm *c);
int32_t dh_comm_rank(const dh_comm *c);
int32_t dh_comm_world(const dh_comm *c);
int dh_comm_all_gather(dh_comm *c, const uint8_t *payload, int64_t nbytes, uint8_t **out, int64_t *sizes);
int dh_comm_all_to_all(dh_comm *c, const uint8_t *const *per_dest, const int64_t *send_sizes, uint8_t **out,
                       int64_t *recv_sizes);
int dh_shard_run(dh_comm *c, dh_db *contigs, dh_db *reads, int32_t read_first, const int64_t *contig_off, int32_t ncontigs,
                 const dh_la *las, int64_t n, const uint16_t *trace, const dh_process_opts *opts, const dh_pileups *cands,
                 const int64_t *read_off, const int32_t *input_gaps, int32_t ngaps, const struct dh_scaffold_opts *sopts,
                 dh_insertions **out, int64_t *info4);

int32_t dh_cropped_nreads(const dh_cropped *c);
const int32_t *dh_cropped_pile(const dh_cropped *c);
const int32_t *dh_cropped_entry(const dh_cropped *c);
const int32_t *dh_cropped_read_id(const dh_cropped *c);
const int64_t *dh_cropped_offsets(const dh_cropped *c);
const uint8_t *dh_cropped_bases(dh_cropped *c);
int dh_process_cropped(dh_ctx *ctx, dh_db *contigs, dh_cropped *crop, const dh_process_opts *opts,
                       dh_insertions **out);
int dh_get_process_stats(dh_ctx *ctx, float *ms7, int64_t *counters3);
int dh_get_process_work(dh_ctx *ctx, int64_t *work4);


int dh_tile_qv(dh_ctx *ctx, dh_db *db, const dh_la *las, int64_t n, const uint16_t *trace, int32_t tspace,
               int32_t cov, uint8_t *qv, int32_t maxtiles);
int dh_consensus(dh_ctx *ctx, dh_db *db, const dh_la *las, int64_t n, const uint16_t *trace, int32_t tspace,
                 int32_t ref_read, int32_t rounds, uint8_t *out, int64_t cap, int64_t *out_len);

typedef struct dh_edit_paths dh_edit_paths;
int dh_la_edit_paths(dh_ctx *ctx, dh_db *A, dh_db *B, const dh_la *las, int64_t n, const uint16_t *trace,
                     int32_t tspace, int64_t first, int64_t count, dh_edit_paths **out);
int dh_la_set_edit_paths(dh_ctx *ctx, dh_db *A, dh_db *B, const dh_la_set *set, int64_t first, int64_t count,
                         dh_edit_paths **out);
void dh_edit_paths_destroy(dh_edit_paths *p);
int64_t dh_edit_paths_count(const dh_edit_paths *p);
const int64_t *dh_edit_paths_op_off(const dh_edit_paths *p);
const uint8_t *dh_edit_paths_ops(const dh_edit_paths *p);
const int32_t *dh_edit_paths_score(const dh_edit_paths *p);
const int64_t *dh_edit_paths_tile_off(const dh_edit_paths *p);
const uint16_t *dh_edit_paths_tile_score(const dh_edit_paths *p);
int64_t dh_edit_paths_general_tiles(const dh_edit_paths *p);
int64_t dh_format_cigar(const uint8_t *ops, int64_t nops, int32_t extended, char *out, int64_t cap);
int64_t dh_format_alignment(const uint8_t *a, const uint8_t *b, const uint8_t *ops, int64_t nops, int32_t width,
                            char *out, int64_t cap);

int dh_la_transpose(dh_ctx *ctx, dh_db *A, dh_db *B, const dh_la *las, int64_t n, const uint16_t *trace,
                    int32_t tspace, int32_t want_best, dh_la_set **out, int64_t *src_index );
int dh_la_set_transpose(dh_ctx *ctx, dh_db *A, dh_db *B, const dh_la_set *set, int32_t want_best,
                        dh_la_set **out, int64_t *src_index);

int dh_output_fasta(const char *fasta_path, const char *bed_path, const uint8_t *contig_bases,
                    const int64_t *contig_off, int32_t ncontigs, const int32_t *scaffold_of,
                    const char *const *headers, const int32_t *gap_len, const dh_insertion *ins,
                    int32_t nins, const uint8_t *ins_bases, int32_t line_width, int32_t highlight);
typedef struct {
    int32_t line_width, highlight, join_policy, agp_dazzler, agp_skip_read_ids;
    int32_t only;
    const char *agp_version, *tool, *input_assembly;
    int32_t min_extension_length;
    int32_t pad;
} dh_output_opts;
void dh_default_output_opts(dh_output_opts *o);
int dh_scaffold_graph_probe(int32_t ncontigs, const int32_t *joins4, int32_t njoins, int32_t normalize, int32_t *edges4,
                            int32_t *nedges, int32_t *starts2, int32_t *nstarts, const int32_t *walk_start2,
                            const int32_t *walk_first4, int32_t *walk4, int32_t *walk_len, int32_t *cyclic, int32_t cap);
int dh_output_assembly(const char *fasta_path, const char *bed_path, const char *agp_path,
                       const uint8_t *contig_bases, const int64_t *contig_off, int32_t ncontigs,
                       const int32_t *scaffold_of, const char *const *headers, const int32_t *gap_len,
                       const dh_insertion *ins, int32_t nins, const uint8_t *ins_bases, const int32_t *read_ids,
                       const int32_t *read_ids_off, int32_t nreads, const char *const *read_names,
                       const dh_output_opts *opts, int32_t *dropped);

typedef struct dh_dazz dh_dazz;
int dh_dazz_create_dam(const char *path, const char *fasta_text, int64_t n);
int dh_dazz_create_db(const char *path, const char *fasta_text, int64_t n);
int dh_dazz_split(const char *path, int32_t cutoff, int32_t all, int64_t size_mb);
int dh_dazz_open(const char *path, dh_dazz **out);
void dh_dazz_close(dh_dazz *db);
int32_t dh_dazz_nreads(const dh_dazz *db);
int32_t dh_dazz_first_id(const dh_dazz *db);
const uint8_t *dh_dazz_bases(const dh_dazz *db);
const int64_t *dh_dazz_offsets(const dh_dazz *db);
const int32_t *dh_dazz_origin(const dh_dazz *db);
const int32_t *dh_dazz_fpulse(const dh_dazz *db);
const int32_t *dh_dazz_flags(const dh_dazz *db);
const char *dh_dazz_header(const dh_dazz *db, int32_t i);
int64_t dh_dazz_read_mask(const dh_dazz *db, const char *db_path, const char *name, int64_t *ptr, int32_t *iv,
                          int64_t iv_cap);
int dh_dazz_write_mask(const char *db_path, const char *name, int32_t nreads, const int64_t *ptr,
                       const int32_t *iv);

typedef struct {
    int64_t id;
    uint32_t contig_a_id, contig_a_len, contig_b_id, contig_b_len;
    uint8_t flags, seed;
    uint16_t tspace;
    int32_t nla;
} dh_seeded;
typedef struct {
    uint32_t a_begin, a_end, b_begin, b_end, diffs;
    int32_t ntp;
} dh_chain_la;
typedef struct {
    int64_t start_contig, end_contig;
    uint8_t start_part, end_part;
    uint8_t pad[6];
    int64_t seq_len, contig_len;
    int32_t noverlaps, nread_ids;
} dh_insertion_rec;
typedef struct dh_chaindb dh_chaindb;
int dh_pileupdb_write(const char *path, int32_t npiles, const int32_t *nra_of_pile, const int32_t *nsa_of_ra,
                      const dh_seeded *sa, const dh_chain_la *la, const uint16_t *tp);
int dh_pileupdb_read(const char *path, dh_chaindb **out);
int dh_insertiondb_write(const char *path, int32_t nins, const dh_insertion_rec *ins, const uint8_t *bases,
                         const uint32_t *read_ids, const dh_seeded *sa, const dh_chain_la *la, const uint16_t *tp);
int dh_insertiondb_read(const char *path, dh_chaindb **out);
int dh_insertiondb_merge(const char *const *paths, int32_t npaths, const char *out_path, int64_t *ntotal);
int dh_pileups_write_db(const dh_pileups *p, const dh_la *las, int64_t n, const uint16_t *trace,
                        const int64_t *contig_off, int32_t ncontigs, const int64_t *read_off, int32_t nreads,
                        int32_t tspace, const char *path);
int dh_insertions_write_db(const dh_insertions *r, const int64_t *contig_off, int32_t ncontigs, int32_t tspace,
                           const char *path);
void dh_chaindb_destroy(dh_chaindb *d);
int32_t dh_chaindb_npiles(const dh_chaindb *d);
const int32_t *dh_chaindb_pile_counts(const dh_chaindb *d);
int32_t dh_chaindb_nread_alignments(const dh_chaindb *d);
const int32_t *dh_chaindb_read_alignment_counts(const dh_chaindb *d);
int64_t dh_chaindb_nseeded(const dh_chaindb *d);
const dh_seeded *dh_chaindb_seeded(const dh_chaindb *d);
int64_t dh_chaindb_nlas(const dh_chaindb *d);
const dh_chain_la *dh_chaindb_las(const dh_chaindb *d);
int64_t dh_chaindb_ntrace(const dh_chaindb *d);
const uint16_t *dh_chaindb_trace(const dh_chaindb *d);
int32_t dh_chaindb_ninsertions(const dh_chaindb *d);
const dh_insertion_rec *dh_chaindb_insertions(const dh_chaindb *d);
const uint8_t *dh_chaindb_bases(const dh_chaindb *d);
const uint32_t *dh_chaindb_read_ids(const dh_chaindb *d);

int dh_dazz_write_track(const char *db_path, const char *name, int32_t nreads, const int64_t *ptr,
                        const uint8_t *data);
int64_t dh_dazz_read_track(const dh_dazz *db, const char *db_path, const char *name, int64_t *ptr, uint8_t *data,
                           int64_t cap);
int dh_dazz_remove(const char *db_path);

#ifdef __cplusplus
}
#endif
#endif
```

Measured before the change: 2.284 million.

## Classify consensus tiles per segment band and add a narrow one-word bit-parallel fill

Consensus tiles are now sorted into four classes by their own band (half-word, one, two, or four 64-bit words, plus scalar) rather than by the maximum diff of the whole alignment. A new H=1 variant packs Z and L into a single 64-bit word per row, and the vote kernel now reuses the shared editpath fill/traceback helpers instead of its own LDS-based plane code. The intent is to send most tiles to narrower, cheaper bit-vector kernels and to shrink the per-row traceback matrix. In exchange it adds per-tile classification work on the host, more kernel launches, and counters exposed through a new stats API.

```diff
diff --git a/dentist_amd/_lib.py b/dentist_amd/_lib.py
--- a/dentist_amd/_lib.py
+++ b/dentist_amd/_lib.py
@@ -69,7 +69,7 @@
     "dh_las_write", "dh_las_read", "dh_default_process_opts", "dh_collect_spanning", "dh_pileups_destroy",
     "dh_pileups_count", "dh_pileups_get", "dh_process_pileups", "dh_insertions_destroy",
     "dh_insertions_count", "dh_insertions_records", "dh_insertions_bases", "dh_insertions_bases_len",
-    "dh_get_process_stats", "dh_dazz_create_dam", "dh_dazz_create_db", "dh_dazz_split", "dh_dazz_open",
+    "dh_get_process_stats", "dh_get_consensus_classes", "dh_dazz_create_dam", "dh_dazz_create_db", "dh_dazz_split", "dh_dazz_open",
     "dh_dazz_close", "dh_dazz_nreads", "dh_dazz_first_id", "dh_dazz_bases", "dh_dazz_offsets",
     "dh_dazz_origin", "dh_dazz_fpulse", "dh_dazz_header", "dh_dazz_read_mask", "dh_dazz_write_mask",
     "dh_db_set_mask", "dh_output_fasta", "dh_tile_qv", "dh_consensus", "dh_las_merge",
@@ -177,6 +177,7 @@
     L.dh_insertions_bases_len.argtypes = [vp]
     L.dh_insertions_bases_len.restype = i64
     L.dh_get_process_stats.argtypes = [vp, vp, vp]
+    L.dh_get_consensus_classes.argtypes = [vp, vp]
     L.dh_dazz_create_dam.argtypes = [ctypes.c_char_p, ctypes.c_char_p, i64]
     L.dh_dazz_create_db.argtypes = [ctypes.c_char_p, ctypes.c_char_p, i64]
     L.dh_dazz_split.argtypes = [ctypes.c_char_p, i32, i32, i64]
@@ -1480,6 +1481,9 @@
     wk = (ctypes.c_int64 * 4)()
     _check(lib().dh_get_process_work(ctx._h, wk))
     d.update(pile_ups=int(wk[0]), entries=int(wk[1]), cropped_bases=int(wk[2]), algorithmic_bytes=int(wk[3]))
+    ct = (ctypes.c_int64 * 4)()
+    _check(lib().dh_get_consensus_classes(ctx._h, ct))
+    d.update(cons_tiles_w1=int(ct[0]), cons_tiles_w2=int(ct[1]), cons_tiles_w4=int(ct[2]), cons_tiles_scalar=int(ct[3]))
     return d
 
 
diff --git a/dentist_amd/csrc/dh_consensus.hip b/dentist_amd/csrc/dh_consensus.hip
--- a/dentist_amd/csrc/dh_consensus.hip
+++ b/dentist_amd/csrc/dh_consensus.hip
@@ -3,6 +3,7 @@
 #include <stdlib.h>
 
 #include "dh_device.h"
+#include "dh_editpath.h"
 
 #define MAXINS 4
 #define OP_WORD(g) ((uint64_t *)opbuf)[(int64_t)(g)*NDP + dp]
@@ -446,38 +447,13 @@
 #define VP(i)
 #endif
 
-template <int NW>
-struct BV {
-    uint64_t w[NW];
-};
-template <int NW>
-__device__ __forceinline__ BV<NW> bv_shl1(const BV<NW> &a)
-{
-    BV<NW> r;
-#pragma unroll
-    for (int k = NW - 1; k > 0; k--) r.w[k] = (a.w[k] << 1) | (a.w[k - 1] >> 63);
-    r.w[0] = a.w[0] << 1;
-    return r;
-}
-template <int NW>
-__device__ __forceinline__ BV<NW> bv_shr1(const BV<NW> &a, uint64_t top)
-{
-    BV<NW> r;
-#pragma unroll
-    for (int k = 0; k < NW - 1; k++) r.w[k] = (a.w[k] >> 1) | (a.w[k + 1] << 63);
-    r.w[NW - 1] = (a.w[NW - 1] >> 1) | (top << 63);
-    return r;
-}
-
-template <int NW>
+template <int H>
 __global__ void __launch_bounds__(64)
 k_seg_vote_bp(const SegDesc *__restrict__ segs, int32_t nseg, DbView T, DbView R, const uint8_t *__restrict__ rrc,
               uint64_t *__restrict__ dmat, uint8_t *__restrict__ opbuf, uint16_t *__restrict__ nops_out,
               int32_t *__restrict__ status)
 {
-    constexpr int HALF = 32 * NW;
-    constexpr int QW = (SEG_MAX + 63) / 64 + 1 + NW;
-    __shared__ uint64_t s_pl[3][QW][64];
+    constexpr int HALF = 16 * H;
     const int32_t dp = blockIdx.x * blockDim.x + threadIdx.x;
     if (dp >= nseg) return;
     const SegDesc sg = segs[dp];
@@ -490,169 +466,17 @@
     const uint8_t *ref = T.bases + T.off[sg.tmpl] + sg.a0;
     const uint8_t *qry = (sg.comp ? rrc : R.bases) + R.off[sg.bseq] + sg.b0;
     const int64_t NDP = nseg;
-    const int lane = threadIdx.x;
 #ifdef DH_SEED_PROF
     unsigned long long tp_ = wall_clock64();
 #endif
-    {
-        uint64_t a0 = 0, a1 = 0, a2 = 0;
-        int32_t wi = HALF / 64, bi = HALF % 64;
-#pragma unroll
-        for (int k = 0; k < QW; k++) s_pl[0][k][lane] = s_pl[1][k][lane] = s_pl[2][k][lane] = 0;
-        uint64_t qnext = 0;
-        if (ql > 0) __builtin_memcpy(&qnext, qry, 8);
-        for (int32_t j0 = 0; j0 < ql; j0 += 8) {
-            const uint64_t qw = qnext;
-            if (j0 + 8 < ql) __builtin_memcpy(&qnext, qry + j0 + 8, 8);
-#pragma unroll
-            for (int u = 0; u < 8; u++) {
-                const int32_t j = j0 + u;
-                if (j >= ql) break;
-                const uint64_t c = (qw >> (8 * u)) & 7u;
-                a0 |= (c & 1u) << bi;
-                a1 |= ((c >> 1) & 1u) << bi;
-                a2 |= ((c >> 2) & 1u) << bi;
-                if (++bi == 64 || j + 1 == ql) {
-                    s_pl[0][wi][lane] = a0;
-                    s_pl[1][wi][lane] = a1;
-                    s_pl[2][wi][lane] = a2;
-                    a0 = a1 = a2 = 0;
-                    bi = 0;
-                    wi++;
-                }
-            }
-        }
-    }
-    VP(8)
-    BV<NW> p0, p1, p2;
-#pragma unroll
-    for (int k = 0; k < NW; k++) {
-        p0.w[k] = s_pl[0][k][lane];
-        p1.w[k] = s_pl[1][k][lane];
-        p2.w[k] = s_pl[2][k][lane];
-    }
-    uint64_t f0 = s_pl[0][NW][lane], f1 = s_pl[1][NW][lane], f2 = s_pl[2][NW][lane];
-    int32_t fword = NW, fleft = 64;
-    BV<NW> Pv, Mv, lv;
-#pragma unroll
-    for (int k = 0; k < NW; k++) {
-        const uint64_t hi = k * 64 >= HALF ? ~0ull : (k * 64 + 64 <= HALF ? 0ull : ~0ull << (HALF - k * 64));
-        Pv.w[k] = hi;
-        Mv.w[k] = ~hi;
-        const int hb = HALF + 1;
-        lv.w[k] = k * 64 >= hb ? ~0ull : (k * 64 + 64 <= hb ? 0ull : ~0ull << (hb - k * 64));
-    }
-#define DMW(i, k) dmat[((int64_t)(i) * (2 * NW) + (k)) * NDP + dp]
-    uint64_t refw = 0;
-    for (int32_t i = 1; i <= rl; i++) {
-        if (((i - 1) & 7) == 0) __builtin_memcpy(&refw, ref + (i - 1), 8);
-        const uint32_t rc = (uint32_t)(refw >> (8 * ((i - 1) & 7))) & 7u;
-        const uint64_t x0 = 0ull - (uint64_t)(rc & 1u), x1 = 0ull - (uint64_t)((rc >> 1) & 1u), x2 = 0ull - (uint64_t)((rc >> 2) & 1u);
-        {
-            const uint64_t top = lv.w[NW - 1] >> 63;
-            lv = bv_shr1<NW>(lv, top);
-        }
-        BV<NW> Eq, D0, HP, HN;
-        uint64_t carry = 0;
-#pragma unroll
-        for (int k = 0; k < NW; k++) {
-            Eq.w[k] = ~((p0.w[k] ^ x0) | (p1.w[k] ^ x1) | (p2.w[k] ^ x2)) & lv.w[k];
-            const uint64_t x = Eq.w[k] & Pv.w[k];
-            const uint64_t s1 = x + Pv.w[k];
-            const uint64_t c1 = s1 < x ? 1ull : 0ull;
-            const uint64_t s2 = s1 + carry;
-            const uint64_t c2 = s2 < s1 ? 1ull : 0ull;
-            carry = c1 | c2;
-            D0.w[k] = (s2 ^ Pv.w[k]) | Eq.w[k] | Mv.w[k];
-            HP.w[k] = Mv.w[k] | ~(D0.w[k] | Pv.w[k]);
-            HN.w[k] = Pv.w[k] & D0.w[k];
-        }
-        const BV<NW> HPs = bv_shl1<NW>(HP), HNs = bv_shl1<NW>(HN);
-#pragma unroll
-        for (int k = 0; k < NW; k++) {
-            uint64_t A = ~HNs.w[k];
-            const uint64_t B = ~(D0.w[k] & HP.w[k]);
-            const uint64_t t2 = HPs.w[k] & HP.w[k];
-            const uint64_t t1 = (HPs.w[k] & ~HP.w[k] & ~HN.w[k]) | (~HPs.w[k] & ~HNs.w[k] & HP.w[k]);
-            uint64_t L = ~t2 & ~(t1 & D0.w[k]);
-            if (k == 0) {
-                A |= 1ull;
-                L &= ~1ull;
-            }
-            DMW(i, k) = A & B;
-            DMW(i, NW + k) = L;
-        }
-        const BV<NW> Xv = bv_shr1<NW>(D0, 0ull);
-#pragma unroll
-        for (int k = 0; k < NW; k++) {
-            Pv.w[k] = HN.w[k] | ~(Xv.w[k] | HP.w[k]);
-            Mv.w[k] = HP.w[k] & Xv.w[k];
-        }
-        p0 = bv_shr1<NW>(p0, f0 & 1ull);
-        p1 = bv_shr1<NW>(p1, f1 & 1ull);
-        p2 = bv_shr1<NW>(p2, f2 & 1ull);
-        f0 >>= 1;
-        f1 >>= 1;
-        f2 >>= 1;
-        if (--fleft == 0) {
-            fword++;
-            f0 = fword < QW ? s_pl[0][fword][lane] : 0ull;
-            f1 = fword < QW ? s_pl[1][fword][lane] : 0ull;
-            f2 = fword < QW ? s_pl[2][fword][lane] : 0ull;
-            fleft = 64;
-        }
-    }
+    ep::fill_h<H, 2>(ref, rl, qry, ql, dmat + dp, NDP);
     VP(9)
-    int32_t i = rl, j = ql, nops = 0;
-    uint64_t oacc = 0;
-    constexpr int PB = NW == 1 ? 8 : 4;
-    while (i > 0 && j > 0) {
-        uint64_t zr[PB][NW], lr[PB][NW];
-        const int32_t i0 = i;
-#pragma unroll
-        for (int u = 0; u < PB; u++)
-#pragma unroll
-            for (int k = 0; k < NW; k++) {
-                zr[u][k] = i0 - u > 0 ? DMW(i0 - u, k) : 0ull;
-                lr[u][k] = i0 - u > 0 ? DMW(i0 - u, NW + k) : 0ull;
-            }
-#pragma unroll
-        for (int u = 0; u < PB; u++) {
-            while (i == i0 - u && i > 0 && j > 0) {
-                const int32_t Rr = j - i + HALF;
-                uint64_t z = zr[u][0], l = lr[u][0];
-                if (NW > 1 && (Rr >> 6)) {
-                    z = zr[u][NW - 1];
-                    l = lr[u][NW - 1];
-                }
-                const uint8_t op = ((z >> (Rr & 63)) & 1ull) ? 0 : (((l >> (Rr & 63)) & 1ull) ? 2 : 1);
-                if (op == 0) {
-                    --i;
-                    --j;
-                } else if (op == 2) {
-                    --j;
-                } else {
-                    --i;
-                }
-                OP_PUT(op)
-            }
-        }
-    }
-    while (i > 0) {
-        OP_PUT(1)
-        --i;
-    }
-    while (j > 0) {
-        OP_PUT(2)
-        --j;
-    }
-    OP_FLUSH
-    nops_out[dp] = (uint16_t)nops;
+    const EpResult r = ep::traceback_h<H, 2, false>(rl, ql, dmat + dp, NDP, (uint64_t *)opbuf + dp, NDP);
+    nops_out[dp] = (uint16_t)r.nops;
     VP(10)
 #ifdef DH_SEED_PROF
     if (threadIdx.x == 0) atomicAdd(&g_vote_prof[15], 1ull);
 #endif
-#undef DMW
 }
 
 __host__ __device__ inline int32_t seg_vote2_arr(int32_t ncolmax) { return (ncolmax + 2 + 7) & ~7; }
@@ -1205,12 +1029,16 @@
                   uint32_t *vother, int32_t *status, int32_t mode)
 {
     if (nseg <= 0) return;
-    if (mode == 1)
-        hipLaunchKernelGGL(k_seg_vote_bp<1>, dim3((nseg + 63) / 64), dim3(64), 0, st, (const SegDesc *)segs, nseg, T, R, rrc,
+    auto bp = [&](auto kern) {
+        hipLaunchKernelGGL(kern, dim3((nseg + 63) / 64), dim3(64), 0, st, (const SegDesc *)segs, nseg, T, R, rrc,
                            (uint64_t *)dmat, opbuf, nops, status);
+    };
+    if (mode == 3)
+        bp(k_seg_vote_bp<1>);
+    else if (mode == 1)
+        bp(k_seg_vote_bp<2>);
     else if (mode == 2)
-        hipLaunchKernelGGL(k_seg_vote_bp<2>, dim3((nseg + 63) / 64), dim3(64), 0, st, (const SegDesc *)segs, nseg, T, R, rrc,
-                           (uint64_t *)dmat, opbuf, nops, status);
+        bp(k_seg_vote_bp<4>);
     else {
         const size_t lds = (size_t)(2 * bandmax + 2) * 64 + ((size_t)(qmax + 7) / 8 + 1) * 256;
         hipLaunchKernelGGL(k_seg_vote, dim3((nseg + 63) / 64), dim3(64), lds, st, (const SegDesc *)segs, nseg,
@@ -1238,8 +1066,8 @@
         (void)hipMemcpyFromSymbol(h, HIP_SYMBOL(g_vote_prof), sizeof h);
         (void)hipMemcpyToSymbol(HIP_SYMBOL(g_vote_prof), z, sizeof z);
         const double w = h[7] ? (double)h[7] : 1.0, wb = h[15] ? (double)h[15] : 1.0;
-        fprintf(stderr, "[vote prof] fill mode %d, %.0f wavefronts timed: planes %.1f fill %.1f traceback %.1f us/wavefront\n", mode, wb,
-                h[8] / wb / 100.0, h[9] / wb / 100.0, h[10] / wb / 100.0);
+        fprintf(stderr, "[vote prof] fill mode %d, %.0f wavefronts timed: fill %.1f traceback %.1f us/wavefront\n", mode, wb,
+                h[9] / wb / 100.0, h[10] / wb / 100.0);
         fprintf(stderr, "[vote prof] %d tiles, %.0f wavefronts timed: init %.1f ops %.1f canon-del %.1f canon-ins %.1f votes %.1f us/wavefront\n",
                 nseg, w, h[0] / w / 100.0, h[1] / w / 100.0, h[2] / w / 100.0, h[3] / w / 100.0, h[4] / w / 100.0);
     }
diff --git a/dentist_amd/csrc/dh_editpath.h b/dentist_amd/csrc/dh_editpath.h
--- a/dentist_amd/csrc/dh_editpath.h
+++ b/dentist_amd/csrc/dh_editpath.h
@@ -62,16 +62,23 @@
     r[H - 1] = (a[H - 1] >> 1) | (top << 31);
 }
 
-template <int NW>
-EP_HD int64_t dm_index(int32_t i, int p, int k, int64_t stride)
-{
-    return ((int64_t)(i - 1) * (3 * NW) + p * NW + k) * stride;
-}
-
-template <int NW>
-EP_HD void fill(const uint8_t *ref, int32_t rl, const uint8_t *qry, int32_t ql, uint64_t *dm, int64_t stride)
-{
-    constexpr int H = 2 * NW, HALF = 32 * NW;
+template <int H, int PL>
+EP_HD int64_t dm_word(int32_t i, int w, int64_t stride)
+{
+    return ((int64_t)(i - 1) * ((PL * H + 1) / 2) + w) * stride;
+}
+
+EP_HD uint32_t bits_from(int h, int from)
+{
+    return 32 * h >= from ? ~0u : (32 * h + 32 <= from ? 0u : ~0u << (from - 32 * h));
+}
+
+template <int H, int PL>
+EP_HD void fill_h(const uint8_t *ref, int32_t rl, const uint8_t *qry, int32_t ql, uint64_t *dm, int64_t stride)
+{
+    static_assert(H == 1 || H % 2 == 0, "one word or whole 64-bit words");
+    static_assert(PL == 3 ? H % 2 == 0 : PL == 2, "three planes need whole 64-bit words");
+    constexpr int HALF = 16 * H;
     uint32_t p0[H], p1[H], p2[H];
     for (int h = 0; h < H; h++) p0[h] = p1[h] = p2[h] = 0;
     for (int g = 0; g < HALF / 8; g++) {
@@ -84,16 +91,16 @@
             b1 |= ((c >> 1) & 1u) << u;
             b2 |= ((c >> 2) & 1u) << u;
         }
-        const int h = H / 2 + g / 4, sh = 8 * (g & 3);
+        const int h = (HALF + 8 * g) / 32, sh = (HALF + 8 * g) % 32;
         p0[h] |= b0 << sh;
         p1[h] |= b1 << sh;
         p2[h] |= b2 << sh;
     }
     uint32_t Pv[H], Mv[H], lv[H];
     for (int h = 0; h < H; h++) {
-        Pv[h] = h >= H / 2 ? ~0u : 0u;
+        Pv[h] = bits_from(h, HALF);
         Mv[h] = ~Pv[h];
-        lv[h] = h > H / 2 ? ~0u : (h == H / 2 ? ~1u : 0u);
+        lv[h] = bits_from(h, HALF + 1);
     }
     uint64_t refw = 0, qfw = 0;
     for (int32_t i = 1; i <= rl; i++) {
@@ -118,9 +125,11 @@
             S[h] = Eq[h] & Pv[h];
             EM[h] = Eq[h] | Mv[h];
         }
-        {
+        if (H == 1) {
+            sum[0] = S[0] + Pv[0];
+        } else {
             uint64_t carry = 0;
-            for (int k = 0; k < NW; k++) {
+            for (int k = 0; k < H / 2; k++) {
                 const uint64_t x = ((uint64_t)S[2 * k + 1] << 32) | S[2 * k], y = ((uint64_t)Pv[2 * k + 1] << 32) | Pv[2 * k];
                 const uint64_t s1 = x + y, s2 = s1 + carry;
                 carry = (uint64_t)(s1 < x) | (uint64_t)(s2 < s1);
@@ -145,10 +154,14 @@
             L[h] = b3<~(BA & BB) & ~BC>(HPs[h], HP[h], t1);
         }
         L[0] &= ~1u;
-        for (int k = 0; k < NW; k++) {
-            dm[dm_index<NW>(i, 0, k, stride)] = ((uint64_t)Z[2 * k + 1] << 32) | Z[2 * k];
-            dm[dm_index<NW>(i, 1, k, stride)] = ((uint64_t)L[2 * k + 1] << 32) | L[2 * k];
-            dm[dm_index<NW>(i, 2, k, stride)] = ((uint64_t)Eq[2 * k + 1] << 32) | Eq[2 * k];
+        if (H == 1) {
+            dm[dm_word<H, PL>(i, 0, stride)] = ((uint64_t)L[0] << 32) | Z[0];
+        } else {
+            for (int k = 0; k < H / 2; k++) {
+                dm[dm_word<H, PL>(i, k, stride)] = ((uint64_t)Z[2 * k + 1] << 32) | Z[2 * k];
+                dm[dm_word<H, PL>(i, H / 2 + k, stride)] = ((uint64_t)L[2 * k + 1] << 32) | L[2 * k];
+                if (PL == 3) dm[dm_word<H, PL>(i, H + k, stride)] = ((uint64_t)Eq[2 * k + 1] << 32) | Eq[2 * k];
+            }
         }
         shr1<H>(D0, 0u, Xv);
         for (int h = 0; h < H; h++) {
@@ -164,6 +177,12 @@
         shr1<H>(p2, (qc >> 2) & 1u, t);
         for (int h = 0; h < H; h++) p2[h] = t[h];
     }
+}
+
+template <int NW>
+EP_HD void fill(const uint8_t *ref, int32_t rl, const uint8_t *qry, int32_t ql, uint64_t *dm, int64_t stride)
+{
+    fill_h<2 * NW, 3>(ref, rl, qry, ql, dm, stride);
 }
 
 struct OpWriter {
@@ -187,11 +206,12 @@
     }
 };
 
-template <int NW>
-EP_HD EpResult traceback(int32_t rl, int32_t ql, const uint64_t *dm, int64_t stride, uint64_t *ow, int64_t ostride)
-{
-    constexpr int HALF = 32 * NW;
-    constexpr int PB = NW == 1 ? 8 : 4;
+template <int H, int PL, bool CHECK>
+EP_HD EpResult traceback_h(int32_t rl, int32_t ql, const uint64_t *dm, int64_t stride, uint64_t *ow, int64_t ostride)
+{
+    constexpr int HALF = 16 * H;
+    constexpr int NW = H == 1 ? 1 : H / 2;
+    constexpr int PB = H <= 2 ? 8 : 4;
     OpWriter w(ow, ostride);
     int32_t i = rl, j = ql;
     uint32_t cost = 0, bad = 0;
@@ -201,14 +221,14 @@
         for (int u = 0; u < PB; u++)
             for (int k = 0; k < NW; k++) {
                 const bool in = i0 - u > 0;
-                zr[u][k] = in ? dm[dm_index<NW>(i0 - u, 0, k, stride)] : 0ull;
-                lr[u][k] = in ? dm[dm_index<NW>(i0 - u, 1, k, stride)] : 0ull;
-                er[u][k] = in ? dm[dm_index<NW>(i0 - u, 2, k, stride)] : 0ull;
+                zr[u][k] = in ? dm[dm_word<H, PL>(i0 - u, k, stride)] : 0ull;
+                lr[u][k] = H == 1 ? zr[u][k] >> 32 : (in ? dm[dm_word<H, PL>(i0 - u, NW + k, stride)] : 0ull);
+                er[u][k] = PL == 3 && in ? dm[dm_word<H, PL>(i0 - u, 2 * NW + k, stride)] : 0ull;
             }
         for (int u = 0; u < PB; u++) {
             while (i == i0 - u && i > 0 && j > 0) {
                 const int32_t R = j - i + HALF;
-                if ((uint32_t)R >= (uint32_t)(2 * HALF)) {
+                if (CHECK && (uint32_t)R >= (uint32_t)(2 * HALF)) {
                     bad = 1;
                     i = -1;
                     break;
@@ -219,20 +239,20 @@
                     l = lr[u][NW - 1];
                     e = er[u][NW - 1];
                 }
-                const uint32_t sh = (uint32_t)R & 63u;
+                const uint32_t sh = (uint32_t)R & (H == 1 ? 31u : 63u);
                 if ((z >> sh) & 1ull) {
-                    const uint32_t m = (uint32_t)(e >> sh) & 1u;
+                    const uint32_t m = PL == 3 ? (uint32_t)(e >> sh) & 1u : 1u;
                     w.put(m ? EP_OP_MATCH : EP_OP_MISMATCH);
-                    cost += 1u - m;
+                    if (CHECK) cost += 1u - m;
                     --i;
                     --j;
                 } else if ((l >> sh) & 1ull) {
                     w.put(EP_OP_INS);
-                    cost++;
+                    if (CHECK) cost++;
                     --j;
                 } else {
                     w.put(EP_OP_DEL);
-                    cost++;
+                    if (CHECK) cost++;
                     --i;
                 }
             }
@@ -240,12 +260,12 @@
     }
     while (i > 0) {
         w.put(EP_OP_DEL);
-        cost++;
+        if (CHECK) cost++;
         --i;
     }
     while (j > 0 && !bad) {
         w.put(EP_OP_INS);
-        cost++;
+        if (CHECK) cost++;
         --j;
     }
     w.flush();
@@ -254,6 +274,14 @@
     r.score = cost;
     return r;
 }
+
+template <int NW>
+EP_HD EpResult traceback(int32_t rl, int32_t ql, const uint64_t *dm, int64_t stride, uint64_t *ow, int64_t ostride)
+{
+    return traceback_h<2 * NW, 3, true>(rl, ql, dm, stride, ow, ostride);
+}
+
+inline int cons_words(int32_t band) { return band <= 15 ? 1 : (band <= 31 ? 2 : (band <= 63 ? 4 : 0)); }
 
 inline int tile_class(int32_t rl, int32_t ql, int32_t diffs)
 {
diff --git a/dentist_amd/csrc/dh_process.cpp b/dentist_amd/csrc/dh_process.cpp
--- a/dentist_amd/csrc/dh_process.cpp
+++ b/dentist_amd/csrc/dh_process.cpp
@@ -9,6 +9,7 @@
 #include <numeric>
 
 #include "dh_internal.h"
+#include "dh_editpath.h"
 #include "dh_parallel.h"
 
 extern "C" {
@@ -840,8 +841,10 @@
     float ms[7] = {0, 0, 0, 0, 0, 0, 0};
     int64_t counters[3] = {0, 0, 0};
     int64_t work[4] = {0, 0, 0, 0};
+    int64_t cons_tiles[4] = {0, 0, 0, 0};
 };
 static thread_local ProcStats g_pstats;
+static thread_local int64_t g_cons_tiles[4] = {0, 0, 0, 0};
 
 extern "C" int dh_get_process_work(dh_ctx *ctx, int64_t *work4)
 {
@@ -855,6 +858,13 @@
     if (!ctx) return dh_fail(DH_EINVAL, "ctx is NULL");
     if (ms7) memcpy(ms7, g_pstats.ms, sizeof(g_pstats.ms));
     if (counters3) memcpy(counters3, g_pstats.counters, sizeof(g_pstats.counters));
+    return DH_OK;
+}
+
+extern "C" int dh_get_consensus_classes(dh_ctx *ctx, int64_t *tiles4)
+{
+    if (!ctx || !tiles4) return dh_fail(DH_EINVAL, "dh_get_consensus_classes: NULL argument");
+    memcpy(tiles4, g_pstats.cons_tiles, sizeof(g_pstats.cons_tiles));
     return DH_OK;
 }
 
@@ -867,13 +877,24 @@
     std::vector<SegDescH, PinnedAlloc<SegDescH>> segs;
     int32_t wmax = 1, bandmax = 1;
     int64_t ncell = 0;
-    size_t class_end[3] = {0, 0, 0};
+    size_t class_end[4] = {0, 0, 0, 0};
+    const bool all_scalar = getenv("DH_CONS_SCALAR") != nullptr;
+    const bool no_narrow = getenv("DH_CONS_NO_NARROW") != nullptr;
+    auto tile_band = [](int32_t diffs, int32_t rl, int32_t ql) { return std::min<int32_t>(diffs, std::max(rl, ql)) + 1; };
+    auto tile_cls = [&](int32_t band) {
+        const int h = all_scalar ? 0 : ep::cons_words(band);
+        return h == 0 ? 3 : (h == 4 ? 2 : (h == 2 || no_narrow ? 1 : 0));
+    };
     {
-        std::vector<size_t> sel;
-        std::vector<size_t> soff(1, 0);
+        struct Sel {
+            size_t la;
+            uint32_t n[4];
+        };
+        std::vector<Sel> sel;
+        std::vector<std::array<size_t, 4>> soff;
         {
             const int64_t grain = 1 << 16, nch = ((int64_t)las.size() + grain - 1) / grain;
-            std::vector<std::array<std::vector<size_t>, 3>> part((size_t)std::max<int64_t>(nch, 1));
+            std::vector<std::vector<Sel>> part((size_t)std::max<int64_t>(nch, 1));
             dh_parallel_for(nch, 1, [&](int64_t clo, int64_t chi) {
                 for (int64_t c = clo; c < chi; c++) {
                     const size_t i1 = std::min(las.size(), (size_t)(c + 1) * (size_t)grain);
@@ -881,42 +902,51 @@
                         if (tmpl_of[i] >= 0 && !(las[i].flags & DH_FLAG_DISABLED)) {
                             const uint16_t *tr = trace.data() + las[i].toff;
                             bool too_long = false;
-                            int32_t dmax = 0;
+                            Sel x{i, {0, 0, 0, 0}};
+                            int32_t a0 = las[i].abpos;
                             for (int32_t e = 0; e < las[i].tlen / 2; e++) {
                                 too_long = too_long || tr[2 * e + 1] > SEG_MAX;
-                                dmax = std::max<int32_t>(dmax, tr[2 * e]);
+                                const int32_t a1 = std::min((a0 / ts + 1) * ts, las[i].aepos);
+                                x.n[tile_cls(tile_band(tr[2 * e], a1 - a0, tr[2 * e + 1]))]++;
+                                a0 = a1;
                             }
-                            if (!too_long) part[(size_t)c][dmax + 1 <= 31 ? 0 : (dmax + 1 <= 63 ? 1 : 2)].push_back(i);
+                            if (!too_long) part[(size_t)c].push_back(x);
                         }
                 }
             });
-            for (int cls = 0; cls < 3; cls++) {
-                for (const auto &v : part)
-                    for (size_t i : v[(size_t)cls]) {
-                        sel.push_back(i);
-                        soff.push_back(soff.back() + (size_t)(las[i].tlen / 2));
-                    }
-                class_end[cls] = soff.back();
-            }
-        }
-        segs.resize(soff.back());
+            size_t total[4] = {0, 0, 0, 0};
+            for (const auto &v : part)
+                for (const Sel &x : v) {
+                    sel.push_back(x);
+                    soff.push_back({total[0], total[1], total[2], total[3]});
+                    for (int k = 0; k < 4; k++) total[k] += x.n[k];
+                }
+            size_t base[4];
+            for (int k = 0; k < 4; k++) {
+                base[k] = k ? class_end[k - 1] : 0;
+                class_end[k] = base[k] + total[k];
+            }
+            for (auto &o : soff)
+                for (int k = 0; k < 4; k++) o[(size_t)k] += base[k];
+        }
+        segs.resize(class_end[3]);
         std::mutex red;
         dh_parallel_for((int64_t)sel.size(), 256, [&](int64_t lo_, int64_t hi_) {
             int32_t wm = 1, bm = 1;
             int64_t nc = 0;
             for (int64_t q = lo_; q < hi_; q++) {
-                const size_t i = sel[(size_t)q];
+                const size_t i = sel[(size_t)q].la;
                 const int32_t t = tmpl_of[i];
                 const dh_la &la = las[i];
                 const uint16_t *tr = trace.data() + la.toff;
-                SegDescH *out = segs.data() + soff[(size_t)q];
+                std::array<size_t, 4> at = soff[(size_t)q];
                 int32_t a0 = la.abpos, b0 = la.bbpos;
                 for (int32_t e = 0; e < la.tlen / 2; e++) {
                     int32_t a1 = (a0 / ts + 1) * ts;
                     if (a1 > la.aepos) a1 = la.aepos;
                     const int32_t b1 = b0 + tr[2 * e + 1];
-                    const int32_t band = std::min<int32_t>((int32_t)tr[2 * e], std::max(a1 - a0, b1 - b0)) + 1;
-                    out[e] = SegDescH{t, a0, a1, la.bread, b0, b1, (int32_t)(la.flags & DH_FLAG_COMP), band};
+                    const int32_t band = tile_band(tr[2 * e], a1 - a0, b1 - b0);
+                    segs[at[(size_t)tile_cls(band)]++] = SegDescH{t, a0, a1, la.bread, b0, b1, (int32_t)(la.flags & DH_FLAG_COMP), band};
                     wm = std::max(wm, b1 - b0);
                     bm = std::max(bm, band);
                     nc += (int64_t)(a1 - a0) * std::min(b1 - b0, 2 * band + 1);
@@ -930,6 +960,7 @@
             ncell += nc;
         });
     }
+    for (int k = 0; k < 4; k++) g_cons_tiles[k] += (int64_t)(class_end[k] - (k ? class_end[k - 1] : 0));
     *nseg_out = (int64_t)segs.size();
     *ncell_out = ncell;
     const int32_t nt = T->n;
@@ -964,11 +995,11 @@
     uint32_t *d_vother = d_cdiff.p + ncolp, *d_csums = d_vother + ncolp;
     HIPCHK(dhk_memset(st, d_cdiff.p, 0, sizeof(uint32_t) * 2 * ncolp));
     if (int rc = dh_ensure_rc(R)) return rc;
-    for (int cls = 0; cls < 3; cls++) {
+    for (int cls = 0; cls < 4; cls++) {
         const size_t c0 = cls ? class_end[cls - 1] : 0, c1 = class_end[cls];
         if (c1 <= c0) continue;
-        const int32_t mode = getenv("DH_CONS_SCALAR") ? 0 : (cls == 0 ? 1 : (cls == 1 ? 2 : 0));
-        const size_t mrow = mode ? (size_t)16 * (size_t)mode : 4 * (size_t)((2 * bandmax + 16) >> 4);
+        const int32_t mode = cls == 0 ? 3 : (cls == 1 ? 1 : (cls == 2 ? 2 : 0));
+        const size_t mrow = mode == 3 ? 8 : (mode ? (size_t)16 * (size_t)mode : 4 * (size_t)((2 * bandmax + 16) >> 4));
         const int64_t per_dp = (int64_t)(ts + 1) * (int64_t)mrow + 2 * SEG_MAX;
         const int64_t max_dp = std::max<int64_t>(4096, (6ll << 30) / per_dp);
         for (size_t s0 = c0; s0 < c1; s0 += (size_t)max_dp) {
@@ -1187,6 +1218,7 @@
         return dh_fail(DH_EINVAL, "dh_consensus: bad argument");
     HIPCHK(hipSetDevice(ctx->device));
     hipStream_t st = ctx->stream;
+    memset(g_cons_tiles, 0, sizeof(g_cons_tiles));
     DbGuard dbg;
     SetGuard sg;
     LaVec pl(las, las + n);
@@ -1210,6 +1242,7 @@
     const dh_align_opts ro = pile_align_opts(tspace, 500, 4, 32);
     for (int32_t round = 1; round < rounds; round++)
         if (int rc = realign_round(ctx, db, ro, nullptr, dbg, sg, nullptr, nullptr, &T)) return rc;
+    memcpy(g_pstats.cons_tiles, g_cons_tiles, sizeof(g_cons_tiles));
     *out_len = T->total;
     if (T->total > cap) return dh_fail(DH_EOVERFLOW, "dh_consensus: output buffer too small");
     if (T->total > 0) HIPCHK(hipMemcpyAsync(out, T->d_bases, (size_t)T->total, hipMemcpyDeviceToHost, st));
@@ -1719,6 +1752,7 @@
         for (int i = 0; i < 7; i++) g_pstats.ms[i] = std::max(g_pstats.ms[i], sts[(size_t)k].ms[i]);
         for (int i = 0; i < 3; i++) g_pstats.counters[i] += sts[(size_t)k].counters[i];
         for (int i = 0; i < 4; i++) g_pstats.work[i] += sts[(size_t)k].work[i];
+        for (int i = 0; i < 4; i++) g_pstats.cons_tiles[i] += sts[(size_t)k].cons_tiles[i];
     }
     dh_insertions *r0 = res[0];
     for (int32_t k = 1; k < nparts; k++) {
@@ -2520,6 +2554,7 @@
     ProcRun run{ctx, ctx->stream, *opts, contigs, crop, opts->tspace_pile, pwidth, palgo};
     ProcStats &ps = run.ps;
     ps.ms[0] = crop->ms_crop;
+    memset(g_cons_tiles, 0, sizeof(g_cons_tiles));
     if (int rc = run.tm.init(run.st)) return rc;
     init_result(run);
     PileLayout lay;
@@ -2545,6 +2580,7 @@
     }
     run.tm.lap("insertions");
     ps.ms[6] = ps.ms[0] + ps.ms[1] + ps.ms[2] + ps.ms[3] + ps.ms[4] + ps.ms[5];
+    memcpy(ps.cons_tiles, g_cons_tiles, sizeof(g_cons_tiles));
     g_pstats = ps;
     *out = run.res;
     run.res = nullptr;
diff --git a/include/dentist_hip.h b/include/dentist_hip.h
--- a/include/dentist_hip.h
+++ b/include/dentist_hip.h
@@ -341,6 +341,7 @@
                        dh_insertions **out);
 int dh_get_process_stats(dh_ctx *ctx, float *ms7, int64_t *counters3);
 int dh_get_process_work(dh_ctx *ctx, int64_t *work4);
+int dh_get_consensus_classes(dh_ctx *ctx, int64_t *tiles4);
 
 
 int dh_tile_qv(dh_ctx *ctx, dh_db *db, const dh_la *las, int64_t n, const uint16_t *trace, int32_t tspace,
```

New measurement: 2.165 million. 0.948x the previous value.
